# jhultman/vision3d

Measured on AMD Instinct MI355X. Metric: frames/sec SECOND fwd, 16k-pt KITTI cloud, higher is better.
Workload: dtype f16x3-scaled (fp32-class): fp32 operands split into f16 hi + lo pieces of x * s under per-tensor power-of-two scales, 3 MFMA terms (lo*hi + hi*lo + hi*hi), fp32 accumulate; relative product error 2^-22 -- the result differs from the reference's fp32 modules by fp32 summation noise: strict elementwis

## Files before the change

### include/vision3d_hip.h

```cpp
#ifndef VISION3D_HIP_H
#define VISION3D_HIP_H

#include <stddef.h>
#include <stdint.h>

#ifdef __cplusplus
extern "C" {
#endif

#define V3D_OK 0
#define V3D_EINVAL (-1)
#define V3D_EWORKSPACE (-2)
#define V3D_EUNSUPPORTED (-3)

typedef void* v3d_stream_t;

const char* v3d_version(void);
int v3d_hip_runtime_version(void);
const char* v3d_compiler_version(void);
const char* v3d_error_string(int code);

int v3d_box_iou_rotated(const float* boxes1, int M, const float* boxes2, int N, float* ious, v3d_stream_t stream);

int v3d_box_iou_rotated_3d(const float* boxes1, int M, const float* boxes2, int N, float* ious, v3d_stream_t stream);

size_t v3d_nms_rotated_workspace(int N);
int v3d_nms_rotated(const float* boxes, const float* scores, int N, float iou_threshold, int64_t* keep,
                    int32_t* n_keep, void* workspace, size_t workspace_bytes, v3d_stream_t stream);

size_t v3d_proposals_workspace(int B, int n_cls, int topk);
int v3d_proposals(const float* head_maps, const float* anchors, int B, int n_cls, int n_yaw, int H, int W, int topk,
                  const float* score_thresh_host, float iou_threshold, float* out_boxes, int64_t* out_batch_idx,
                  int64_t* out_class_idx, float* out_scores, int32_t* n_out, void* workspace, size_t workspace_bytes,
                  v3d_stream_t stream);
int v3d_proposals_flag(const float* head_maps, const float* anchors, int B, int n_cls, int n_yaw, int H, int W, int topk,
                       const float* score_thresh_host, float iou_threshold, float* out_boxes, int64_t* out_batch_idx,
                       int64_t* out_class_idx, float* out_scores, int32_t* n_out , const int32_t* aux_flag,
                       void* workspace, size_t workspace_bytes, v3d_stream_t stream);
int v3d_proposals_topk(const float* head_maps, const float* anchors, int B, int n_cls, int n_yaw, int H, int W, int topk,
                       float* boxes, float* scores, void* workspace, size_t workspace_bytes, v3d_stream_t stream);
size_t v3d_refine_nms_workspace(int B, int n_cls, int topk);
int v3d_refine_nms(const float* deltas, const float* proposals, const float* conf, int B, int n_cls, int topk,
                   const float* score_thresh_host, float iou_threshold, float* refined, float* out_boxes, int64_t* out_batch_idx,
                   int64_t* out_class_idx, float* out_scores, int32_t* n_out, void* workspace, size_t workspace_bytes,
                   v3d_stream_t stream);

size_t v3d_sparse_bn_workspace(int n, int C);
int v3d_sparse_bn_relu_fwd(const float* x, int n, int C, const float* gamma, const float* beta, float eps, int relu, float* y,
                           float* save_mean, float* save_invstd, float* var_unbiased, float* running_mean ,
                           float* running_var , float momentum,
                           int64_t* num_batches_tracked , void* workspace, size_t workspace_bytes,
                           v3d_stream_t stream);
int v3d_sparse_bn_relu_bwd(const float* x, const float* dy, int n, int C, const float* gamma, const float* beta,
                           const float* save_mean, const float* save_invstd, int relu, float* dx, float* dgamma, float* dbeta,
                           void* workspace, size_t workspace_bytes, v3d_stream_t stream);

size_t v3d_assign_targets_workspace(int n_gt, int n_cls, int anchors_per_class);
int v3d_assign_targets(const float* gt_boxes, const int64_t* gt_class, int n_gt, const float* anchors, int n_cls,
                       int anchors_per_class, const float* iou_thresh_host, int allow_low_quality, int8_t* G_cls, uint8_t* M_cls,
                       float* G_reg, uint8_t* M_reg, int64_t* matches, void* workspace, size_t workspace_bytes,
                       v3d_stream_t stream);

int v3d_refine_targets(const float* proposals, const int64_t* proposal_class, int B, int n, const float* gt_boxes,
                       const int64_t* gt_class, const int32_t* gt_offsets, int n_gt, const float* draws, float conf_lo, float conf_hi,
                       float reg_iou, float fg_iou, int rois_per_frame, int fg_quota, float* iou, int64_t* match, float* conf,
                       float* G_reg, uint8_t* M_cls, uint8_t* M_reg, v3d_stream_t stream);

size_t v3d_augment_work_bytes(int N, int n, int k);
int v3d_augment_frame(const float* points, int N, int C, const float* boxes, const int64_t* class_idx, int n,
                      const float* db_points, const float* db_boxes, const void* samples, int k, int sample_points, int flip,
                      double factor, double cos_theta, double sin_theta, double theta, float* out_points, float* out_boxes,
                      int64_t* out_class_idx, void* work, size_t work_bytes, v3d_stream_t stream);

size_t v3d_object_noise_workspace(int n_boxes, int T);
int v3d_object_noise(const float* points, const int32_t* point_offsets_host, const float* boxes, const int32_t* box_offsets_host,
                     int B, int C, const float* trans, const float* rot, int T, float collision_iou, float* out_points,
                     float* out_boxes, int32_t* chosen, void* workspace, size_t workspace_bytes, v3d_stream_t stream);

#define V3D_DATABASE_MAX_BOXES 256
size_t v3d_database_work_bytes(int n_points, int n_boxes, int n_frames);
int v3d_database_extract(const float* points, int n_points, int C, const int32_t* point_offsets, const double* box_prep, int n_boxes,
                         const int32_t* box_offsets, int n_frames, int min_pts, int32_t* counts, int32_t* starts, int32_t* src_index,
                         float* out_points, int64_t cap, int32_t* totals, void* work, size_t work_bytes, v3d_stream_t stream);

int v3d_points_in_boxes(const float* points, int N, int C, const float* boxes, int n, int use_z, uint8_t* mask,
                        v3d_stream_t stream);

size_t v3d_voxelize_workspace(int n_points);
int v3d_voxelize(const float* points, int n_points, int C, const int32_t* frame_offsets_host, int B,
                 const float* voxel_size_host, const float* bounds_host, int max_pts, int max_voxels, float* voxels,
                 int32_t* coords, int32_t* occupancy, float* mean, int32_t* n_voxels, void* workspace,
                 size_t workspace_bytes, v3d_stream_t stream);

size_t v3d_rulebook_workspace(int cap_in, int cap_out, int K);
int v3d_rulebook_subm(const int32_t* coords, const int32_t* n, int cap, const int32_t* spatial_shape_host,
                      const int32_t* ksize_host, int32_t* nbr, void* workspace, size_t workspace_bytes,
                      v3d_stream_t stream);
int v3d_rulebook_sparse(const int32_t* coords_in, const int32_t* n_in, int cap_in,
                        const int32_t* spatial_shape_host, const int32_t* ksize_host, const int32_t* stride_host,
                        const int32_t* padding_host, int32_t* coords_out, int32_t* n_out, int cap_out, int32_t* nbr,
                        int32_t* overflow, void* workspace, size_t workspace_bytes, v3d_stream_t stream);

int v3d_sparse_conv_fwd(const float* in, const float* weight, const int32_t* nbr, const int32_t* n_out, int cap_out,
                        int K, int Cin, int Cout, const float* scale, const float* shift, int relu, float* out,
                        int algo, v3d_stream_t stream);

#define V3D_PREC_BF16X3 0
#define V3D_PREC_F16S 1
size_t v3d_sparse_conv_weight_image_bytes(int K, int Cin, int Cout);
int v3d_sparse_conv_pack_weights(const float* weight, int K, int Cin, int Cout, int prec, void* image, v3d_stream_t stream);
int v3d_act_scale_from_rows(const float* rows, const int32_t* n_rows, int cap, int C, int headroom_bits, float* entry,
                            uint32_t* scratch, v3d_stream_t stream);
int v3d_sparse_conv_fwd_packed(const float* in, const void* weight_image, const int32_t* nbr, const int32_t* n_out,
                               int cap_out, int K, int Cin, int Cout, const float* scale, const float* shift, int relu,
                               float* out, int rows_hint, int prec, const float* act_in, const float* act_next,
                               int32_t* range_flag, const void* in_split, void* out_split, v3d_stream_t stream);
int v3d_sparse_rows_split(const float* rows, const int32_t* n_rows, int cap, int C, int prec, const float* act_entry,
                          void* out_split, v3d_stream_t stream);
size_t v3d_sparse_brick_table_bytes(int cap, int K, size_t* lidx_bytes, size_t* ulist_bytes, size_t* ucnt_bytes,
                                    size_t* tmask_bytes);
int v3d_sparse_brick_plan(const int32_t* nbr, const int32_t* n_rows, int cap, int K, uint16_t* lidx, int32_t* ulist,
                          int32_t* ucnt, uint32_t* tmask, v3d_stream_t stream);
int v3d_sparse_conv_fwd_brick(const void* in_split, const void* weight_image, const int32_t* nbr, const uint16_t* lidx,
                              const int32_t* ulist, const int32_t* ucnt, const uint32_t* tmask, const int32_t* n_out,
                              int cap, int K, int Cin, int Cout, const float* scale, const float* shift, int relu, float* out,
                              int prec, const float* act_in, const float* act_next, int32_t* range_flag, void* out_split,
                              v3d_stream_t stream);

int v3d_rulebook_transpose(const int32_t* nbr, const int32_t* n_out, int cap_out, int K, int cap_in, int32_t* nbr_t,
                           v3d_stream_t stream);
size_t v3d_sparse_conv_bwd_weight_workspace(int K, int Cin, int Cout);
int v3d_sparse_conv_bwd_weight(const float* X, const float* dY, const int32_t* nbr, const int32_t* n_out, int cap_out,
                               int K, int Cin, int Cout, float* dW, void* workspace, size_t workspace_bytes,
                               v3d_stream_t stream);

int v3d_densify(const float* feat, const int32_t* coords, const int32_t* n, int cap, int B, int C,
                const int32_t* spatial_shape_host, float* dense, v3d_stream_t stream);

size_t v3d_fps_workspace(int B, int N);
int v3d_furthest_point_sample(const float* xyz, int B, int N, int K, int32_t* idx, void* workspace,
                              size_t workspace_bytes, v3d_stream_t stream);
size_t v3d_keypoints_sector_workspace(int B, int N, int S);
int v3d_keypoints_sector(const float* points, int point_stride, int B, int N, int K, int S, const float* proposals, int P, float radius,
                         int32_t* idx, int32_t* sector_counts, void* workspace, size_t workspace_bytes, v3d_stream_t stream);
int v3d_gather_points(const float* feat, const int32_t* idx, int B, int C, int N, int K, float* out,
                      v3d_stream_t stream);
int v3d_ball_query(const float* xyz, const float* new_xyz, int B, int N, int M, float radius_a, int nsample_a, int32_t* idx_a,
                   float radius_b, int nsample_b, int32_t* idx_b, v3d_stream_t stream);
size_t v3d_ball_query_grid_workspace(int B, int N);
int v3d_ball_query_grid(const float* xyz, const float* new_xyz, int B, int N, int M, float radius_a, int nsample_a, int32_t* idx_a,
                        float radius_b, int nsample_b, int32_t* idx_b, void* workspace, size_t workspace_bytes, v3d_stream_t stream);
int v3d_ball_query_grid_build(int n_db, const float* const* xyz, const int32_t* N, const float* radius_max, void* const* workspace,
                              const size_t* workspace_bytes, int B, v3d_stream_t stream);
int v3d_ball_query_grid_query(const float* new_xyz, int B, int N, int M, float radius_a, int nsample_a, int32_t* idx_a,
                              float radius_b, int nsample_b, int32_t* idx_b, const void* workspace, size_t workspace_bytes,
                              v3d_stream_t stream);
int v3d_ball_query_grid_query_many(int n_jobs, const float* new_xyz, int B, int M, const int32_t* N, const float* radius_a,
                                   const int32_t* nsample_a, int32_t* const* idx_a, const float* radius_b, const int32_t* nsample_b,
                                   int32_t* const* idx_b, const void* const* workspace, const size_t* workspace_bytes,
                                   v3d_stream_t stream);
int v3d_group_points(const float* feat, const int32_t* idx, int B, int C, int N, int M, int nsample, float* out,
                     v3d_stream_t stream);
int v3d_bev_bilinear(const float* feature_map, const float* grid, int B, int C, int H, int W, int K, float* out,
                     v3d_stream_t stream);
int v3d_bev_gather_keypoints(const float* feature_map, const float* keypoint_xyz, int B, int C, int H, int W, int K, float offset_x,
                             float offset_y, float pixel_x, float pixel_y, float* out, int ldo, v3d_stream_t stream);

int v3d_voxel_centers(const int32_t* indices, int n, float scale_x, float scale_y, float scale_z, float offset_x, float offset_y,
                      float offset_z, float* out, v3d_stream_t stream);
int v3d_roi_grid_points(const float* boxes, const float* samples, const float* cos_yaw, const float* sin_yaw, int n_boxes, int m,
                        float* out, v3d_stream_t stream);

int v3d_sa_mlp_layer(const float* feat, const float* xyz, const float* new_xyz, const int32_t* idx, int B, int N, int M, int ns,
                     int Kf, const float* W, const float* bias, int Nout, int relu, int pool, float* out, int ldo, int n_store,
                     v3d_stream_t stream);
int v3d_sa_mlp_pair(const float* P, const float* xyz, const float* new_xyz, const int32_t* idx, int B, int N, int M, int ns, int K1,
                    int ldp, const float* wx, const float* b1, const float* W, const float* bias, int Nout, int relu, int pool,
                    float* out, int ldo, int n_store, v3d_stream_t stream);
int v3d_sa_mlp_pair2(const float* P_a, const float* P_b, const float* xyz, const float* new_xyz, const int32_t* idx_a, const int32_t* idx_b,
                     int B, int N, int M, int ns_a, int ns_b, int K1, int ldp, const float* wx_a, const float* b1_a, const float* wx_b,
                     const float* b1_b, const float* W_a, const float* bias_a, const float* W_b, const float* bias_b, int Nout, int relu,
                     int pool, float* out_a, float* out_b, int ldo, int n_store, v3d_stream_t stream);
int v3d_linear_rows(const float* A, int lda, int R, int K, const float* W, const float* bias, int Nout, int relu, float* out, int ldo,
                    int n_store, v3d_stream_t stream);
int v3d_linear_rows_many(int n_jobs, const float* const* A, const int32_t* lda, const int32_t* R, const int32_t* K, const float* const* W,
                         const float* const* bias, const int32_t* Nout, const int32_t* relu, float* const* out, const int32_t* ldo,
                         const int32_t* n_store, v3d_stream_t stream);

typedef struct v3d_backbone v3d_backbone;
typedef struct {
  int32_t subm;
  int32_t cin, cout;
  int32_t ksize[3], stride[3], padding[3];
  int32_t key;
  int32_t relu;
} v3d_layer_desc;
typedef struct {
  float voxel_size[3];
  float bounds[6];
  int32_t max_pts, max_voxels;
  int32_t point_channels;
  int32_t grid_shape[3];
  int32_t max_batch, max_points;
  int32_t n_layers;
  float growth;
  int32_t conv_algo;
} v3d_backbone_config;
int v3d_backbone_create(const v3d_backbone_config* cfg, const v3d_layer_desc* layers, v3d_backbone** out);
void v3d_backbone_destroy(v3d_backbone* plan);
size_t v3d_backbone_arena_bytes(const v3d_backbone* plan);
int v3d_backbone_num_layers(const v3d_backbone* plan);
int v3d_backbone_set_layer(v3d_backbone* plan, int layer, const float* weight, const float* scale, const float* shift,
                           v3d_stream_t stream);
int v3d_backbone_forward(v3d_backbone* plan, const float* points, int n_points, const int32_t* frame_offsets_host,
                         int B, float* dense_nchw, void* dense_hi, void* dense_lo, v3d_stream_t stream);
int v3d_backbone_layer_output(v3d_backbone* plan, int layer, float** features, int32_t** coords,
                              int32_t** n_rows_dev, int* cap, int* channels, int32_t* shape_host);
int v3d_backbone_tune(v3d_backbone* plan);
int32_t* v3d_backbone_occupancy(v3d_backbone* plan);
int32_t* v3d_backbone_overflow_flags(v3d_backbone* plan);

size_t v3d_conv2d_weight_image_bytes(int Cin, int Cout, int ksize);
size_t v3d_bev_occupancy_words(int B, int H, int W);
int v3d_bev_occupancy_bits(const int32_t* coords , const int32_t* n, int cap, int B, int H, int W,
                           uint32_t* occ, v3d_stream_t stream);
uint32_t* v3d_backbone_bev_occupancy(v3d_backbone* plan);
int v3d_backbone_bev_planes(v3d_backbone* plan, void** hi, void** lo);
int v3d_backbone_set_throughput_mode(v3d_backbone* plan, int on);
int v3d_backbone_set_precision(v3d_backbone* plan, int prec);
int v3d_backbone_precision(const v3d_backbone* plan);
int v3d_backbone_set_presplit(v3d_backbone* plan, int on);
float* v3d_backbone_act_scales(v3d_backbone* plan);
int v3d_backbone_set_calibrating(v3d_backbone* plan, int on);
int v3d_backbone_calibrate(v3d_backbone* plan, int headroom_bits, v3d_stream_t stream);
int v3d_conv2d_bg_tiles(int B, int H, int W);
typedef struct v3d_conv2d_prec {
  int32_t prec;
  const float* in_entry;
  const float* out_entry;
  int32_t* range_flag;
  const float* w_inv;
  const float* w_inv2;
} v3d_conv2d_prec;
int v3d_conv2d_pack_weights(const float* weight, const float* scale, int Cout, int Cin, int ksize, int prec, void* image,
                            v3d_stream_t stream);
int v3d_conv2d_nhwc_split(const void* x_hi, const void* x_lo, const void* weight_image, const float* bias, int relu, int B,
                          int H, int W, int Cin, int Cout, int ksize, void* y_hi, void* y_lo, float* y_nchw,
                          const uint32_t* occ, int reach, const void* bg_hi, const void* bg_lo, uint32_t* work,
                          uint32_t* tile_state, uint32_t* reset_ptr, int reset_words, const v3d_conv2d_prec* pr,
                          v3d_stream_t stream);
int v3d_conv2d_1x1_head_fused(const void* x_hi, const void* x_lo, const void* w1_image, const float* b1, int relu1,
                              const void* w2_image, const float* b2, int relu2, int B, int H, int W, int Cmid, int Cout2,
                              float* y_nchw, const v3d_conv2d_prec* pr, v3d_stream_t stream);
int v3d_nchw_to_split_nhwc(const float* x, int B, int C, int H, int W, void* out_hi, void* out_lo, int prec,
                           const float* act_entry, v3d_stream_t stream);
int v3d_densify_nhwc_split(const float* feat, const int32_t* coords, const int32_t* n, int cap, int B, int C,
                           const int32_t* spatial_shape_host, void* out_hi, void* out_lo, v3d_stream_t stream);
int v3d_split_nhwc_to_nchw(const void* x_hi, const void* x_lo, int B, int C, int H, int W, float* out, v3d_stream_t stream);
int v3d_backbone_forward_reuse(v3d_backbone* plan, int B, float* dense_nchw, void* dense_hi, void* dense_lo, v3d_stream_t stream);

int v3d_backbone_forward_voxels(v3d_backbone* plan, const float* voxel_mean, const int32_t* coords, int n_voxels, int B,
                                float* dense_nchw, void* dense_hi, void* dense_lo, v3d_stream_t stream);

size_t v3d_proposal_loss_workspace(void);
int v3d_proposal_loss_fwd_bwd(const float* maps, const int8_t* g_cls, const uint8_t* m_cls, const float* g_reg, const uint8_t* m_reg,
                              int B, int n_cls, int n_yaw, int H, int W, float alpha, float gamma, float* losses, float* dmaps,
                              void* workspace, size_t workspace_bytes, v3d_stream_t stream);
int v3d_proposal_loss_scale(float* dmaps, int B, int n_cls, int n_yaw, int H, int W, const float* g_cls, const float* g_reg,
                            v3d_stream_t stream);

int v3d_refine_loss_fwd_bwd(const float* R_reg, int ld_reg, const float* R_cls, int ld_cls, const float* G_conf, const float* G_reg,
                            const uint8_t* M_cls, const uint8_t* M_reg, int rows, float* losses, float* dR_reg, float* dR_cls,
                            v3d_stream_t stream);
int v3d_refine_loss_scale(float* dR_reg, float* dR_cls, int rows, const float* g_cls, const float* g_reg, v3d_stream_t stream);

int v3d_keypoint_weight(const float* hidden, int ldh, int H, const float* w2, const float* b2, float* feats, int ldf, int C,
                        int rows, float* logits, v3d_stream_t stream);

int v3d_keypoint_seg_loss_fwd_bwd(const float* keypoints, const float* logits, int B, int K, const float* gt_boxes,
                                  const int64_t* gt_class, const int32_t* gt_offsets, int n_gt, const float* extra_host, float alpha,
                                  float gamma, uint8_t* labels, float* losses, float* d_logits, v3d_stream_t stream);
int v3d_keypoint_seg_loss_scale(float* d_logits, int rows, const float* g, v3d_stream_t stream);

size_t v3d_voxel_query_workspace(int cap);
int v3d_voxel_query(const float* points, int rows, int rows_per_frame, const int32_t* coords, const int32_t* n, int cap,
                    const int32_t* shape_host, const float* scale_host, const float* offset_host, const int32_t* range_host,
                    float radius, int nsample, int32_t* idx, uint8_t* empty, void* workspace, size_t workspace_bytes,
                    v3d_stream_t stream);
int v3d_voxel_pool_pair(const float* P, int ldp, const int32_t* coords, int cap, const float* points, const int32_t* idx, int rows,
                        int nsample, const float* scale_host, const float* offset_host, int K1, const float* wx, const float* b1,
                        const float* W, const float* bias, int Nout, float* out, int ldo, v3d_stream_t stream);

int v3d_center_targets(const float* boxes, const int32_t* classes, const int32_t* box_offsets_host, int B, int n_cls, int H, int W,
                       const double* geom_host, double min_overlap, int min_radius, float* heat, int32_t* ind, uint8_t* mask,
                       int32_t* cls, float* reg, v3d_stream_t stream);
size_t v3d_center_loss_workspace(void);
int v3d_center_loss_fwd_bwd(const float* maps, const float* heat, const int32_t* ind, const uint8_t* mask, const float* reg, int B,
                            int n_cls, int H, int W, float alpha, float beta, const float* code_weights_host, float* losses,
                            float* dmaps, void* workspace, size_t workspace_bytes, v3d_stream_t stream);
int v3d_center_loss_scale(float* dmaps, int B, int n_cls, int H, int W, const float* g_hm, const float* g_reg, v3d_stream_t stream);
size_t v3d_center_decode_workspace(int B, int n_cls, int H, int W);
int v3d_center_decode(const float* maps, int B, int n_cls, int H, int W, const double* geom_host, int topk, float* boxes,
                      float* scores, void* workspace, size_t workspace_bytes, v3d_stream_t stream);

typedef struct {
  const float* weight;
  const float* gamma;
  const float* beta;
  float* running_mean;
  float* running_var;
  int64_t* num_batches_tracked;
  float eps, momentum;
  float* grad_weight;
  float* grad_gamma;
  float* grad_beta;
} v3d_train_layer;
int v3d_backbone_train_forward(v3d_backbone* plan, const float* voxel_mean, const int32_t* coords, int n_voxels, int B,
                               const v3d_train_layer* layers_host, float* dense_out ,
                               void* dense_nhwc_bf16 ,
                               v3d_stream_t stream);
int v3d_backbone_train_backward(v3d_backbone* plan, const float* grad_dense ,
                                const void* grad_nhwc_bf16, int B, const v3d_train_layer* layers_host, v3d_stream_t stream);
size_t v3d_backbone_train_arena_bytes(const v3d_backbone* plan);
int v3d_backbone_tune_from_voxels(v3d_backbone* plan, const int32_t* coords, int n_voxels, int B, v3d_stream_t stream);


size_t v3d_dense_train_weight_image_bytes(int ksize);
int v3d_dense_train_pack_weights(const float* weight, int ksize, int transpose, void* image, v3d_stream_t stream);
int v3d_dense_train_conv_tiles(int B, int H, int W);
int v3d_dense_train_conv(const void* x, const void* image, int B, int H, int W, int ksize, void* y, float* stats,
                         v3d_stream_t stream);
int v3d_dense_train_bn_finalize(const float* stats, int tiles, long long count, float eps, float momentum, float* mean,
                                float* invstd, float* running_mean, float* running_var, int64_t* num_batches_tracked,
                                v3d_stream_t stream);
int v3d_dense_train_bn_relu_apply(const void* x, long long M, const float* mean, const float* invstd, const float* gamma,
                                  const float* beta, int relu, void* y, v3d_stream_t stream);
size_t v3d_dense_train_bn_bwd_workspace(void);
int v3d_dense_train_bn_relu_bwd(const void* x, const void* dy, long long M, const float* mean, const float* invstd,
                                const float* gamma, const float* beta, int relu, void* dx, float* dgamma, float* dbeta,
                                void* workspace, size_t workspace_bytes, v3d_stream_t stream);
size_t v3d_dense_train_wgrad_workspace(int ksize);
int v3d_dense_train_wgrad(const void* x, const void* dy, int B, int H, int W, int ksize, float* dw, void* workspace,
                          size_t workspace_bytes, v3d_stream_t stream);
size_t v3d_dense_train_head_workspace(int O);
int v3d_dense_train_head_fwd(const void* feat, int B, int H, int W, const float* weight, const float* bias, int O, float* maps,
                             v3d_stream_t stream);
int v3d_dense_train_head_bwd(const void* feat, const float* dmaps, int B, int H, int W, const float* weight, int O, void* dfeat,
                             float* dweight, float* dbias, void* workspace, size_t workspace_bytes, v3d_stream_t stream);
typedef struct {
  const float* weight;
  const float* gamma;
  const float* beta;
  float* running_mean;
  float* running_var;
  int64_t* num_batches_tracked;
  float eps, momentum;
  int32_t ksize;
  float* grad_weight;
  float* grad_gamma;
  float* grad_beta;
} v3d_dense_train_layer;
size_t v3d_dense_train_arena_bytes(int B, int H, int W, int n_layers, int O);
int v3d_dense_train_arena_init(void* arena, int B, int H, int W, int n_layers, int O, v3d_stream_t stream);
int v3d_dense_train_forward(const void* bev, int B, int H, int W, const v3d_dense_train_layer* layers, int n_layers,
                            const float* head_weight, const float* head_bias, int O, void* arena, float* maps, v3d_stream_t stream);
int v3d_dense_train_backward(const void* bev, const float* dmaps, int B, int H, int W, const v3d_dense_train_layer* layers,
                             int n_layers, const float* head_weight, int O, void* arena, float* dhead_weight, float* dhead_bias,
                             void* dbev, v3d_stream_t stream);
size_t v3d_dense_train_arena_bytes_split(int B, int H, int W, int n_layers, int O);
int v3d_dense_train_forward_split(const void* bev_hi, const void* bev_lo, int B, int H, int W, const v3d_dense_train_layer* layers,
                                  int n_layers, const float* head_weight, const float* head_bias, int O, void* arena, float* maps,
                                  v3d_stream_t stream);
int v3d_dense_train_backward_split(const void* bev_hi, const void* bev_lo, const float* dmaps, int B, int H, int W,
                                   const v3d_dense_train_layer* layers, int n_layers, const float* head_weight, int O, void* arena,
                                   float* dhead_weight, float* dhead_bias, void* dbev_hi, void* dbev_lo, v3d_stream_t stream);

#define V3D_KITTI_MAX_DT 1024
#define V3D_KITTI_MAX_GT 256
#define V3D_KITTI_MAX_COMBOS 1024
#define V3D_KITTI_COMBO_CHUNK 64
#define V3D_KITTI_SAMPLE_PTS 41
#define V3D_KITTI_CODE_CAR 0
#define V3D_KITTI_CODE_PEDESTRIAN 1
#define V3D_KITTI_CODE_CYCLIST 2
// ... 37 lines not shown
```

### vision3d_amd/_lib.py

```python
import ctypes as C
import contextlib
import os

import torch

_HERE = os.path.dirname(os.path.abspath(__file__))
LIB_PATH = os.environ.get("V3D_HIP_LIB") or os.path.join(_HERE, "lib", "libvision3d_hip.so")

_vp, _i, _f, _sz = C.c_void_p, C.c_int, C.c_float, C.c_size_t

_SIGNATURES = {
    "v3d_version": (C.c_char_p, []),
    "v3d_hip_runtime_version": (_i, []),
    "v3d_compiler_version": (C.c_char_p, []),
    "v3d_error_string": (C.c_char_p, [_i]),
    "v3d_box_iou_rotated": (_i, [_vp, _i, _vp, _i, _vp, _vp]),
    "v3d_box_iou_rotated_3d": (_i, [_vp, _i, _vp, _i, _vp, _vp]),
    "v3d_nms_rotated_workspace": (_sz, [_i]),
    "v3d_nms_rotated": (_i, [_vp, _vp, _i, _f, _vp, _vp, _vp, _sz, _vp]),
    "v3d_proposals_workspace": (_sz, [_i, _i, _i]),
    "v3d_proposals": (_i, [_vp, _vp, _i, _i, _i, _i, _i, _i, _vp, _f, _vp, _vp, _vp, _vp, _vp, _vp, _sz, _vp]),
    "v3d_proposals_flag": (_i, [_vp, _vp, _i, _i, _i, _i, _i, _i, _vp, _f, _vp, _vp, _vp, _vp, _vp, _vp, _vp, _sz, _vp]),
    "v3d_proposals_topk": (_i, [_vp, _vp, _i, _i, _i, _i, _i, _i, _vp, _vp, _vp, _sz, _vp]),
    "v3d_refine_nms_workspace": (_sz, [_i, _i, _i]),
    "v3d_refine_nms": (_i, [_vp, _vp, _vp, _i, _i, _i, _vp, _f, _vp, _vp, _vp, _vp, _vp, _vp, _vp, _sz, _vp]),
    "v3d_sparse_bn_workspace": (_sz, [_i, _i]),
    "v3d_sparse_bn_relu_fwd": (_i, [_vp, _i, _i, _vp, _vp, _f, _i, _vp, _vp, _vp, _vp, _vp, _vp, _f, _vp, _vp, _sz, _vp]),
    "v3d_sparse_bn_relu_bwd": (_i, [_vp, _vp, _i, _i, _vp, _vp, _vp, _vp, _i, _vp, _vp, _vp, _vp, _sz, _vp]),
    "v3d_assign_targets_workspace": (_sz, [_i, _i, _i]),
    "v3d_assign_targets": (_i, [_vp, _vp, _i, _vp, _i, _i, _vp, _i, _vp, _vp, _vp, _vp, _vp, _vp, _sz, _vp]),
    "v3d_points_in_boxes": (_i, [_vp, _i, _i, _vp, _i, _i, _vp, _vp]),
    "v3d_augment_work_bytes": (_sz, [_i, _i, _i]),
    "v3d_augment_frame": (_i, [_vp, _i, _i, _vp, _vp, _i, _vp, _vp, _vp, _i, _i, _i, C.c_double, C.c_double, C.c_double, C.c_double,
                               _vp, _vp, _vp, _vp, _sz, _vp]),
    "v3d_object_noise_workspace": (_sz, [_i, _i]),
    "v3d_object_noise": (_i, [_vp, _vp, _vp, _vp, _i, _i, _vp, _vp, _i, _f, _vp, _vp, _vp, _vp, _sz, _vp]),
    "v3d_database_work_bytes": (_sz, [_i, _i, _i]),
    "v3d_database_extract": (_i, [_vp, _i, _i, _vp, _vp, _i, _vp, _i, _i, _vp, _vp, _vp, _vp, C.c_int64, _vp, _vp, _sz, _vp]),
    "v3d_voxelize_workspace": (_sz, [_i]),
    "v3d_voxelize": (_i, [_vp, _i, _i, _vp, _i, _vp, _vp, _i, _i, _vp, _vp, _vp, _vp, _vp, _vp, _sz, _vp]),
    "v3d_rulebook_workspace": (_sz, [_i, _i, _i]),
    "v3d_rulebook_subm": (_i, [_vp, _vp, _i, _vp, _vp, _vp, _vp, _sz, _vp]),
    "v3d_rulebook_sparse": (_i, [_vp, _vp, _i, _vp, _vp, _vp, _vp, _vp, _vp, _i, _vp, _vp, _vp, _sz, _vp]),
    "v3d_sparse_conv_fwd": (_i, [_vp, _vp, _vp, _vp, _i, _i, _i, _i, _vp, _vp, _i, _vp, _i, _vp]),
    "v3d_sparse_conv_weight_image_bytes": (_sz, [_i, _i, _i]),
    "v3d_sparse_conv_pack_weights": (_i, [_vp, _i, _i, _i, _i, _vp, _vp]),
    "v3d_sparse_conv_fwd_packed": (_i, [_vp, _vp, _vp, _vp, _i, _i, _i, _i, _vp, _vp, _i, _vp, _i, _i, _vp, _vp, _vp, _vp, _vp, _vp]),
    "v3d_sparse_rows_split": (_i, [_vp, _vp, _i, _i, _i, _vp, _vp, _vp]),
    "v3d_sparse_brick_table_bytes": (_sz, [_i, _i, _vp, _vp, _vp, _vp]),
    "v3d_sparse_brick_plan": (_i, [_vp, _vp, _i, _i, _vp, _vp, _vp, _vp, _vp]),
    "v3d_sparse_conv_fwd_brick": (_i, [_vp, _vp, _vp, _vp, _vp, _vp, _vp, _vp, _i, _i, _i, _i, _vp, _vp, _i, _vp, _i, _vp, _vp, _vp, _vp, _vp]),
    "v3d_act_scale_from_rows": (_i, [_vp, _vp, _i, _i, _i, _vp, _vp, _vp]),
    "v3d_rulebook_transpose": (_i, [_vp, _vp, _i, _i, _i, _vp, _vp]),
    "v3d_sparse_conv_bwd_weight_workspace": (_sz, [_i, _i, _i]),
    "v3d_sparse_conv_bwd_weight": (_i, [_vp, _vp, _vp, _vp, _i, _i, _i, _i, _vp, _vp, _sz, _vp]),
    "v3d_densify": (_i, [_vp, _vp, _vp, _i, _i, _i, _vp, _vp, _vp]),
    "v3d_fps_workspace": (_sz, [_i, _i]),
    "v3d_furthest_point_sample": (_i, [_vp, _i, _i, _i, _vp, _vp, _sz, _vp]),
    "v3d_keypoints_sector_workspace": (_sz, [_i, _i, _i]),
    "v3d_keypoints_sector": (_i, [_vp, _i, _i, _i, _i, _i, _vp, _i, _f, _vp, _vp, _vp, _sz, _vp]),
    "v3d_gather_points": (_i, [_vp, _vp, _i, _i, _i, _i, _vp, _vp]),
    "v3d_ball_query": (_i, [_vp, _vp, _i, _i, _i, _f, _i, _vp, _f, _i, _vp, _vp]),
    "v3d_ball_query_grid_workspace": (_sz, [_i, _i]),
    "v3d_ball_query_grid": (_i, [_vp, _vp, _i, _i, _i, _f, _i, _vp, _f, _i, _vp, _vp, _sz, _vp]),
    "v3d_ball_query_grid_build": (_i, [_i, _vp, _vp, _vp, _vp, _vp, _i, _vp]),
    "v3d_ball_query_grid_query_many": (_i, [_i, _vp, _i, _i, _vp, _vp, _vp, _vp, _vp, _vp, _vp, _vp, _vp, _vp]),
    "v3d_ball_query_grid_query": (_i, [_vp, _i, _i, _i, _f, _i, _vp, _f, _i, _vp, _vp, _sz, _vp]),
    "v3d_group_points": (_i, [_vp, _vp, _i, _i, _i, _i, _i, _vp, _vp]),
    "v3d_bev_bilinear": (_i, [_vp, _vp, _i, _i, _i, _i, _i, _vp, _vp]),
    "v3d_sa_mlp_layer": (_i, [_vp, _vp, _vp, _vp, _i, _i, _i, _i, _i, _vp, _vp, _i, _i, _i, _vp, _i, _i, _vp]),
    "v3d_sa_mlp_pair": (_i, [_vp, _vp, _vp, _vp, _i, _i, _i, _i, _i, _i, _vp, _vp, _vp, _vp, _i, _i, _i, _vp, _i, _i, _vp]),
    "v3d_voxel_centers": (_i, [_vp, _i, _f, _f, _f, _f, _f, _f, _vp, _vp]),
    "v3d_sa_mlp_pair2": (_i, [_vp, _vp, _vp, _vp, _vp, _vp, _i, _i, _i, _i, _i, _i, _i, _vp, _vp, _vp, _vp, _vp, _vp, _vp, _vp, _i, _i, _i,
                              _vp, _vp, _i, _i, _vp]),
    "v3d_roi_grid_points": (_i, [_vp, _vp, _vp, _vp, _i, _i, _vp, _vp]),
    "v3d_linear_rows_many": (_i, [_i, _vp, _vp, _vp, _vp, _vp, _vp, _vp, _vp, _vp, _vp, _vp, _vp]),
    "v3d_linear_rows": (_i, [_vp, _i, _i, _i, _vp, _vp, _i, _i, _vp, _i, _i, _vp]),
    "v3d_bev_gather_keypoints": (_i, [_vp, _vp, _i, _i, _i, _i, _i, _f, _f, _f, _f, _vp, _i, _vp]),
    "v3d_backbone_create": (_i, [_vp, _vp, _vp]),
    "v3d_backbone_destroy": (None, [_vp]),
    "v3d_backbone_arena_bytes": (_sz, [_vp]),
    "v3d_backbone_tune": (_i, [_vp]),
    "v3d_backbone_num_layers": (_i, [_vp]),
    "v3d_backbone_set_layer": (_i, [_vp, _i, _vp, _vp, _vp, _vp]),
    "v3d_backbone_layer_output": (_i, [_vp, _i, _vp, _vp, _vp, _vp, _vp, _vp]),
    "v3d_backbone_occupancy": (_vp, [_vp]),
    "v3d_backbone_overflow_flags": (_vp, [_vp]),
    "v3d_backbone_forward": (_i, [_vp, _vp, _i, _vp, _i, _vp, _vp, _vp, _vp]),
    "v3d_backbone_forward_reuse": (_i, [_vp, _i, _vp, _vp, _vp, _vp]),
    "v3d_backbone_forward_voxels": (_i, [_vp, _vp, _vp, _i, _i, _vp, _vp, _vp, _vp]),
    "v3d_backbone_train_forward": (_i, [_vp, _vp, _vp, _i, _i, _vp, _vp, _vp, _vp]),
    "v3d_backbone_train_backward": (_i, [_vp, _vp, _vp, _i, _vp, _vp]),
    "v3d_backbone_train_arena_bytes": (_sz, [_vp]),
    "v3d_backbone_tune_from_voxels": (_i, [_vp, _vp, _i, _i, _vp]),
    "v3d_bev_occupancy_words": (_sz, [_i, _i, _i]),
    "v3d_bev_occupancy_bits": (_i, [_vp, _vp, _i, _i, _i, _i, _vp, _vp]),
    "v3d_backbone_bev_occupancy": (_vp, [_vp]),
    "v3d_backbone_bev_planes": (_i, [_vp, C.POINTER(_vp), C.POINTER(_vp)]),
    "v3d_backbone_set_throughput_mode": (_i, [_vp, _i]),
    "v3d_conv2d_bg_tiles": (_i, [_i, _i, _i]),
    "v3d_conv2d_pack_weights": (_i, [_vp, _vp, _i, _i, _i, _i, _vp, _vp]),
    "v3d_conv2d_nhwc_split": (_i, [_vp, _vp, _vp, _vp, _i, _i, _i, _i, _i, _i, _i, _vp, _vp, _vp, _vp, _i, _vp, _vp, _vp, _vp, _vp, _i, _vp, _vp]),
    "v3d_conv2d_1x1_head_fused": (_i, [_vp, _vp, _vp, _vp, _i, _vp, _vp, _i, _i, _i, _i, _i, _i, _vp, _vp, _vp]),
    "v3d_nchw_to_split_nhwc": (_i, [_vp, _i, _i, _i, _i, _vp, _vp, _i, _vp, _vp]),
    "v3d_backbone_set_precision": (_i, [_vp, _i]),
    "v3d_backbone_precision": (_i, [_vp]),
    "v3d_backbone_set_presplit": (_i, [_vp, _i]),
    "v3d_backbone_act_scales": (_vp, [_vp]),
    "v3d_backbone_set_calibrating": (_i, [_vp, _i]),
    "v3d_backbone_calibrate": (_i, [_vp, _i, _vp]),
    "v3d_proposal_loss_workspace": (_sz, []),
    "v3d_proposal_loss_fwd_bwd": (_i, [_vp, _vp, _vp, _vp, _vp, _i, _i, _i, _i, _i, _f, _f, _vp, _vp, _vp, _sz, _vp]),
    "v3d_proposal_loss_scale": (_i, [_vp, _i, _i, _i, _i, _i, _vp, _vp, _vp]),
    "v3d_refine_targets": (_i, [_vp, _vp, _i, _i, _vp, _vp, _vp, _i, _vp, _f, _f, _f, _f, _i, _i, _vp, _vp, _vp, _vp, _vp, _vp, _vp]),
    "v3d_refine_loss_fwd_bwd": (_i, [_vp, _i, _vp, _i, _vp, _vp, _vp, _vp, _i, _vp, _vp, _vp, _vp]),
    "v3d_refine_loss_scale": (_i, [_vp, _vp, _i, _vp, _vp, _vp]),
    "v3d_keypoint_weight": (_i, [_vp, _i, _i, _vp, _vp, _vp, _i, _i, _i, _vp, _vp]),
    "v3d_keypoint_seg_loss_fwd_bwd": (_i, [_vp, _vp, _i, _i, _vp, _vp, _vp, _i, _vp, _f, _f, _vp, _vp, _vp, _vp]),
    "v3d_keypoint_seg_loss_scale": (_i, [_vp, _i, _vp, _vp]),
    "v3d_voxel_query_workspace": (_sz, [_i]),
    "v3d_voxel_query": (_i, [_vp, _i, _i, _vp, _vp, _i, _vp, _vp, _vp, _vp, _f, _i, _vp, _vp, _vp, _sz, _vp]),
    "v3d_voxel_pool_pair": (_i, [_vp, _i, _vp, _i, _vp, _vp, _i, _i, _vp, _vp, _i, _vp, _vp, _vp, _vp, _i, _vp, _i, _vp]),
    "v3d_center_targets": (_i, [_vp, _vp, _vp, _i, _i, _i, _i, _vp, C.c_double, _i, _vp, _vp, _vp, _vp, _vp, _vp]),
    "v3d_center_loss_workspace": (_sz, []),
    "v3d_center_loss_fwd_bwd": (_i, [_vp, _vp, _vp, _vp, _vp, _i, _i, _i, _i, _f, _f, _vp, _vp, _vp, _vp, _sz, _vp]),
    "v3d_center_loss_scale": (_i, [_vp, _i, _i, _i, _i, _vp, _vp, _vp]),
    "v3d_center_decode_workspace": (_sz, [_i, _i, _i, _i]),
    "v3d_center_decode": (_i, [_vp, _i, _i, _i, _i, _vp, _i, _vp, _vp, _vp, _sz, _vp]),
    "v3d_conv2d_weight_image_bytes": (_sz, [_i, _i, _i]),
    "v3d_densify_nhwc_split": (_i, [_vp, _vp, _vp, _i, _i, _i, _vp, _vp, _vp, _vp]),
    "v3d_split_nhwc_to_nchw": (_i, [_vp, _vp, _i, _i, _i, _i, _vp, _vp]),
    "v3d_dense_train_weight_image_bytes": (_sz, [_i]),
    "v3d_dense_train_pack_weights": (_i, [_vp, _i, _i, _vp, _vp]),
    "v3d_dense_train_conv_tiles": (_i, [_i, _i, _i]),
    "v3d_dense_train_conv": (_i, [_vp, _vp, _i, _i, _i, _i, _vp, _vp, _vp]),
    "v3d_dense_train_bn_finalize": (_i, [_vp, _i, C.c_longlong, _f, _f, _vp, _vp, _vp, _vp, _vp, _vp]),
    "v3d_dense_train_bn_relu_apply": (_i, [_vp, C.c_longlong, _vp, _vp, _vp, _vp, _i, _vp, _vp]),
    "v3d_dense_train_bn_bwd_workspace": (_sz, []),
    "v3d_dense_train_bn_relu_bwd": (_i, [_vp, _vp, C.c_longlong, _vp, _vp, _vp, _vp, _i, _vp, _vp, _vp, _vp, _sz, _vp]),
    "v3d_dense_train_wgrad_workspace": (_sz, [_i]),
    "v3d_dense_train_wgrad": (_i, [_vp, _vp, _i, _i, _i, _i, _vp, _vp, _sz, _vp]),
    "v3d_dense_train_head_workspace": (_sz, [_i]),
    "v3d_dense_train_head_fwd": (_i, [_vp, _i, _i, _i, _vp, _vp, _i, _vp, _vp]),
    "v3d_dense_train_head_bwd": (_i, [_vp, _vp, _i, _i, _i, _vp, _i, _vp, _vp, _vp, _vp, _sz, _vp]),
    "v3d_dense_train_arena_bytes": (_sz, [_i, _i, _i, _i, _i]),
    "v3d_dense_train_arena_init": (_i, [_vp, _i, _i, _i, _i, _i, _vp]),
    "v3d_dense_train_forward": (_i, [_vp, _i, _i, _i, _vp, _i, _vp, _vp, _i, _vp, _vp, _vp]),
    "v3d_dense_train_arena_bytes_split": (_sz, [_i, _i, _i, _i, _i]),
    "v3d_dense_train_forward_split": (_i, [_vp, _vp, _i, _i, _i, _vp, _i, _vp, _vp, _i, _vp, _vp, _vp]),
    "v3d_dense_train_backward_split": (_i, [_vp, _vp, _vp, _i, _i, _i, _vp, _i, _vp, _i, _vp, _vp, _vp, _vp, _vp, _vp]),
    "v3d_dense_train_backward": (_i, [_vp, _vp, _i, _i, _i, _vp, _i, _vp, _i, _vp, _vp, _vp, _vp, _vp]),
    "v3d_kitti_eval_overlaps": (_i, [_vp, _vp, _vp, _vp, _vp, _i, _i, _i, _vp, _vp, _vp]),
    "v3d_kitti_eval_overlaps_image": (_i, [_vp, _vp, _vp, _vp, _vp, _i, _i, _i, _vp, _vp]),
    "v3d_kitti_eval_pass1": (_i, [_vp, _vp, _vp, _vp, _vp, _vp, _vp, C.c_longlong, _i, _i, _i, _vp, _i, _i, _vp, _vp, _vp, _vp]),
    "v3d_kitti_eval_thresholds": (_i, [_vp, _i, _vp, _vp, _i, _vp, _vp, _vp]),
    "v3d_kitti_eval_pass2": (_i, [_vp, _vp, _vp, _vp, _vp, _vp, _vp, _vp, _vp, C.c_longlong, _i, _i, _i, _vp, _i, _vp, _vp, _vp,
                                  _vp, _vp]),
    "v3d_kitti_eval_ap": (_i, [_vp, _vp, _vp, _i, _vp, _vp, _vp]),
}


class LayerDesc(C.Structure):
    _fields_ = [("subm", C.c_int32), ("cin", C.c_int32), ("cout", C.c_int32), ("ksize", C.c_int32 * 3),
                ("stride", C.c_int32 * 3), ("padding", C.c_int32 * 3), ("key", C.c_int32), ("relu", C.c_int32)]


class BackboneConfig(C.Structure):
    _fields_ = [("voxel_size", C.c_float * 3), ("bounds", C.c_float * 6), ("max_pts", C.c_int32),
                ("max_voxels", C.c_int32), ("point_channels", C.c_int32), ("grid_shape", C.c_int32 * 3),
                ("max_batch", C.c_int32), ("max_points", C.c_int32), ("n_layers", C.c_int32), ("growth", C.c_float),
                ("conv_algo", C.c_int32)]



class Conv2dPrec(C.Structure):
    _fields_ = [("prec", C.c_int32), ("in_entry", _vp), ("out_entry", _vp), ("range_flag", _vp), ("w_inv", _vp), ("w_inv2", _vp)]


PREC_BF16X3, PREC_F16S = 0, 1
PRECISIONS = {"bf16x3": PREC_BF16X3, "fp32": PREC_F16S, "f16s": PREC_F16S}


class TrainLayer(C.Structure):
    _fields_ = [("weight", _vp), ("gamma", _vp), ("beta", _vp), ("running_mean", _vp), ("running_var", _vp),
                ("num_batches_tracked", _vp), ("eps", C.c_float), ("momentum", C.c_float), ("grad_weight", _vp),
                ("grad_gamma", _vp), ("grad_beta", _vp)]


class DenseTrainLayer(C.Structure):
    _fields_ = [("weight", _vp), ("gamma", _vp), ("beta", _vp), ("running_mean", _vp), ("running_var", _vp),
                ("num_batches_tracked", _vp), ("eps", C.c_float), ("momentum", C.c_float), ("ksize", C.c_int32),
                ("grad_weight", _vp), ("grad_gamma", _vp), ("grad_beta", _vp)]


class KittiCombo(C.Structure):
    _fields_ = [("cls", C.c_int32), ("neighbour", C.c_int32), ("difficulty", C.c_int32), ("metric", C.c_int32),
                ("min_overlap", C.c_float)]


_lib = None


class NativeLibraryMissing(RuntimeError):
    pass


def lib():
    global _lib
    if _lib is None:
        if not os.path.exists(LIB_PATH):
            raise NativeLibraryMissing(
                f"{LIB_PATH} not found: build it with `python -c 'import __graft_entry__ as g; g.build()'` "
                "(make -C vision3d_amd/csrc).  vision3d_amd has no CPU fallback.")
        handle = C.CDLL(LIB_PATH)
        for name, (res, args) in _SIGNATURES.items():
            fn = getattr(handle, name)
            fn.restype, fn.argtypes = res, args
        _lib = handle
    return _lib


def exported_symbols():
    return sorted(_SIGNATURES)


def check(code, what):
    if code != 0:
        msg = lib().v3d_error_string(int(code)).decode()
        raise RuntimeError(f"{what} failed: {msg} (code {code})")


_raw_stream = getattr(torch._C, "_cuda_getCurrentRawStream", None)


def stream_ptr():
    if _raw_stream is not None:
        return _raw_stream(torch.cuda.current_device())
    return torch.cuda.current_stream().cuda_stream


_NULL_GUARD = contextlib.nullcontext()


def device_guard(device):
    index = device.index if isinstance(device, torch.device) else torch.device(device).index
    if index is None or index == torch.cuda.current_device():
        return _NULL_GUARD
    return torch.cuda.device(index)


def ptr(t):
    return 0 if t is None else t.data_ptr()


def require_gpu(name, *tensors):
    for t in tensors:
        if t is not None and not t.is_cuda:
            raise RuntimeError(f"{name}: tensors must live on the GPU (vision3d_amd has no CPU path); got {t.device}")


# ... 38 lines not shown
```

### vision3d_amd/csrc/rb_device.h

```cpp
#pragma once
#include "v3d_internal.h"

struct RbGeom {
  int in_shape[3];
  int out_shape[3];
  int ks[3], stride[3], pad[3];
  int K;
  int kc[3], Kc;
};

#define RB_MAX_BATCH 64
__device__ __forceinline__ v3d_key_t rb_key(int b, int z, int y, int x, const int* shape) {
  return (((v3d_key_t)b * shape[0] + z) * shape[1] + y) * shape[2] + x;
}

template <int KPT>
__device__ __forceinline__ void rb_subm_entries(const int4* __restrict__ coords, int n, int cap, const RbGeom& g, const V3dHash& h,
                                                int* __restrict__ nbr, int kgroup, int o) {
  if (o >= n) return;
  const int4 c = coords[o];
  const bool keyed = (unsigned)c.x < (unsigned)RB_MAX_BATCH;
  v3d_key_t key[KPT], w[KPT];
  unsigned s[KPT];
  bool look[KPT];
// ... 143 lines not shown
    int k, oz, oy, ox, s = -1;
    if (rb_ticket(c, j, g, k, oz, oy, ox)) {
      s = (unsigned)c.x < (unsigned)RB_MAX_BATCH ? v3d_site_insert(h, rb_key(c.x, oz, oy, ox, g.out_shape), V3D_SITE_NO_ROW) : -1;
      if (s >= 0) {
        atomicMin(&first_ticket[s], (unsigned)t);
        s |= k << RB_SLOT_BITS;
      } else {
        atomicExch(overflow, 1);
        if (overflow_any) atomicExch(overflow_any, 1);
      }
    }
    cand_slot[t] = s;
  }
}

__device__ __forceinline__ bool rb_is_first(const int* cand_slot, const unsigned* first_ticket, long long t,
                                            long long nt) {
  if (t >= nt) return false;
  const int s = cand_slot[t];
  return s != -1 && first_ticket[s & RB_SLOT_MASK] == (unsigned)t;
}

#define RB_PER_THREAD (V3D_SCAN_CHUNK / V3D_BLOCK)
static_assert(RB_PER_THREAD == 8, "rb_first_flags loads two int4");
__device__ __forceinline__ unsigned rb_first_flags(const int* __restrict__ cand_slot, const unsigned* __restrict__ first_ticket,
                                                   long long t0, long long nt) {
  if (t0 >= nt) return 0u;
  const int4 a = *reinterpret_cast<const int4*>(cand_slot + t0);
  const int4 b = *reinterpret_cast<const int4*>(cand_slot + t0 + 4);
  const int s[8] = {a.x, a.y, a.z, a.w, b.x, b.y, b.z, b.w};
  unsigned flags = 0u;
#pragma unroll
  for (int r = 0; r < 8; r++)
    if (t0 + r < nt && s[r] != -1 && first_ticket[s[r] & RB_SLOT_MASK] == (unsigned)(t0 + r)) flags |= 1u << r;
  return flags;
}

#define RB_SCAN_LDS (32 + 2 * V3D_SCAN_CHUNK)
__device__ __forceinline__ void rb_scan_emit_body(const int4* __restrict__ coords, const int* __restrict__ n_ptr, int cap_in, const RbGeom& g,
                                                  const int* __restrict__ cand_slot, const unsigned* __restrict__ first_ticket,
                                                  int* __restrict__ chunk_counts, int cap_out, int4* __restrict__ coords_out,
                                                  int* __restrict__ vals, int* __restrict__ n_out, int* __restrict__ overflow,
                                                  int* __restrict__ overflow_any, int* __restrict__ nbr_init, const V3dHash& out_hash,
                                                  const int b, const int nblocks, unsigned char* __restrict__ lds_raw) {
  int* lds = reinterpret_cast<int*>(lds_raw);
  int* s_part = lds + 4;
  unsigned short* list = reinterpret_cast<unsigned short*>(lds_raw + 32);
  const long long nt = (long long)min(*n_ptr, cap_in) * g.Kc;
  const int tid = threadIdx.x, lane = tid & 63, w = tid >> 6;
  const long long base = (long long)b * V3D_SCAN_CHUNK;
  const bool live = base < nt, last = b == nblocks - 1;
  if (!live && !last) return;
  const long long t0 = base + (long long)tid * RB_PER_THREAD;
  const unsigned flags = live ? rb_first_flags(cand_slot, first_ticket, t0, nt) : 0u;
  const int mine = __popc(flags);
  int incl = mine;
#pragma unroll
  for (int off = 1; off < 64; off <<= 1) {
    const int t = __shfl_up(incl, off);
    if (lane >= off) incl += t;
  }
  if (lane == 63) lds[w] = incl;
  __syncthreads();
  const int cnt = lds[0] + lds[1] + lds[2] + lds[3];
  if (tid == 0 && live) v3d_publish_count(chunk_counts + b, cnt);
  {
    int lr = incl - mine;
    for (int i = 0; i < w; i++) lr += lds[i];
    unsigned f = flags;
    while (f) {
      const int r = __ffs(f) - 1;
      f &= f - 1;
      list[lr++] = (unsigned short)(tid * RB_PER_THREAD + r);
    }
  }
  __syncthreads();
  int word0 = -1;
  int4 c0 = make_int4(0, 0, 0, 0);
  if (tid < cnt) {
    const long long t = base + list[tid];
    word0 = cand_slot[t];
    c0 = coords[(int)(t / g.Kc)];
  }
  asm volatile("" ::: "memory");
  int part = 0;
  {
    const int n_live = (int)((nt + V3D_SCAN_CHUNK - 1) / V3D_SCAN_CHUNK);
    for (int i = tid; i < min(b, n_live); i += V3D_BLOCK) part += v3d_wait_count(chunk_counts + i);
#pragma unroll
    for (int off = 32; off > 0; off >>= 1) part += __shfl_xor(part, off);
    if (lane == 0) s_part[w] = part;
  }
  __syncthreads();
  const int prefix = s_part[0] + s_part[1] + s_part[2] + s_part[3];
  if (last && tid == 0) {
    const int total = prefix + cnt;
    if (total > cap_out) {
      atomicExch(overflow, 1);
      if (overflow_any) atomicExch(overflow_any, 1);
    }
    *n_out = min(total, cap_out);
  }
  if (!live) return;
  if (nbr_init) {
    const int c0r = min(prefix, cap_out), c1r = min(prefix + cnt, cap_out), w_ = c1r - c0r;
    for (int kk = tid >> 5; kk < g.K; kk += V3D_BLOCK / 32)
      for (int r = tid & 31; r < w_; r += 32) nbr_init[(size_t)kk * cap_out + c0r + r] = -1;
  }
  for (int q = tid; q < cnt; q += V3D_BLOCK) {
    const int rank = prefix + q;
    if (rank >= cap_out) break;
    int word = word0;
    int4 c = c0;
    if (q != tid) {
      const long long t = base + list[q];
      word = cand_slot[t];
      c = coords[(int)(t / g.Kc)];
    }
    const int s = word & RB_SLOT_MASK;
    int oz, oy, ox;
    rb_candidate(c, (int)((unsigned)word >> RB_SLOT_BITS), g, oz, oy, ox);
    coords_out[rank] = make_int4(c.x, oz, oy, ox);
    vals[s] = rank;
    v3d_site_set_row(out_hash, s, rb_key(c.x, oz, oy, ox, g.out_shape), (unsigned)rank);
  }
}

__device__ __forceinline__ void rb_fill_nbr_body(const int* __restrict__ n_ptr, int cap_in, int K, const int* __restrict__ cand_slot,
                                                 const int* __restrict__ vals, int cap_out, int* __restrict__ nbr, int fill_blocks,
                                                 const int4* __restrict__ coords_out, const int* __restrict__ n_out_ptr, const RbGeom& sg,
                                                 const V3dHash& sh, int* __restrict__ subm_nbr, int subm_blocks, const RbCandJob& job,
                                                 const int bid) {
  if (bid < fill_blocks) {
    const long long nt = (long long)min(*n_ptr, cap_in) * K;
    for (long long t = (long long)bid * V3D_BLOCK + threadIdx.x; t < nt; t += (long long)fill_blocks * V3D_BLOCK) {
      const int word = cand_slot[t];
      if (word == -1) continue;
      const int o = vals[word & RB_SLOT_MASK];
      if (o < 0) continue;
      nbr[(size_t)((unsigned)word >> RB_SLOT_BITS) * cap_out + o] = (int)(t / K);
    }
    return;
  }
  if (bid >= fill_blocks + subm_blocks) {
    rb_candidates_body(job.coords, job.n_ptr, job.cap_in, job.g, job.h, job.first_ticket, job.cand_slot, job.overflow,
                       job.overflow_any, bid - fill_blocks - subm_blocks, job.blocks);
    return;
  }
  const int idx = bid - fill_blocks;
  rb_subm_block(coords_out, min(*n_out_ptr, cap_out), cap_out, sg, sh, subm_nbr, idx);
}


struct RbScanJob {
  int blocks;
  int cap_in, cap_out;
  const int4* coords;
  const int* n_ptr;
  RbGeom g;
  const int* cand_slot;
  const unsigned* first_ticket;
  int* chunk_counts;
  int4* coords_out;
  int* vals;
  int* n_out;
  int* overflow;
  int* overflow_any;
  int* nbr_init;
  V3dHash out_hash;
};
struct RbFillJob {
  int blocks;
  const int* n_ptr;
  int cap_in, Kc;
  const int* cand_slot;
  const int* vals;
  int cap_out;
  int* nbr;
  int fill_blocks, subm_blocks;
  const int4* coords_out;
  const int* n_out;
  RbGeom sg;
  V3dHash sh;
  int* subm_nbr;
  RbCandJob job;
};
struct RbStep {
  int kind;
  RbScanJob scan;
  RbFillJob fill;
};

__device__ __forceinline__ void rb_rider_run(const RbScanJob& r, const int bid, unsigned char* __restrict__ lds) {
  rb_scan_emit_body(r.coords, r.n_ptr, r.cap_in, r.g, r.cand_slot, r.first_ticket, r.chunk_counts, r.cap_out, r.coords_out, r.vals, r.n_out,
                    r.overflow, r.overflow_any, r.nbr_init, r.out_hash, bid, r.blocks, lds);
}
```

### vision3d_amd/csrc/rulebook.hip

```cpp
#include "rb_device.h"

__global__ __launch_bounds__(V3D_BLOCK) void rb_hash_build_kernel(const int4* __restrict__ coords,
                                                                  const int* __restrict__ n_ptr, int cap,
                                                                  const RbGeom g, const V3dHash h,
                                                                  int* __restrict__ vals) {
  const int n = min(*n_ptr, cap);
  for (int i = blockIdx.x * V3D_BLOCK + threadIdx.x; i < n; i += gridDim.x * V3D_BLOCK) {
    const int4 c = coords[i];
    if ((unsigned)c.x >= (unsigned)RB_MAX_BATCH) continue;
    const int s = v3d_site_insert(h, rb_key(c.x, c.y, c.z, c.w, g.in_shape), (unsigned)i);
    if (s >= 0) vals[s] = i;
  }
}

__global__ __launch_bounds__(V3D_BLOCK) void rb_candidates_kernel(const int4* __restrict__ coords,
                                                                  const int* __restrict__ n_ptr, int cap_in,
                                                                  const RbGeom g, const V3dHash h,
                                                                  unsigned* __restrict__ first_ticket,
                                                                  int* __restrict__ cand_slot,
                                                                  int* __restrict__ overflow, int* __restrict__ overflow_any) {
  rb_candidates_body(coords, n_ptr, cap_in, g, h, first_ticket, cand_slot, overflow, overflow_any, blockIdx.x, gridDim.x);
}

__global__ __launch_bounds__(V3D_BLOCK) void rb_subm_nbr_kernel(const int4* __restrict__ coords,
                                                                const int* __restrict__ n_ptr, int cap,
                                                                const RbGeom g, const V3dHash h,
                                                                const int* __restrict__ vals, int* __restrict__ nbr,
                                                                int subm_blocks, const RbCandJob job) {
  if ((int)blockIdx.x >= subm_blocks) {
    rb_candidates_body(job.coords, job.n_ptr, job.cap_in, job.g, job.h, job.first_ticket, job.cand_slot, job.overflow,
                       job.overflow_any, blockIdx.x - subm_blocks, job.blocks);
    return;
  }
  rb_subm_block(coords, min(*n_ptr, cap), cap, g, h, nbr, blockIdx.x);
}

static int fill_geom(RbGeom& g, const int32_t* shape, const int32_t* ks, const int32_t* stride, const int32_t* pad) {
  g.K = 1;
  for (int j = 0; j < 3; j++) {
    g.in_shape[j] = shape[j];
    g.ks[j] = ks[j];
    g.stride[j] = stride ? stride[j] : 1;
    g.pad[j] = pad ? pad[j] : ks[j] / 2;
    if (g.in_shape[j] < 1 || g.ks[j] < 1 || g.stride[j] < 1 || g.pad[j] < 0) return V3D_EINVAL;
    g.out_shape[j] = (g.in_shape[j] + 2 * g.pad[j] - g.ks[j]) / g.stride[j] + 1;
    if (g.out_shape[j] < 1) return V3D_EINVAL;
    g.K *= g.ks[j];
  }
  g.Kc = 1;
  for (int j = 0; j < 3; j++) {
    g.kc[j] = (g.ks[j] + g.stride[j] - 1) / g.stride[j];
    g.Kc *= g.kc[j];
  }
  if (g.K > 62) return V3D_EUNSUPPORTED;
  if ((long long)g.in_shape[0] * g.in_shape[1] * g.in_shape[2] >= (1ll << 34)) return V3D_EUNSUPPORTED;
  if ((long long)g.out_shape[0] * g.out_shape[1] * g.out_shape[2] >= (1ll << 34)) return V3D_EUNSUPPORTED;
  return V3D_OK;
}

int v3d_i_hash_build(const int32_t* coords, const int32_t* n, int cap, const int32_t* shape, V3dRbHash h, int clear,
                     hipStream_t st) {
  RbGeom g;
  const int32_t ones[3] = {1, 1, 1};
  int rc = fill_geom(g, shape, ones, nullptr, nullptr);
  if (rc) return rc;
  if (cap > V3D_SITE_MAX_ROWS) return V3D_EUNSUPPORTED;
  if (clear) V3D_CHECK_HIP(v3d_fill_async(h.keys, 0xFF, (size_t)h.hcap * 8, st));
  V3dHash hh = v3d_make_hash(h.keys, h.hcap);
  hipLaunchKernelGGL(rb_hash_build_kernel, dim3(min(v3d_ceil_div(cap, V3D_BLOCK), 2048)), dim3(V3D_BLOCK), 0, st,
                     (const int4*)coords, n, cap, g, hh, h.vals);
  V3D_CHECK_LAUNCH();
  return V3D_OK;
}

static int make_cand_job(const V3dRbCandNext* next, RbCandJob& job) {
  job = RbCandJob{};
  if (!next) return V3D_OK;
  int rc = fill_geom(job.g, next->shape, next->ksize, next->stride, next->padding);
  if (rc) return rc;
  const long long tickets = (long long)next->cap_in * job.g.Kc;
  if (tickets >= (1ll << 31) || next->out.hcap > (1u << RB_SLOT_BITS)) return V3D_EUNSUPPORTED;
  if ((char*)next->first_ticket != (char*)next->out.keys + (size_t)next->out.hcap * 8 ||
      (char*)next->out.vals != (char*)next->first_ticket + (size_t)next->out.hcap * 4)
    return V3D_EINVAL;
  job.coords = (const int4*)next->coords_in;
  job.n_ptr = next->n_in;
  job.cap_in = next->cap_in;
  job.h = v3d_make_hash(next->out.keys, next->out.hcap);
  job.first_ticket = next->first_ticket;
  job.cand_slot = next->cand_slot;
  job.overflow = next->overflow;
  job.overflow_any = next->overflow_any;
  job.blocks = min(v3d_ceil_div(tickets, V3D_BLOCK), 4096);
  return V3D_OK;
}

int v3d_i_subm_nbr(const int32_t* coords, const int32_t* n, int cap, const int32_t* shape, const int32_t* ksize,
                   V3dRbHash h, int32_t* nbr, hipStream_t st, const V3dRbCandNext* next) {
  RbGeom g;
  int rc = fill_geom(g, shape, ksize, nullptr, nullptr);
  if (rc) return rc;
  for (int j = 0; j < 3; j++)
    if (!(g.ks[j] & 1)) return V3D_EINVAL;
  V3dHash hh = v3d_make_hash(h.keys, h.hcap);
  RbCandJob job;
  rc = make_cand_job(next, job);
  if (rc) return rc;
  const int subm_blocks = rb_subm_blocks(cap, g);
  hipLaunchKernelGGL(rb_subm_nbr_kernel, dim3(subm_blocks + job.blocks), dim3(V3D_BLOCK), 0, st,
                     (const int4*)coords, n, cap, g, hh, h.vals, nbr, subm_blocks, job);
  V3D_CHECK_LAUNCH();
  return V3D_OK;
}

__global__ __launch_bounds__(V3D_BLOCK) void rb_scan_emit_kernel(const RbScanJob r) {
  __shared__ __attribute__((aligned(16))) unsigned char lds[RB_SCAN_LDS];
  rb_rider_run(r, blockIdx.x, lds);
}
__global__ __launch_bounds__(V3D_BLOCK) void rb_fill_nbr_kernel(const int* __restrict__ n_ptr, int cap_in, int K,
                                                                const int* __restrict__ cand_slot,
                                                                const int* __restrict__ vals, int cap_out,
                                                                int* __restrict__ nbr, int fill_blocks,
                                                                const int4* __restrict__ coords_out,
                                                                const int* __restrict__ n_out_ptr, const RbGeom sg,
                                                                const V3dHash sh, int* __restrict__ subm_nbr, int subm_blocks,
                                                                const RbCandJob job) {
  rb_fill_nbr_body(n_ptr, cap_in, K, cand_slot, vals, cap_out, nbr, fill_blocks, coords_out, n_out_ptr, sg, sh, subm_nbr, subm_blocks, job,
                   blockIdx.x);
}
int v3d_i_rb_step_launch(const RbStep& s, hipStream_t st) {
  if (s.kind == 1) {
    if (s.scan.blocks < 1) return V3D_OK;
    hipLaunchKernelGGL(rb_scan_emit_kernel, dim3(s.scan.blocks), dim3(V3D_BLOCK), 0, st, s.scan);
  } else {
    const RbFillJob& f = s.fill;
    if (f.blocks < 1) return V3D_OK;
    hipLaunchKernelGGL(rb_fill_nbr_kernel, dim3(f.blocks), dim3(V3D_BLOCK), 0, st, f.n_ptr, f.cap_in, f.Kc, f.cand_slot, f.vals, f.cap_out, f.nbr,
                       f.fill_blocks, f.coords_out, f.n_out, f.sg, f.sh, f.subm_nbr, f.subm_blocks, f.job);
  }
  V3D_CHECK_LAUNCH();
  return V3D_OK;
}

int v3d_i_sparse_rulebook_steps(const int32_t* coords_in, const int32_t* n_in, int cap_in, const int32_t* shape,
                                const int32_t* ksize, const int32_t* stride, const int32_t* padding, int32_t* coords_out,
                                int32_t* n_out, int cap_out, int32_t* nbr, int32_t* overflow, V3dRbHash out,
                                unsigned* first_ticket, int* cand_slot, int* chunk_counts, const int32_t* next_subm_ksize,
                                int32_t* next_subm_nbr, int32_t* overflow_any, const V3dRbCandNext* next, int init_columns,
                                RbStep* scan, RbStep* fill) {
  RbGeom g;
  int rc = fill_geom(g, shape, ksize, stride, padding);
  if (rc) return rc;
  const long long tickets = (long long)cap_in * g.Kc;
  if (tickets >= (1ll << 31) || cap_out > V3D_SITE_MAX_ROWS || out.hcap > (1u << RB_SLOT_BITS)) return V3D_EUNSUPPORTED;
  if ((char*)first_ticket != (char*)out.keys + (size_t)out.hcap * 8 || (char*)out.vals != (char*)first_ticket + (size_t)out.hcap * 4)
    return V3D_EINVAL;
  *scan = RbStep{};
  scan->kind = 1;
  RbScanJob& r = scan->scan;
  r.blocks = v3d_ceil_div(tickets, V3D_SCAN_CHUNK);
  r.cap_in = cap_in;
  r.cap_out = cap_out;
  r.coords = (const int4*)coords_in;
  r.n_ptr = n_in;
  r.g = g;
  r.cand_slot = cand_slot;
  r.first_ticket = first_ticket;
  r.chunk_counts = chunk_counts;
  r.coords_out = (int4*)coords_out;
  r.vals = out.vals;
  r.n_out = n_out;
  r.overflow = overflow;
  r.overflow_any = overflow_any;
  r.nbr_init = init_columns ? nbr : nullptr;
  r.out_hash = v3d_make_hash(out.keys, out.hcap);
  *fill = RbStep{};
  fill->kind = 2;
  RbFillJob& f = fill->fill;
  f.n_ptr = n_in;
  f.cap_in = cap_in;
  f.Kc = g.Kc;
  f.cand_slot = cand_slot;
  f.vals = out.vals;
  f.cap_out = cap_out;
  f.nbr = nbr;
  f.fill_blocks = min(v3d_ceil_div(tickets, V3D_BLOCK), 4096);
  f.coords_out = (const int4*)coords_out;
  f.n_out = n_out;
  f.sg = g;
  f.sh = r.out_hash;
  if (next_subm_ksize && next_subm_nbr) {
    rc = fill_geom(f.sg, g.out_shape, next_subm_ksize, nullptr, nullptr);
    if (rc) return rc;
    for (int j = 0; j < 3; j++)
      if (!(f.sg.ks[j] & 1)) return V3D_EINVAL;
    f.subm_blocks = rb_subm_blocks(cap_out, f.sg);
    f.subm_nbr = next_subm_nbr;
  }
  rc = make_cand_job(next, f.job);
  if (rc) return rc;
  f.blocks = f.fill_blocks + f.subm_blocks + f.job.blocks;
  return V3D_OK;
}

int v3d_i_sparse_rulebook(const int32_t* coords_in, const int32_t* n_in, int cap_in, const int32_t* shape,
                          const int32_t* ksize, const int32_t* stride, const int32_t* padding, int32_t* coords_out,
                          int32_t* n_out, int cap_out, int32_t* nbr, int32_t* overflow, V3dRbHash out,
                          unsigned* first_ticket, int* cand_slot, int* chunk_counts, int32_t* out_shape, int clear,
                          const int32_t* next_subm_ksize, int32_t* next_subm_nbr, hipStream_t st, int32_t* overflow_any,
                          int candidates_done, const V3dRbCandNext* next, int init_columns) {
  RbStep scan, fill;
  int rc = v3d_i_sparse_rulebook_steps(coords_in, n_in, cap_in, shape, ksize, stride, padding, coords_out, n_out, cap_out, nbr, overflow,
                                       out, first_ticket, cand_slot, chunk_counts, next_subm_ksize, next_subm_nbr, overflow_any, next,
                                       init_columns, &scan, &fill);
  if (rc) return rc;
  const RbGeom& g = scan.scan.g;
  if (out_shape)
    for (int j = 0; j < 3; j++) out_shape[j] = g.out_shape[j];
  if (clear) {
    V3D_CHECK_HIP(v3d_fill_async(out.keys, 0xFF, (size_t)out.hcap * 16, st));
    V3D_CHECK_HIP(v3d_fill_async(nbr, 0xFF, (size_t)g.K * cap_out * 4, st));
    V3D_CHECK_HIP(v3d_fill_async(overflow, 0, 4, st));
    V3D_CHECK_HIP(v3d_fill_async(chunk_counts, 0xFF, (size_t)scan.scan.blocks * 4, st));
  }
  if (!candidates_done)
    hipLaunchKernelGGL(rb_candidates_kernel, dim3(fill.fill.fill_blocks), dim3(V3D_BLOCK), 0, st, (const int4*)coords_in, n_in, cap_in,
                       g, scan.scan.out_hash, first_ticket, cand_slot, overflow, overflow_any);
  rc = v3d_i_rb_step_launch(scan, st);
  if (rc) return rc;
  return v3d_i_rb_step_launch(fill, st);
}

extern "C" size_t v3d_rulebook_workspace(int cap_in, int cap_out, int K) {
  const size_t ci = (size_t)(cap_in > 0 ? cap_in : 1), co = (size_t)(cap_out > 0 ? cap_out : 1);
  const size_t hcap = v3d_hash_capacity((long long)(ci > co ? ci : co));
  const size_t tickets = ci * (size_t)(K > 0 ? K : 1);
  const size_t chunks = (tickets + V3D_SCAN_CHUNK - 1) / V3D_SCAN_CHUNK;
  return v3d_align(hcap * 8) + 2 * v3d_align(hcap * 4) + v3d_align(tickets * 4) + v3d_align(chunks * 4) + 256;
}

extern "C" int v3d_rulebook_subm(const int32_t* coords, const int32_t* n, int cap, const int32_t* spatial_shape_host,
                                 const int32_t* ksize_host, int32_t* nbr, void* workspace, size_t workspace_bytes,
                                 v3d_stream_t stream) {
  hipStream_t st = (hipStream_t)stream;
  if (!coords || !n || cap < 1 || !spatial_shape_host || !ksize_host || !nbr || !workspace) return V3D_EINVAL;
  const unsigned hcap = v3d_hash_capacity(cap);
  V3dArena ar(workspace, workspace_bytes);
  V3dRbHash h;
  h.keys = ar.take<v3d_key_t>(hcap);
  h.vals = ar.take<int>(hcap);
  h.hcap = hcap;
  if (!ar.ok()) return V3D_EWORKSPACE;
  int rc = v3d_i_hash_build(coords, n, cap, spatial_shape_host, h, 1, st);
  if (rc) return rc;
  return v3d_i_subm_nbr(coords, n, cap, spatial_shape_host, ksize_host, h, nbr, st, nullptr);
}

extern "C" int v3d_rulebook_sparse(const int32_t* coords_in, const int32_t* n_in, int cap_in,
                                   const int32_t* spatial_shape_host, const int32_t* ksize_host,
                                   const int32_t* stride_host, const int32_t* padding_host, int32_t* coords_out,
                                   int32_t* n_out, int cap_out, int32_t* nbr, int32_t* overflow, void* workspace,
                                   size_t workspace_bytes, v3d_stream_t stream) {
  hipStream_t st = (hipStream_t)stream;
// ... 45 lines not shown
```

### vision3d_amd/csrc/second_plan.hip

```cpp
#include <algorithm>
#include <new>
#include <vector>

#include "v3d_internal.h"
#include "rb_device.h"
#include "split_prec.h"

struct PlanLayer {
  v3d_layer_desc d;
  int K;
  int stage_in, stage_out;
  int rulebook;
  bool builds_rulebook;
  float *weight, *scale, *shift, *out;
  void* out_s;
  void* wimg;
  int has_affine;
  int* chunk_counts;
  int rows_hint;
  int rows_hint_in;
  int cand_buf;
};

struct PlanTrain;

struct PlanStage {
  int cap;
  int hash_items;
  int shape[3];
  int32_t* coords;
  int32_t* n_dev;
  V3dRbHash hash;
  unsigned* first_ticket;
  bool hash_ready_by_sparse;
};

struct v3d_backbone {
  v3d_backbone_config cfg;
  std::vector<PlanLayer> layers;
  std::vector<PlanStage> stages;
  std::vector<int32_t*> nbr;
  std::vector<int> nbr_cap;
  void* arena = nullptr;
  size_t arena_bytes = 0;
  void* vox_ws = nullptr;
  size_t vox_ws_bytes = 0;
  int32_t* occupancy = nullptr;
  float* mean = nullptr;
  int* cand_slot[2] = {nullptr, nullptr};
  int32_t* overflow = nullptr;
  char* ff_begin = nullptr;
  size_t ff_bytes = 0;
  int out_channels = 0;
  uint32_t* bev_occ = nullptr;
  void *bev_hi = nullptr, *bev_lo = nullptr;
  int32_t *bev_pix = nullptr, *bev_pix_n = nullptr;
  int ring_tiles_min = 2;
#ifdef V3D_EXP_NO_RIDERS
  bool rb_riders = false;
#else
  bool rb_riders = true;
#endif
  int prec = V3D_PREC_BF16X3;
  bool calibrating = false;
  bool presplit = true;
  bool fp32_rows = true;
  float* act_tab = nullptr;
  float* w_inv_tab = nullptr;
  unsigned* frame_max = nullptr;
  const int32_t** entry_rows = nullptr;
  struct PlanTrain* train = nullptr;
};

static int conv_fan(const v3d_layer_desc& d) {
  int fan = 1;
  for (int j = 0; j < 3; j++) fan *= (d.ksize[j] + d.stride[j] - 1) / d.stride[j];
  return fan;
}

extern "C" int v3d_backbone_create(const v3d_backbone_config* cfg, const v3d_layer_desc* descs, v3d_backbone** out) {
  if (!cfg || !descs || !out || cfg->n_layers < 1 || cfg->max_batch < 1 || cfg->max_points < 1) return V3D_EINVAL;
  if (cfg->max_batch > 64) return V3D_EUNSUPPORTED;
  v3d_backbone* p = new (std::nothrow) v3d_backbone();
  if (!p) return V3D_EINVAL;
  p->cfg = *cfg;
  const float growth = cfg->growth > 0.f ? cfg->growth : 2.0f;
  long long cap0 = (long long)cfg->max_batch * cfg->max_voxels;
  if (cap0 > cfg->max_points) cap0 = cfg->max_points;
  if (cap0 < 1) cap0 = 1;

  PlanStage s0{};
  s0.hash_items = (int)cap0;
  cap0 = (cap0 + 63) / 64 * 64;
  if ((cap0 / 64) % 2 == 0) cap0 += 64;
  s0.cap = (int)cap0;
  for (int j = 0; j < 3; j++) s0.shape[j] = cfg->grid_shape[j];
  p->stages.push_back(s0);
  std::vector<int> key_to_rb;
  std::vector<int> key_stage, key_id;
  int cur = 0, cin = cfg->point_channels, n_strided = 0;
  long long max_tickets = 1;
  for (int l = 0; l < cfg->n_layers; l++) {
    PlanLayer L{};
    L.d = descs[l];
    if (L.d.cin != cin) { delete p; return V3D_EINVAL; }
    L.K = L.d.ksize[0] * L.d.ksize[1] * L.d.ksize[2];
    if (L.K < 1 || L.K > 62) { delete p; return V3D_EUNSUPPORTED; }
    L.stage_in = cur;
    if (L.d.subm) {
      L.stage_out = cur;
      int found = -1;
      if (L.d.key >= 0)
        for (size_t i = 0; i < key_id.size(); i++)
          if (key_id[i] == L.d.key && key_stage[i] == cur) found = key_to_rb[i];
      if (found >= 0) {
        L.rulebook = found;
        L.builds_rulebook = false;
      } else {
        L.rulebook = (int)p->nbr_cap.size();
        L.builds_rulebook = true;
        p->nbr_cap.push_back(p->stages[cur].cap);
        if (L.d.key >= 0) { key_id.push_back(L.d.key); key_stage.push_back(cur); key_to_rb.push_back(L.rulebook); }
      }
    } else {
      PlanStage ns{};
      long long cells = cfg->max_batch;
      for (int j = 0; j < 3; j++) {
        ns.shape[j] = (p->stages[cur].shape[j] + 2 * L.d.padding[j] - L.d.ksize[j]) / L.d.stride[j] + 1;
        if (ns.shape[j] < 1) { delete p; return V3D_EINVAL; }
        cells *= ns.shape[j];
      }
      long long cap = (long long)p->stages[cur].cap * conv_fan(L.d);
      if (cap > cells) cap = cells;
      const long long lim = (long long)(cap0 * (double)growth);
      if (cap > lim) cap = lim;
      if (cap < 1) cap = 1;
      ns.hash_items = (int)cap;
      cap = (cap + 63) / 64 * 64;
      if ((cap / 64) % 2 == 0) cap += 64;
      ns.cap = (int)cap;
      ns.hash_ready_by_sparse = true;
      const long long tickets = (long long)p->stages[cur].cap * conv_fan(L.d);
      if (tickets > max_tickets) max_tickets = tickets;
      p->stages.push_back(ns);
      cur = (int)p->stages.size() - 1;
      L.stage_out = cur;
      L.rulebook = (int)p->nbr_cap.size();
      L.builds_rulebook = true;
      L.cand_buf = n_strided++ & 1;
      p->nbr_cap.push_back(ns.cap);
    }
    L.rows_hint = L.rows_hint_in = 0;
    cin = L.d.cout;
    p->layers.push_back(L);
  }
  p->out_channels = cin;

  for (const auto& st : p->stages)
    if (st.cap > V3D_SITE_MAX_ROWS) { delete p; return V3D_EUNSUPPORTED; }
  auto carve = [&](V3dArena& ar) {
    p->ff_begin = ar.base + ar.off;
    p->vox_ws_bytes = v3d_voxelize_workspace(cfg->max_points);
    p->vox_ws = ar.take<char>(p->vox_ws_bytes);
    for (auto& st : p->stages) {
      st.hash.hcap = v3d_hash_capacity(st.hash_items);
      st.hash.keys = ar.take<v3d_key_t>(st.hash.hcap);
      st.first_ticket = ar.take<unsigned>(st.hash.hcap);
      st.hash.vals = ar.take<int>(st.hash.hcap);
    }
    p->nbr.resize(p->nbr_cap.size());
    std::vector<int> rbK(p->nbr_cap.size(), 1);
    for (auto& L : p->layers) rbK[L.rulebook] = L.K;
    p->overflow = ar.take<int32_t>(p->layers.size() + 1);
    {
      const PlanStage& sl = p->stages.back();
      p->bev_occ = ar.take<uint32_t>(v3d_bev_occupancy_words(cfg->max_batch, sl.shape[1], sl.shape[2]));
    }
    for (auto& L : p->layers)
      if (!L.d.subm) L.chunk_counts = ar.take<int>((size_t)v3d_ceil_div((long long)p->stages[L.stage_in].cap * conv_fan(L.d), V3D_SCAN_CHUNK) + 2);
    p->ff_bytes = (size_t)((ar.base + ar.off) - p->ff_begin);
    for (size_t i = 0; i < p->nbr.size(); i++) p->nbr[i] = ar.take<int32_t>((size_t)rbK[i] * p->nbr_cap[i]);
    p->occupancy = ar.take<int32_t>(p->stages[0].cap);
    p->mean = ar.take<float>((size_t)p->stages[0].cap * cfg->point_channels);
    for (auto& st : p->stages) {
      st.coords = ar.take<int32_t>((size_t)st.cap * 4);
      st.n_dev = ar.take<int32_t>(1);
    }
    {
      const PlanStage& sl = p->stages.back();
      const size_t plane = (size_t)cfg->max_batch * sl.shape[0] * sl.shape[1] * sl.shape[2] * p->out_channels * 2;
      p->bev_hi = ar.take<char>(plane);
      p->bev_lo = ar.take<char>(plane);
      p->bev_pix = ar.take<int32_t>(sl.cap);
      p->bev_pix_n = ar.take<int32_t>(1);
    }
    p->act_tab = ar.take<float>(4 * (p->layers.size() + 1) + p->layers.size());
    p->w_inv_tab = p->act_tab + 4 * (p->layers.size() + 1);
    p->frame_max = ar.take<unsigned>(p->layers.size() + 1);
    p->entry_rows = ar.take<const int32_t*>(p->layers.size() + 1);
    p->cand_slot[0] = ar.take<int>((size_t)max_tickets);
    p->cand_slot[1] = ar.take<int>((size_t)max_tickets);
    for (auto& L : p->layers) {
      L.weight = ar.take<float>((size_t)L.K * L.d.cin * L.d.cout);
      L.wimg = ar.take<char>(v3d_sparse_conv_weight_image_bytes(L.K, L.d.cin, L.d.cout));
      L.scale = ar.take<float>(L.d.cout);
      L.shift = ar.take<float>(L.d.cout);
      L.out = ar.take<float>((size_t)p->stages[L.stage_out].cap * L.d.cout);
      L.out_s = (&L != &p->layers.back() && L.d.cout % 8 == 0) ? (void*)ar.take<float>((size_t)p->stages[L.stage_out].cap * L.d.cout) : nullptr;
    }
  };
  {
    V3dArena probe((void*)256, (size_t)1 << 60);
    carve(probe);
    p->arena_bytes = probe.off + 4096;
  }
  hipError_t e = hipMalloc(&p->arena, p->arena_bytes);
  if (e != hipSuccess) { delete p; return (int)e; }
  V3dArena ar(p->arena, p->arena_bytes);
  carve(ar);
  if (!ar.ok()) { (void)hipFree(p->arena); delete p; return V3D_EWORKSPACE; }
  e = hipMemset(p->ff_begin, 0xFF, p->ff_bytes);
  if (e == hipSuccess) e = hipMemset(p->bev_hi, 0, (size_t)((char*)p->bev_lo - (char*)p->bev_hi) * 2);
  if (e == hipSuccess) e = hipMemset(p->bev_pix_n, 0, sizeof(int32_t));
  if (e == hipSuccess) e = hipMemset(p->frame_max, 0, (p->layers.size() + 1) * sizeof(unsigned));
  if (e == hipSuccess) {
    std::vector<const int32_t*> rows(p->layers.size() + 1);
    rows[0] = p->stages[0].n_dev;
    for (size_t l = 0; l < p->layers.size(); l++) rows[l + 1] = p->stages[p->layers[l].stage_out].n_dev;
    e = hipMemcpy(p->entry_rows, rows.data(), rows.size() * sizeof(const int32_t*), hipMemcpyHostToDevice);
  }
  if (e == hipSuccess) {
    std::vector<float> tab;
    for (size_t i = 0; i <= p->layers.size(); i++) tab.insert(tab.end(), {1.f, 1.f, 32768.f, 0.f});
    for (size_t i = 0; i < p->layers.size(); i++) tab.push_back(1.f);
    e = hipMemcpy(p->act_tab, tab.data(), tab.size() * sizeof(float), hipMemcpyHostToDevice);
  }
  if (e != hipSuccess) { (void)hipFree(p->arena); delete p; return (int)e; }
  *out = p;
  return V3D_OK;
}

static void plan_train_free(v3d_backbone* p);

extern "C" void v3d_backbone_destroy(v3d_backbone* p) {
  if (!p) return;
  plan_train_free(p);
  if (p->arena) (void)hipFree(p->arena);
  delete p;
}

extern "C" size_t v3d_backbone_arena_bytes(const v3d_backbone* p) { return p ? p->arena_bytes : 0; }

extern "C" int v3d_backbone_set_layer(v3d_backbone* p, int layer, const float* weight, const float* scale,
                                      const float* shift, v3d_stream_t stream) {
  if (!p || layer < 0 || layer >= (int)p->layers.size() || !weight) return V3D_EINVAL;
  if ((scale == nullptr) != (shift == nullptr)) return V3D_EINVAL;
  hipStream_t st = (hipStream_t)stream;
  PlanLayer& L = p->layers[layer];
  V3D_CHECK_HIP(hipMemcpyAsync(L.weight, weight, (size_t)L.K * L.d.cin * L.d.cout * 4, hipMemcpyDeviceToDevice, st));
  L.has_affine = scale != nullptr;
  if (L.d.cout % 16 == 0) {
    int rc = v3d_sparse_conv_pack_weights(L.weight, L.K, L.d.cin, L.d.cout, p->prec, L.wimg, stream);
    if (rc) return rc;
    if (p->prec == V3D_PREC_F16S) {
      const char* trailer = (const char*)L.wimg + v3d_sparse_conv_weight_image_bytes(L.K, L.d.cin, L.d.cout) - V3D_WIMG_TRAILER;
      V3D_CHECK_HIP(hipMemcpyAsync(p->w_inv_tab + layer, trailer + V3D_WIMG_INV_SCALE * sizeof(float), sizeof(float), hipMemcpyDeviceToDevice, st));
    }
  }
  if (scale) {
    V3D_CHECK_HIP(hipMemcpyAsync(L.scale, scale, (size_t)L.d.cout * 4, hipMemcpyDeviceToDevice, st));
    V3D_CHECK_HIP(hipMemcpyAsync(L.shift, shift, (size_t)L.d.cout * 4, hipMemcpyDeviceToDevice, st));
  }
  return V3D_OK;
}

static int plan_run_layers(v3d_backbone* p, int B, bool hash0_done, float* dense_out, void* dense_hi, void* dense_lo,
                           hipStream_t st, bool reuse_rulebooks = false);

__global__ __launch_bounds__(256) void plan_frame_start_kernel(uint4* __restrict__ ff, size_t nvec, int fill_blocks,
                                                               const int* __restrict__ pix, const int* __restrict__ n_ptr, int cap,
                                                               int units, uint4* __restrict__ hi, uint4* __restrict__ lo,
                                                               unsigned* __restrict__ frame_max, int n_frame_max) {
  if (blockIdx.x == 0 && (int)threadIdx.x < n_frame_max) frame_max[threadIdx.x] = 0u;
  if ((int)blockIdx.x < fill_blocks) {
    for (size_t i = (size_t)blockIdx.x * 256 + threadIdx.x; i < nvec; i += (size_t)fill_blocks * 256)
      ff[i] = make_uint4(0xFFFFFFFFu, 0xFFFFFFFFu, 0xFFFFFFFFu, 0xFFFFFFFFu);
    return;
  }
  const long long total = (long long)min(*n_ptr, cap) * units;
  const int nb = gridDim.x - fill_blocks;
  for (long long t = (long long)(blockIdx.x - fill_blocks) * 256 + threadIdx.x; t < total; t += (long long)nb * 256) {
    const size_t o = (size_t)pix[t / units] * units + (size_t)(t % units);
    hi[o] = make_uint4(0u, 0u, 0u, 0u);
    lo[o] = make_uint4(0u, 0u, 0u, 0u);
  }
}

static int plan_own_planes(v3d_backbone* p, void* dense_hi, void* dense_lo, bool& own) {
  own = false;
  if (!dense_hi && !dense_lo) return V3D_OK;
  if ((dense_hi == p->bev_hi) != (dense_lo == p->bev_lo)) return V3D_EINVAL;
  own = dense_hi == p->bev_hi;
  return V3D_OK;
}

static int plan_frame_start(v3d_backbone* p, void* dense_hi, void* dense_lo, hipStream_t st) {
  bool own;
  int rc = plan_own_planes(p, dense_hi, dense_lo, own);
  if (rc) return rc;
  if (!own || (p->ff_bytes & 15) || ((uintptr_t)p->ff_begin & 15) || (p->out_channels * p->stages.back().shape[0]) % 8) {
    V3D_CHECK_HIP(v3d_fill_async(p->ff_begin, 0xFF, p->ff_bytes, st));
    V3D_CHECK_HIP(v3d_fill_async(p->frame_max, 0, (p->layers.size() + 1) * sizeof(unsigned), st));
    if (!own) return V3D_OK;
    const PlanStage& sl = p->stages.back();
    return v3d_i_bev_clear_pixels(p->bev_pix, p->bev_pix_n, sl.cap, p->out_channels * sl.shape[0], p->bev_hi, p->bev_lo, st);
  }
  const PlanStage& sl = p->stages.back();
  const int units = p->out_channels * sl.shape[0] / 8;
  const size_t nvec = p->ff_bytes / 16;
  const int fill_blocks = (int)std::min<size_t>((nvec + 255) / 256, 4096);
  const int clear_blocks = (int)std::min<long long>(v3d_ceil_div((long long)sl.cap * units, 256), 1024);
  hipLaunchKernelGGL(plan_frame_start_kernel, dim3(fill_blocks + clear_blocks), dim3(256), 0, st, (uint4*)p->ff_begin, nvec, fill_blocks,
                     p->bev_pix, p->bev_pix_n, sl.cap, units, (uint4*)p->bev_hi, (uint4*)p->bev_lo, p->frame_max, (int)p->layers.size() + 1);
  V3D_CHECK_LAUNCH();
  return V3D_OK;
}

__global__ __launch_bounds__(64) void plan_quiet_check_kernel(const float* __restrict__ act_tab, const unsigned* __restrict__ seen,
                                                              const int32_t* const* __restrict__ entry_rows, int n_entries,
                                                              int* __restrict__ flag) {
  bool quiet = false;
  for (int l = 1 + (int)threadIdx.x; l < n_entries; l += 64)
    quiet |= seen[l] == 0u && *entry_rows[l] > 0 && act_tab[4 * l + 3] != 0.f;
  if (__ballot(quiet) != 0ull && threadIdx.x == 0) atomicMax(flag, V3D_FLAG_QUIET);
}

static int plan_clear_own_planes(v3d_backbone* p, void* dense_hi, void* dense_lo, hipStream_t st) {
  bool own;
  int rc = plan_own_planes(p, dense_hi, dense_lo, own);
  if (rc || !own) return rc;
  const PlanStage& sl = p->stages.back();
  return v3d_i_bev_clear_pixels(p->bev_pix, p->bev_pix_n, sl.cap, p->out_channels * sl.shape[0], p->bev_hi, p->bev_lo, st);
}

extern "C" int v3d_backbone_set_throughput_mode(v3d_backbone* p, int on) {
  if (!p) return V3D_EINVAL;
  p->ring_tiles_min = on ? 4 : 2;
  p->fp32_rows = !on;
  return V3D_OK;
}

extern "C" int v3d_backbone_bev_planes(v3d_backbone* p, void** hi, void** lo) {
  if (!p || !hi || !lo) return V3D_EINVAL;
  *hi = p->bev_hi;
  *lo = p->bev_lo;
  return V3D_OK;
}

extern "C" int v3d_backbone_set_precision(v3d_backbone* p, int prec) {
  if (!p || (prec != V3D_PREC_BF16X3 && prec != V3D_PREC_F16S)) return V3D_EINVAL;
  p->prec = prec;
  return V3D_OK;
}
extern "C" int v3d_backbone_precision(const v3d_backbone* p) { return p ? p->prec : V3D_EINVAL; }

extern "C" int v3d_backbone_set_presplit(v3d_backbone* p, int on) {
  if (!p) return V3D_EINVAL;
  p->presplit = on != 0;
  return V3D_OK;
}

extern "C" float* v3d_backbone_act_scales(v3d_backbone* p) { return p ? p->act_tab : nullptr; }

extern "C" int v3d_backbone_set_calibrating(v3d_backbone* p, int on) {
  if (!p) return V3D_EINVAL;
  p->calibrating = on != 0;
  return V3D_OK;
}

extern "C" int v3d_backbone_calibrate(v3d_backbone* p, int headroom_bits, v3d_stream_t stream) {
  if (!p || headroom_bits < 0 || headroom_bits > 12) return V3D_EINVAL;
  for (size_t l = 0; l <= p->layers.size(); l++) {
    const float* rows = l == 0 ? p->mean : p->layers[l - 1].out;
    const int C = l == 0 ? p->cfg.point_channels : p->layers[l - 1].d.cout;
    const PlanStage& sg = p->stages[l == 0 ? 0 : p->layers[l - 1].stage_out];
    int rc = v3d_act_scale_from_rows(rows, sg.n_dev, sg.cap, C, headroom_bits, p->act_tab + 4 * l, nullptr, stream);
    if (rc) return rc;
  }
  return V3D_OK;
}

extern "C" int v3d_backbone_forward(v3d_backbone* p, const float* points, int n_points,
                                     const int32_t* frame_offsets_host, int B, float* dense_out, void* dense_hi,
                                     void* dense_lo, v3d_stream_t stream) {
  if (!p || !frame_offsets_host || B < 1 || B > p->cfg.max_batch || n_points < 0 || n_points > p->cfg.max_points)
    return V3D_EINVAL;
  hipStream_t st = (hipStream_t)stream;
  const v3d_backbone_config& c = p->cfg;
  PlanStage& s0 = p->stages[0];
  {
    const int rcc = plan_frame_start(p, dense_hi, dense_lo, st);
    if (rcc) return rcc;
  }
  const bool vox_hash = !p->layers.empty() && p->layers[0].d.subm && p->layers[0].builds_rulebook;
  int rc = v3d_i_voxelize(points, n_points, c.point_channels, frame_offsets_host, B, c.voxel_size, c.bounds, c.max_pts,
                          c.max_voxels, nullptr, s0.coords, p->occupancy, p->mean, s0.n_dev, p->vox_ws, p->vox_ws_bytes, 0,
                          vox_hash ? &s0.hash : nullptr, s0.shape, st);
  if (rc) return rc;
  return plan_run_layers(p, B, vox_hash, dense_out, dense_hi, dense_lo, st);
}

extern "C" int v3d_backbone_forward_reuse(v3d_backbone* p, int B, float* dense_out, void* dense_hi, void* dense_lo,
                                          v3d_stream_t stream) {
  if (!p || B < 1 || B > p->cfg.max_batch) return V3D_EINVAL;
  {
    const int rcc = plan_clear_own_planes(p, dense_hi, dense_lo, (hipStream_t)stream);
    if (rcc) return rcc;
  }
  return plan_run_layers(p, B, true, dense_out, dense_hi, dense_lo, (hipStream_t)stream, true);
}

extern "C" int v3d_backbone_forward_voxels(v3d_backbone* p, const float* voxel_mean, const int32_t* coords, int n_voxels, int B,
                                           float* dense_out, void* dense_hi, void* dense_lo, v3d_stream_t stream) {
  if (!p || !voxel_mean || !coords || B < 1 || B > p->cfg.max_batch || n_voxels < 0 || n_voxels > p->stages[0].cap)
    return V3D_EINVAL;
  hipStream_t st = (hipStream_t)stream;
  PlanStage& s0 = p->stages[0];
  {
    const int rcc = plan_frame_start(p, dense_hi, dense_lo, st);
    if (rcc) return rcc;
  }
  if (n_voxels > 0) {
    V3D_CHECK_HIP(hipMemcpyAsync(s0.coords, coords, (size_t)n_voxels * 4 * sizeof(int32_t), hipMemcpyDeviceToDevice, st));
    V3D_CHECK_HIP(hipMemcpyAsync(p->mean, voxel_mean, (size_t)n_voxels * p->cfg.point_channels * sizeof(float),
                                 hipMemcpyDeviceToDevice, st));
  }
  V3D_CHECK_HIP(hipMemsetD32Async((hipDeviceptr_t)s0.n_dev, n_voxels, 1, st));
  return plan_run_layers(p, B, false, dense_out, dense_hi, dense_lo, st);
}

static bool plan_next_strided(v3d_backbone* p, size_t l, int stage, std::vector<char>* cand_done, V3dRbCandNext& nx) {
  if (!cand_done) return false;
  for (size_t m = l + 1; m < p->layers.size(); m++) {
    PlanLayer& M = p->layers[m];
    if (!M.builds_rulebook || M.d.subm || M.stage_in != stage) continue;
    if ((*cand_done)[m]) return false;
    PlanStage &mi = p->stages[M.stage_in], &mo = p->stages[M.stage_out];
    nx.coords_in = mi.coords; nx.n_in = mi.n_dev; nx.cap_in = mi.cap; nx.shape = mi.shape;
    nx.ksize = M.d.ksize; nx.stride = M.d.stride; nx.padding = M.d.padding;
    nx.out = mo.hash; nx.first_ticket = mo.first_ticket; nx.cand_slot = p->cand_slot[M.cand_buf];
    nx.overflow = p->overflow + m; nx.overflow_any = p->overflow + p->layers.size();
    (*cand_done)[m] = 1;
    return true;
  }
  return false;
}

struct PlanRbQueue {
  std::vector<RbStep> steps;
  std::vector<int> rb_step;
  size_t launched = 0;
};
static int plan_rb_flush(PlanRbQueue& q, int upto , hipStream_t st) {
  while ((int)q.launched <= upto && q.launched < q.steps.size()) {
    const int rc = v3d_i_rb_step_launch(q.steps[q.launched++], st);
    if (rc) return rc;
  }
  return V3D_OK;
}

static int plan_layer_rulebook(v3d_backbone* p, size_t l, std::vector<char>& rb_done, bool& hash0_done, hipStream_t st,
                               std::vector<char>* cand_done = nullptr, PlanRbQueue* defer = nullptr) {
  PlanLayer& L = p->layers[l];
  if (!L.builds_rulebook || rb_done[l]) return V3D_OK;
  PlanStage& si = p->stages[L.stage_in];
  PlanStage& so = p->stages[L.stage_out];
  int rc;
  V3dRbCandNext nx;
  if (L.d.subm) {
    if (defer) {
      rc = plan_rb_flush(*defer, (int)defer->steps.size() - 1, st);
      if (rc) return rc;
    }
    if (!si.hash_ready_by_sparse && !(L.stage_in == 0 && hash0_done)) {
      rc = v3d_i_hash_build(si.coords, si.n_dev, si.cap, si.shape, si.hash, 0, st);
      if (rc) return rc;
      if (L.stage_in == 0) hash0_done = true;
    }
    const bool carry = plan_next_strided(p, l, L.stage_in, cand_done, nx);
    return v3d_i_subm_nbr(si.coords, si.n_dev, si.cap, si.shape, L.d.ksize, si.hash, p->nbr[L.rulebook], st, carry ? &nx : nullptr);
  }
  const bool fuse = l + 1 < p->layers.size() && p->layers[l + 1].d.subm && p->layers[l + 1].builds_rulebook &&
                    p->layers[l + 1].stage_in == L.stage_out;
  const int mine_done = cand_done && (*cand_done)[l];
  const bool carry = plan_next_strided(p, l, L.stage_out, cand_done, nx);
  if (defer && mine_done) {
    RbStep scan, fill;
    rc = v3d_i_sparse_rulebook_steps(si.coords, si.n_dev, si.cap, si.shape, L.d.ksize, L.d.stride, L.d.padding, so.coords, so.n_dev, so.cap,
                                     p->nbr[L.rulebook], p->overflow + l, so.hash, so.first_ticket, p->cand_slot[L.cand_buf], L.chunk_counts,
                                     fuse ? p->layers[l + 1].d.ksize : nullptr, fuse ? p->nbr[p->layers[l + 1].rulebook] : nullptr,
                                     p->overflow + p->layers.size(), carry ? &nx : nullptr, 1, &scan, &fill);
    if (rc) return rc;
    defer->steps.push_back(scan);
    defer->steps.push_back(fill);
    defer->rb_step[L.rulebook] = (int)defer->steps.size() - 1;
    if (fuse) {
      rb_done[l + 1] = 1;
      defer->rb_step[p->layers[l + 1].rulebook] = (int)defer->steps.size() - 1;
    }
    return V3D_OK;
  }
  if (defer) {
    rc = plan_rb_flush(*defer, (int)defer->steps.size() - 1, st);
    if (rc) return rc;
  }
  rc = v3d_i_sparse_rulebook(si.coords, si.n_dev, si.cap, si.shape, L.d.ksize, L.d.stride, L.d.padding, so.coords, so.n_dev,
                             so.cap, p->nbr[L.rulebook], p->overflow + l, so.hash, so.first_ticket, p->cand_slot[L.cand_buf],
                             L.chunk_counts, nullptr, 0, fuse ? p->layers[l + 1].d.ksize : nullptr,
                             fuse ? p->nbr[p->layers[l + 1].rulebook] : nullptr, st,
                             p->overflow + p->layers.size() , mine_done, carry ? &nx : nullptr,
                             1 );
  if (fuse) rb_done[l + 1] = 1;
  return rc;
}

static int plan_layer_conv(v3d_backbone* p, PlanLayer& L, const float* feat, const void* wimg, const float* weight,
                           const float* scale, const float* shift, int relu, float* out, hipStream_t st,
                           const V3dDensifyOut* densify = nullptr, bool* densified = nullptr, bool inference = false,
                           const void** feat_split = nullptr ,
                           const RbScanJob* rider = nullptr, bool* rider_taken = nullptr ) {
  const v3d_backbone_config& c = p->cfg;
  PlanStage& so = p->stages[L.stage_out];
  int rc = V3D_EUNSUPPORTED;
  if (densified) *densified = false;
  if (rider_taken) *rider_taken = false;
  if (v3d_ablate('c') || (v3d_ablate('r') && L.d.cin == 64 && L.d.cout == 64 && L.K == 27)) return V3D_OK;
  const bool exact_pass = inference && p->calibrating;
  if (!exact_pass && (c.conv_algo == 4 || (c.conv_algo == 0 && L.d.cin >= 16))) {
    const int prec = inference ? p->prec : V3D_PREC_BF16X3;
    const size_t l = (size_t)(&L - p->layers.data());
    const V3dActScale as{p->act_tab + 4 * l, p->act_tab + 4 * (l + 1), p->overflow + p->layers.size(), p->w_inv_tab + l,
#ifdef V3D_EXP_NO_SEEN
                         nullptr};
#else
                         inference ? p->frame_max + l + 1 : nullptr};
#endif
    const void* in_s = feat_split ? *feat_split : nullptr;
    const bool next_packed = l + 1 < p->layers.size() && p->layers[l + 1].d.cin >= 16 && (c.conv_algo == 4 || c.conv_algo == 0) &&
                             v3d_i_sparse_conv_packed_supported(p->layers[l + 1].d.cin, p->layers[l + 1].d.cout);
    void* out_s = (feat_split && p->presplit && next_packed && (prec == V3D_PREC_F16S || !p->fp32_rows)) ? L.out_s : nullptr;
    if (out_s && !p->fp32_rows && !densify && v3d_i_sparse_conv_packed_supported(L.d.cin, L.d.cout)) out = nullptr;
    rc = v3d_i_sparse_conv_fwd_packed(feat, wimg, p->nbr[L.rulebook], so.n_dev, so.cap, L.K, L.d.cin, L.d.cout, scale, shift,
                                      relu, out, L.rows_hint, st, densify, p->ring_tiles_min, prec, &as, in_s, out_s, rider, rider_taken);
    if (rc == V3D_OK && densify && densified) *densified = true;
    if (feat_split) *feat_split = rc == V3D_OK ? out_s : nullptr;
  } else if (feat_split) {
    *feat_split = nullptr;
  }
  if (rc == V3D_EUNSUPPORTED) {
    const bool check = inference && p->prec == V3D_PREC_F16S && !p->calibrating;
    const size_t l = (size_t)(&L - p->layers.data());
    rc = v3d_i_sparse_conv_fwd_exact(feat, weight, p->nbr[L.rulebook], so.n_dev, so.cap, L.K, L.d.cin, L.d.cout, scale, shift, relu,
                                     out, exact_pass ? 0 : ((c.conv_algo == 4 || c.conv_algo == 0) ? 3 : c.conv_algo), st,
                                     check ? p->act_tab + 4 * (l + 1) : nullptr, check ? p->overflow + p->layers.size() : nullptr,
                                     check ? p->frame_max + l + 1 : nullptr, rider, rider_taken);
  }
  return rc;
}

static int plan_run_layers(v3d_backbone* p, int B, bool hash0_done, float* dense_out, void* dense_hi, void* dense_lo,
                           hipStream_t st, bool reuse_rulebooks) {
  int rc = V3D_OK;
  std::vector<char> rb_done(p->layers.size(), 0);
  const float* feat = p->mean;
  const void* feat_split = nullptr;
  std::vector<char> cand_done(p->layers.size(), 0);
  bool densified = false;
  PlanRbQueue rbq;
  const bool riders = !reuse_rulebooks && p->rb_riders;
  if (riders) {
    rbq.rb_step.assign(p->nbr.size(), -1);
    for (size_t l = 0; l < p->layers.size(); l++) {
      rc = plan_layer_rulebook(p, l, rb_done, hash0_done, st, &cand_done, &rbq);
      if (rc) return rc;
    }
  }
  for (size_t l = 0; l < p->layers.size(); l++) {
    PlanLayer& L = p->layers[l];
    if (!reuse_rulebooks && !riders) {
      rc = plan_layer_rulebook(p, l, rb_done, hash0_done, st, &cand_done);
      if (rc) return rc;
    }
    const RbScanJob* rider = nullptr;
    bool rider_taken = false;
    if (riders) {
      rc = plan_rb_flush(rbq, rbq.rb_step[L.rulebook], st);
      if (rc) return rc;
      if (rbq.launched < rbq.steps.size() && rbq.steps[rbq.launched].kind == 2) {
        rc = plan_rb_flush(rbq, (int)rbq.launched, st);
        if (rc) return rc;
      }
      if (rbq.launched < rbq.steps.size() && rbq.steps[rbq.launched].kind == 1) rider = &rbq.steps[rbq.launched].scan;
    }
    V3dDensifyOut dn{};
    const bool want_dn = l + 1 == p->layers.size() && !dense_out && dense_hi == p->bev_hi && dense_lo == p->bev_lo && dense_hi &&
                         L.K != 27 && L.rows_hint < 32768 && L.d.cin >= 16 && L.d.cout % 16 == 0;
    if (want_dn) {
      const PlanStage& sl = p->stages.back();
      dn = V3dDensifyOut{sl.coords, sl.shape[0], sl.shape[1], sl.shape[2], p->bev_hi, p->bev_lo, p->bev_occ, p->bev_pix, p->bev_pix_n};
    }
    rc = plan_layer_conv(p, L, feat, L.wimg, L.weight, L.has_affine ? L.scale : nullptr, L.has_affine ? L.shift : nullptr,
                         L.d.relu, L.out, st, want_dn ? &dn : nullptr, &densified, true, &feat_split, rider, &rider_taken);
    if (rc) return rc;
    if (rider_taken) rbq.launched++;
    feat = L.out;
  }
  if (riders) {
    rc = plan_rb_flush(rbq, (int)rbq.steps.size() - 1, st);
    if (rc) return rc;
  }
  if (dense_out) {
    PlanStage& sl = p->stages.back();
    rc = v3d_densify(feat, sl.coords, sl.n_dev, sl.cap, B, p->out_channels, sl.shape, dense_out, st);
    if (rc) return rc;
  }
  if ((dense_hi || dense_lo) && !densified) {
    PlanStage& sl = p->stages.back();
    const bool own = dense_hi == p->bev_hi && dense_lo == p->bev_lo;
    rc = v3d_i_densify_nhwc_split(feat, sl.coords, sl.n_dev, sl.cap, B, p->out_channels, sl.shape, dense_hi, dense_lo, p->bev_occ,
                                  st, own ? p->bev_pix : nullptr, own ? p->bev_pix_n : nullptr, p->prec,
                                  p->act_tab + 4 * p->layers.size(), p->overflow + p->layers.size(),
                                  p->prec == V3D_PREC_F16S && !p->calibrating ? p->frame_max + p->layers.size() : nullptr);
    if (rc) return rc;
  }
#ifndef V3D_EXP_NO_SEEN
  if (p->prec == V3D_PREC_F16S && !p->calibrating) {
    hipLaunchKernelGGL(plan_quiet_check_kernel, dim3(1), dim3(64), 0, st, p->act_tab, p->frame_max, p->entry_rows, (int)p->layers.size() + 1,
                       p->overflow + (int)p->layers.size());
    V3D_CHECK_LAUNCH();
  }
#endif
  return V3D_OK;
}

extern "C" int v3d_backbone_layer_output(v3d_backbone* p, int layer, float** features, int32_t** coords,
                                         int32_t** n_rows_dev, int* cap, int* channels, int32_t* shape_host) {
  if (!p || layer < -1 || layer >= (int)p->layers.size()) return V3D_EINVAL;
  if (layer < 0) {
    if (features) *features = p->mean;
    if (coords) *coords = p->stages[0].coords;
    if (n_rows_dev) *n_rows_dev = p->stages[0].n_dev;
    if (cap) *cap = p->stages[0].cap;
    if (channels) *channels = p->cfg.point_channels;
    if (shape_host)
      for (int j = 0; j < 3; j++) shape_host[j] = p->stages[0].shape[j];
    return V3D_OK;
  }
  PlanLayer& L = p->layers[layer];
  PlanStage& so = p->stages[L.stage_out];
  if (features) *features = L.out;
  if (coords) *coords = so.coords;
  if (n_rows_dev) *n_rows_dev = so.n_dev;
  if (cap) *cap = so.cap;
  if (channels) *channels = L.d.cout;
  if (shape_host)
    for (int j = 0; j < 3; j++) shape_host[j] = so.shape[j];
  return V3D_OK;
}

extern "C" int v3d_backbone_tune(v3d_backbone* p) {
  if (!p) return V3D_EINVAL;
  std::vector<int> n_stage(p->stages.size(), 0);
  for (size_t s = 0; s < p->stages.size(); s++) {
    hipError_t e = hipMemcpy(&n_stage[s], p->stages[s].n_dev, sizeof(int), hipMemcpyDeviceToHost);
    if (e != hipSuccess) return (int)e;
  }
  for (auto& L : p->layers) {
    L.rows_hint = n_stage[L.stage_out];
    L.rows_hint_in = n_stage[L.stage_in];
  }
  return V3D_OK;
}

extern "C" int v3d_backbone_tune_from_voxels(v3d_backbone* p, const int32_t* coords, int n_voxels, int B, v3d_stream_t stream) {
  if (!p || !coords || B < 1 || B > p->cfg.max_batch || n_voxels < 1 || n_voxels > p->stages[0].cap) return V3D_EINVAL;
  hipStream_t st = (hipStream_t)stream;
  PlanStage& s0 = p->stages[0];
  V3D_CHECK_HIP(v3d_fill_async(p->ff_begin, 0xFF, p->ff_bytes, st));
  V3D_CHECK_HIP(hipMemcpyAsync(s0.coords, coords, (size_t)n_voxels * 4 * sizeof(int32_t), hipMemcpyDeviceToDevice, st));
  V3D_CHECK_HIP(hipMemsetD32Async((hipDeviceptr_t)s0.n_dev, n_voxels, 1, st));
  std::vector<char> rb_done(p->layers.size(), 0);
  bool hash0_done = false;
  for (size_t l = 0; l < p->layers.size(); l++) {
    int rc = plan_layer_rulebook(p, l, rb_done, hash0_done, st);
    if (rc) return rc;
  }
  V3D_CHECK_HIP(hipStreamSynchronize(st));
  return v3d_backbone_tune(p);
}

extern "C" uint32_t* v3d_backbone_bev_occupancy(v3d_backbone* p) { return p ? p->bev_occ : nullptr; }

extern "C" int32_t* v3d_backbone_occupancy(v3d_backbone* p) { return p ? p->occupancy : nullptr; }
extern "C" int32_t* v3d_backbone_overflow_flags(v3d_backbone* p) { return p ? p->overflow : nullptr; }
extern "C" int v3d_backbone_num_layers(const v3d_backbone* p) { return p ? (int)p->layers.size() : 0; }

struct PlanTrainLayer {
  float* conv_out = nullptr;
  float* stats = nullptr;
  void* wimg_t = nullptr;
  bool wimg_t_ready = false;
  int32_t* nbr_t = nullptr;
};

struct PlanTrain {
  void* arena = nullptr;
  size_t arena_bytes = 0;
  std::vector<PlanTrainLayer> tl;
  float* g[2] = {nullptr, nullptr};
  float* g_conv = nullptr;
  float* w_t = nullptr;
  void* dw_ws = nullptr;
  size_t dw_ws_bytes = 0;
  void* bn_ws = nullptr;
  size_t bn_ws_bytes = 0;
  bool forward_done = false;
};

static void plan_train_free(v3d_backbone* p) {
  if (!p->train) return;
  if (p->train->arena) (void)hipFree(p->train->arena);
  delete p->train;
  p->train = nullptr;
}

static int plan_train_alloc(v3d_backbone* p) {
  if (p->train) return V3D_OK;
  for (auto& L : p->layers) {
    const int c = L.d.cout;
    if (c < 4 || c > V3D_BLOCK || (c & (c - 1))) return V3D_EUNSUPPORTED;
  }
  PlanTrain* t = new (std::nothrow) PlanTrain();
  if (!t) return V3D_EINVAL;
  t->tl.resize(p->layers.size());
  auto carve = [&](V3dArena& ar) {
    size_t max_rows = 1, max_w = 1, max_dw = 1;
    int max_c = 4;
    for (size_t l = 0; l < p->layers.size(); l++) {
      PlanLayer& L = p->layers[l];
      PlanTrainLayer& T = t->tl[l];
      const PlanStage &si = p->stages[L.stage_in], &so = p->stages[L.stage_out];
      T.conv_out = ar.take<float>((size_t)so.cap * L.d.cout);
      T.stats = ar.take<float>((size_t)3 * L.d.cout);
      if (L.d.cin >= 16 && L.d.cin % 16 == 0)
        T.wimg_t = ar.take<char>(v3d_sparse_conv_weight_image_bytes(L.K, L.d.cout, L.d.cin));
      if (!L.d.subm && l > 0) T.nbr_t = ar.take<int32_t>((size_t)L.K * si.cap);
      max_rows = std::max(max_rows, std::max((size_t)so.cap * L.d.cout, (size_t)si.cap * L.d.cin));
      max_w = std::max(max_w, (size_t)L.K * L.d.cin * L.d.cout);
      max_dw = std::max(max_dw, v3d_sparse_conv_bwd_weight_workspace(L.K, L.d.cin, L.d.cout));
      max_c = std::max(max_c, (int)L.d.cout);
    }
    t->g[0] = ar.take<float>(max_rows);
    t->g[1] = ar.take<float>(max_rows);
    t->g_conv = ar.take<float>(max_rows);
    t->w_t = ar.take<float>(max_w);
    t->dw_ws_bytes = max_dw;
// ... 213 lines not shown
```

### vision3d_amd/csrc/sp_device.h

```cpp
#pragma once
#include "v3d_internal.h"
#include "split_prec.h"

template <int PREC, int INS>
__device__ __forceinline__ void split_in(const float (&x)[8], const float s, u32x4& hi, u32x4& lo) {
  if constexpr (INS) {
    hi = u32x4{__float_as_uint(x[0]), __float_as_uint(x[1]), __float_as_uint(x[2]), __float_as_uint(x[3])};
    lo = u32x4{__float_as_uint(x[4]), __float_as_uint(x[5]), __float_as_uint(x[6]), __float_as_uint(x[7])};
  } else {
    split_act<PREC>(x, s, hi, lo);
  }
}

template <int PREC, int COUT>
__device__ __forceinline__ void sp_store_split(unsigned short* __restrict__ out_s, const int row, const int col, const int r, const float v,
                                               const float s) {
  const float pv = __builtin_bit_cast(float, __builtin_amdgcn_update_dpp(0, __builtin_bit_cast(int, v), 0xB1 , 0xF, 0xF, true));
  unsigned h, l;
  split_pair<PREC>((r & 1) ? pv : v, (r & 1) ? v : pv, s, h, l);
  *reinterpret_cast<unsigned*>(out_s + (size_t)row * (2 * COUT) + ((r & 1) ? COUT : 0) + (col & ~1)) = (r & 1) ? l : h;
}

#define SP_STAGE_STRIDE(COUT) ((COUT) * 4 + 16)
#define SP_STAGE_BYTES(COUT) (16 * SP_STAGE_STRIDE(COUT))
template <int COUT, int NT = 64>
__device__ __forceinline__ void sp_stage_flush(const unsigned char* stage, unsigned char* __restrict__ dst_tile, const int nv, const int t) {
  constexpr int ROWB = COUT * 4, CPR = ROWB / 16;
#pragma unroll
  for (int i = 0; i < (16 * CPR + NT - 1) / NT; i++) {
    const int ch = i * NT + t, row = ch / CPR, wc = ch % CPR;
    if (ch < 16 * CPR && row < nv)
      *reinterpret_cast<uint4*>(dst_tile + (size_t)row * ROWB + wc * 16) = *reinterpret_cast<const uint4*>(stage + row * SP_STAGE_STRIDE(COUT) + wc * 16);
  }
}
template <int COUT>
__device__ __forceinline__ void sp_stage_put_f32(unsigned char* stage, const int rowi, const int col, const float v) {
  *reinterpret_cast<float*>(stage + rowi * SP_STAGE_STRIDE(COUT) + col * 4) = v;
}
template <int PREC, int COUT>
__device__ __forceinline__ void sp_stage_put_split(unsigned char* stage, const int rowi, const int col, const int r, const float v, const float s) {
  const float pv = __builtin_bit_cast(float, __builtin_amdgcn_update_dpp(0, __builtin_bit_cast(int, v), 0xB1 , 0xF, 0xF, true));
  unsigned h, l;
  split_pair<PREC>((r & 1) ? pv : v, (r & 1) ? v : pv, s, h, l);
  *reinterpret_cast<unsigned*>(stage + rowi * SP_STAGE_STRIDE(COUT) + ((r & 1) ? COUT * 2 : 0) + (col & ~1) * 2) = (r & 1) ? l : h;
}
template <int COUT, int NB>
__device__ __forceinline__ void sp_tile_store_f32(unsigned char* stage, float* __restrict__ out_tile, const float (&v)[NB][4], const int nv,
                                                  const int lane) {
  const int r = lane & 15, kg = lane >> 4;
#pragma unroll
  for (int j = 0; j < NB; j++)
#pragma unroll
    for (int rr = 0; rr < 4; rr++) sp_stage_put_f32<COUT>(stage, kg * 4 + rr, j * 16 + r, v[j][rr]);
  sp_stage_flush<COUT>(stage, reinterpret_cast<unsigned char*>(out_tile), nv, lane);
}
template <int PREC, int COUT, int NB>
__device__ __forceinline__ void sp_tile_store_split(unsigned char* stage, unsigned short* __restrict__ out_s_tile, const float (&v)[NB][4],
                                                    const float s, const int nv, const int lane) {
  const int r = lane & 15, kg = lane >> 4;
#pragma unroll
  for (int j = 0; j < NB; j++)
#pragma unroll
    for (int rr = 0; rr < 4; rr++) sp_stage_put_split<PREC, COUT>(stage, kg * 4 + rr, j * 16 + r, r, v[j][rr], s);
  sp_stage_flush<COUT>(stage, reinterpret_cast<unsigned char*>(out_s_tile), nv, lane);
}

struct SpScales {
  float s_in, undo, limit;
};
template <int PREC>
__device__ __forceinline__ SpScales sp_scales(const V3dActScale& as, const unsigned short* wimg, size_t img_elems) {
  SpScales r{1.f, 1.f, 3.0e38f};
  if constexpr (PREC == 1) {
    r.s_in = as.in[0];
    r.undo = as.in[1] * (as.w_inv ? *as.w_inv : reinterpret_cast<const float*>(wimg + img_elems)[V3D_WIMG_INV_SCALE]);
    if (as.next) r.limit = as.next[2];
  }
  return r;
}
__device__ __forceinline__ void sp_range_check(const V3dActScale& as, const float vmax, const float limit) {
  if (as.flag && vmax > limit) atomicMax(as.flag, V3D_FLAG_RANGE);
  if (as.seen) v3d_mark_seen(as.seen, vmax, limit * (1.f / (float)(1 << V3D_QUIET_BITS)));
}

static __device__ __attribute__((aligned(256))) const float spr_zero_row[128] = {};

__device__ __forceinline__ void asm_gld16(f32x4& d, const void* p) { asm volatile("global_load_dwordx4 %0, %1, off" : "=v"(d) : "v"(p) : "memory"); }
__device__ __forceinline__ void asm_gld16_16(f32x4& d, const void* p) { asm volatile("global_load_dwordx4 %0, %1, off offset:16" : "=v"(d) : "v"(p) : "memory"); }
__device__ __forceinline__ void asm_gld16_128(f32x4& d, const void* p) { asm volatile("global_load_dwordx4 %0, %1, off offset:128" : "=v"(d) : "v"(p) : "memory"); }
__device__ __forceinline__ void asm_gld16_144(f32x4& d, const void* p) { asm volatile("global_load_dwordx4 %0, %1, off offset:144" : "=v"(d) : "v"(p) : "memory"); }
__device__ __forceinline__ void asm_gld4(int& d, const void* p) { asm volatile("global_load_dword %0, %1, off" : "=v"(d) : "v"(p) : "memory"); }
template <int N> __device__ __forceinline__ void vm_wait_tie(f32x4 (&a)[2]) { asm volatile("s_waitcnt vmcnt(%2)" : "+v"(a[0]), "+v"(a[1]) : "n"(N) : "memory"); }
template <int N> __device__ __forceinline__ void vm_wait_tie(f32x4 (&a)[4]) { asm volatile("s_waitcnt vmcnt(%4)" : "+v"(a[0]), "+v"(a[1]), "+v"(a[2]), "+v"(a[3]) : "n"(N) : "memory"); }
template <int N> __device__ __forceinline__ void vm_wait_tie(f32x4 (&a)[8]) {
  asm volatile("s_waitcnt vmcnt(%8)" : "+v"(a[0]), "+v"(a[1]), "+v"(a[2]), "+v"(a[3]), "+v"(a[4]), "+v"(a[5]), "+v"(a[6]), "+v"(a[7]) : "n"(N) : "memory");
}
template <int N> __device__ __forceinline__ void vm_wait_tie(f32x4 (&a)[1]) { asm volatile("s_waitcnt vmcnt(%1)" : "+v"(a[0]) : "n"(N) : "memory"); }
template <int N> __device__ __forceinline__ void vm_wait_tie_after(f32x4 (&a)[1], f32x4& after) { asm volatile("s_waitcnt vmcnt(%2)" : "+v"(a[0]), "+v"(after) : "n"(N) : "memory"); }
template <int N> __device__ __forceinline__ void vm_wait_tie_after(f32x4 (&a)[2], f32x4& after) { asm volatile("s_waitcnt vmcnt(%3)" : "+v"(a[0]), "+v"(a[1]), "+v"(after) : "n"(N) : "memory"); }
template <int N> __device__ __forceinline__ void vm_wait_tie(int (&a)[1]) { asm volatile("s_waitcnt vmcnt(%1)" : "+v"(a[0]) : "n"(N) : "memory"); }
template <int N> __device__ __forceinline__ void vm_wait_tie(int (&a)[2]) { asm volatile("s_waitcnt vmcnt(%2)" : "+v"(a[0]), "+v"(a[1]) : "n"(N) : "memory"); }
template <int N> __device__ __forceinline__ void vm_wait_tie(int (&a)[3]) { asm volatile("s_waitcnt vmcnt(%3)" : "+v"(a[0]), "+v"(a[1]), "+v"(a[2]) : "n"(N) : "memory"); }

__device__ __forceinline__ void asm_gld16_64(f32x4& d, const void* p) { asm volatile("global_load_dwordx4 %0, %1, off offset:64" : "=v"(d) : "v"(p) : "memory"); }
__device__ __forceinline__ void asm_gld16_192(f32x4& d, const void* p) { asm volatile("global_load_dwordx4 %0, %1, off offset:192" : "=v"(d) : "v"(p) : "memory"); }
__device__ __forceinline__ void asm_dma16(const void* gsrc, unsigned lds_dst) {
  unsigned keep;
  asm volatile("s_mov_b32 %0, m0\n\ts_mov_b32 m0, %2\n\ts_nop 0\n\tglobal_load_lds_dwordx4 %1, off\n\ts_mov_b32 m0, %0"
               : "=&s"(keep) : "v"(gsrc), "s"(lds_dst) : "memory");
}
template <int N> __device__ __forceinline__ void vm_wait() { asm volatile("s_waitcnt vmcnt(%0)" ::"n"(N) : "memory"); }
__device__ __forceinline__ unsigned lds_addr_of(const void* p) { return (unsigned)(unsigned long long)p; }
```

### vision3d_amd/csrc/spconv.hip

```cpp
#include "v3d_internal.h"

#include "sp_device.h"
#include "rb_device.h"

#define SP_RIDER_PROLOGUE(lds)                                                                        \
  if (rider.blocks && (int)blockIdx.x < rider.blocks) {                                               \
    if (threadIdx.x < V3D_BLOCK) rb_rider_run(rider, (int)blockIdx.x, (unsigned char*)(lds));         \
    return;                                                                                           \
  }                                                                                                   \
  const int bid = (int)blockIdx.x - rider.blocks;                                                     \
  [[maybe_unused]] const int nblk = (int)gridDim.x - rider.blocks;



__global__ __launch_bounds__(V3D_BLOCK) void spconv_fwd_scalar(const float* __restrict__ in,
                                                               const float* __restrict__ W,
                                                               const int* __restrict__ nbr,
                                                               const int* __restrict__ n_ptr, int cap, int K, int Cin,
                                                               int Cout, const float* __restrict__ scale,
                                                               const float* __restrict__ shift, int relu,
                                                               float* __restrict__ out) {
  const int n = min(*n_ptr, cap);
  const long long total = (long long)n * Cout;
  for (long long t = (long long)blockIdx.x * V3D_BLOCK + threadIdx.x; t < total; t += (long long)gridDim.x * V3D_BLOCK) {
// ... 750 lines not shown
#pragma unroll
    for (int t = 0; t < T; t++)
#pragma unroll
      for (int j = 0; j < NB; j++) acc[t][j] = f32x4{0.f, 0.f, 0.f, 0.f};

    auto step = [&](int k, int cur) {
      issue_idx(k + 2, src[cur]);
      issue_w(k + 1);
      if constexpr (!STAGE) vm_wait_tie<T + WPT>(araw[cur]);
      vm_wait_tie<T + WPT>(src[cur ^ 1]);
      row_ptrs(k + 1, src[cur ^ 1]);
      if constexpr (STAGE) {
        const int sw = (r >> 3) & 1;
        const unsigned char* sl = aslot + wave * (T * CIN * 64) + (INS ? r * 64 + ((kg ^ sw) * 16) : (kg >> 1) * 1024 + r * 64);
#pragma unroll
        for (int t = 0; t < T; t++)
#pragma unroll
          for (int ki = 0; ki < KI; ki++)
#pragma unroll
            for (int v = 0; v < 2; v++)
              araw[0][(t * KI + ki) * 2 + v] =
                  INS ? *reinterpret_cast<const f32x4*>(sl + t * (CIN * 64) + (v * KI + ki) * 1024)
                      : *reinterpret_cast<const f32x4*>(sl + t * (CIN * 64) + ki * 2048 + ((((kg & 1) * 2 + v) ^ sw) * 16));
      }
      const u32x4* bw = reinterpret_cast<const u32x4*>(wbuf0 + cur * WBYTES) + lane;
      u32x4 bh[KI][NB], bl[KI][NB];
#pragma unroll
      for (int ki = 0; ki < KI; ki++)
#pragma unroll
        for (int j = 0; j < NB; j++) {
          bh[ki][j] = bw[(size_t)((ki * NB + j) * 2) * 64];
          bl[ki][j] = bw[(size_t)((ki * NB + j) * 2 + 1) * 64];
        }
#pragma unroll
      for (int t = 0; t < T; t++) {
#pragma unroll
        for (int ki = 0; ki < KI; ki++) {
          const f32x4 v0 = araw[STAGE ? 0 : cur][(t * KI + ki) * 2], v1 = araw[STAGE ? 0 : cur][(t * KI + ki) * 2 + 1];
          const float x[8] = {v0.x, v0.y, v0.z, v0.w, v1.x, v1.y, v1.z, v1.w};
          u32x4 ah, al;
          split_in<PREC, INS>(x, ss.s_in, ah, al);
#pragma unroll
          for (int j = 0; j < NB; j++) acc[t][j] = split_mfma<PREC>(al, bh[ki][j], acc[t][j]);
#pragma unroll
          for (int j = 0; j < NB; j++) acc[t][j] = split_mfma<PREC>(ah, bl[ki][j], acc[t][j]);
#pragma unroll
          for (int j = 0; j < NB; j++) acc[t][j] = split_mfma<PREC>(ah, bh[ki][j], acc[t][j]);
          __builtin_amdgcn_sched_barrier(0);
          issue_chunk(t, ki, araw[STAGE ? 0 : cur ^ 1]);
          __builtin_amdgcn_sched_barrier(0);
        }
      }
      vm_wait_tie_after<G>(wreg, acc[T - 1][NB - 1]);
      store_w(cur ^ 1);
      __syncthreads();
    };

    issue_idx(0, src[0]);
    issue_idx(1, src[1]);
    issue_w(0);
    vm_wait_tie<T + WPT>(src[0]);
    row_ptrs(0, src[0]);
#pragma unroll
    for (int t = 0; t < T; t++)
#pragma unroll
      for (int ki = 0; ki < KI; ki++) issue_chunk(t, ki, araw[0]);
    vm_wait_tie<G>(wreg);
    store_w(0);
    __syncthreads();
#pragma unroll 1
    for (int k = 0; k < K; k += 2) {
      step(k, 0);
      step(k + 1, 1);
    }
    asm volatile("s_waitcnt vmcnt(0)" ::: "memory");
    if constexpr (STAGE && T * CIN * 64 >= SP_STAGE_BYTES(COUT)) {
      unsigned char* stage = aslot + wave * (T * CIN * 64);
#pragma unroll
      for (int t = 0; t < T; t++) {
        float v[NB][4];
#pragma unroll
        for (int j = 0; j < NB; j++) {
          const int col = j * 16 + r;
          const float sc = (scale ? scale[col] : 1.f) * ss.undo, sh = scale ? shift[col] : 0.f;
#pragma unroll
          for (int rr = 0; rr < 4; rr++) {
            float vv = acc[t][j][rr];
            if (scale || PREC == 1) vv = vv * sc + sh;
            if (relu) vv = fmaxf(vv, 0.f);
            if constexpr (PREC == 1)
              if (row0 + t * 16 + kg * 4 + rr < n) vmax = fmaxf(vmax, fabsf(vv));
            v[j][rr] = vv;
          }
        }
        const int nv = min(16, n - (row0 + t * 16));
        if (nv > 0) {
          if (out) sp_tile_store_f32<COUT, NB>(stage, out + (size_t)(row0 + t * 16) * COUT, v, nv, lane);
          if (out_s) sp_tile_store_split<PREC, COUT, NB>(stage, out_s + (size_t)(row0 + t * 16) * (2 * COUT), v, s_next, nv, lane);
        }
      }
    } else {
#pragma unroll
      for (int t = 0; t < T; t++)
#pragma unroll
        for (int j = 0; j < NB; j++) {
          const int col = j * 16 + r;
          const float sc = (scale ? scale[col] : 1.f) * ss.undo, sh = scale ? shift[col] : 0.f;
#pragma unroll
          for (int rr = 0; rr < 4; rr++) {
            const int row = row0 + t * 16 + kg * 4 + rr;
            if (row < n) {
              float vv = acc[t][j][rr];
              if (scale || PREC == 1) vv = vv * sc + sh;
              if (relu) vv = fmaxf(vv, 0.f);
              if constexpr (PREC == 1) vmax = fmaxf(vmax, fabsf(vv));
              if (out) out[(size_t)row * COUT + col] = vv;
              if (out_s) sp_store_split<PREC, COUT>(out_s, row, col, r, vv, s_next);
            }
          }
        }
    }
  }
  if constexpr (PREC == 1) sp_range_check(as, vmax, ss.limit);
}

template <int CIN, int COUT, int TMAX, int K, int STAGE, int PREC, int INS>
__global__ __launch_bounds__(512) void spconv_fwd_rows_kouter(const float* __restrict__ in,
                                                              const unsigned short* __restrict__ wimg,
                                                              const int* __restrict__ nbr, const int* __restrict__ n_ptr,
                                                              int cap, const float* __restrict__ scale,
                                                              const float* __restrict__ shift, int relu,
                                                              float* __restrict__ out, const V3dActScale as,
                                                              unsigned short* __restrict__ out_s) {
  constexpr int WBYTES = (CIN / 32) * (COUT / 16) * 2 * 1024;
  __shared__ __attribute__((aligned(16))) unsigned char wbuf[2 * WBYTES];
  __shared__ __attribute__((aligned(16))) unsigned char aslot[STAGE ? 8 * TMAX * CIN * 64 : 16];
  const int n = min(*n_ptr, cap);
  if constexpr (TMAX == 3) {
    if (n > 2 * 128 * 256)
      spconv_kouter_body<CIN, COUT, 3, K, STAGE, PREC, INS>(in, wimg, nbr, n, cap, scale, shift, relu, out, wbuf, aslot, as, out_s);
    else
      spconv_kouter_body<CIN, COUT, 2, K, STAGE, PREC, INS>(in, wimg, nbr, n, cap, scale, shift, relu, out, wbuf, aslot, as, out_s);
  } else {
    spconv_kouter_body<CIN, COUT, TMAX, K, STAGE, PREC, INS>(in, wimg, nbr, n, cap, scale, shift, relu, out, wbuf, aslot, as, out_s);
  }
}


template <int CIN, int COUT, int OG, int NBUF, int NMV, int ALOOK, int STAGE, int TILES, int PREC, int INS>
__device__ __forceinline__ void spconv_ring_body(const float* __restrict__ in, const unsigned short* __restrict__ wimg,
                                                 const int* __restrict__ nbr, const int n, int cap, const float* __restrict__ scale,
                                                 const float* __restrict__ shift, int relu, float* __restrict__ out, const int wg_in,
                                                 const SpScales& ss, float& vmax, unsigned short* __restrict__ out_s, const float s_next,
                                                 unsigned char* __restrict__ wb0 ) {
  constexpr int K = 27, ROUNDS = (K + OG - 1) / OG, NCW = TILES * OG;
  constexpr int LOOK = NBUF - 1;
  constexpr int ABUF = ALOOK + 1;
  constexpr int KI = CIN / 32, NB = COUT / 16;
  constexpr int NF = KI * NB * 2;
  constexpr int WBYTES = NF * 1024;
  constexpr int RB = OG * WBYTES;
  constexpr int FPM = OG * NF / NMV;
  constexpr int NSTG = (ROUNDS + 3) / 4;
  static_assert(CIN % 32 == 0 && CIN <= 128 && (OG * NF) % NMV == 0 && (LOOK - 1) * FPM < 64, "shape not covered by the ring kernel");
  static_assert(RB >= TILES * OG * NB * 4 * 64 * 4, "partials must fit one round buffer");
  static_assert(ALOOK >= 1 && ALOOK <= 4 && (ALOOK * KI * 2 <= 8 || ALOOK * KI * 2 == 12 || ALOOK * KI * 2 == 16), "gather look-ahead");
  __shared__ __attribute__((aligned(16))) unsigned char wb1[RB];
  __shared__ __attribute__((aligned(16))) unsigned char wb2[NBUF >= 3 ? RB : 16];
  __shared__ __attribute__((aligned(16))) unsigned char wb3[NBUF == 4 ? RB : 16];
  __shared__ int nbr_all[TILES * K * 16];
  __shared__ __attribute__((aligned(16))) unsigned char aslot[STAGE ? NCW * ALOOK * CIN * 64 : 16];
#define SPR_RING(i) ((i) % NBUF == 0 ? wb0 : ((i) % NBUF == 1 ? wb1 : ((i) % NBUF == 2 ? wb2 : wb3)))
  const int tid = threadIdx.x, lane = tid & 63;
  const int wv = __builtin_amdgcn_readfirstlane(tid >> 6);
  int wg = wg_in;
  {
    const int nwg = (n + 16 * TILES - 1) / (16 * TILES);
    const int qd = nwg / 8, rmd = nwg % 8, xcd = wg % 8, idx = wg / 8;
    wg = (xcd < rmd ? xcd * (qd + 1) : rmd * (qd + 1) + (xcd - rmd) * qd) + idx;
  }

  [[maybe_unused]] const int wave = wv == NCW ? 3 : (wv < 3 ? wv : 99);
  SPR_STAMP(0);
  if (wv >= NCW) {
    typedef const __attribute__((address_space(1))) void* gptr_t;
    typedef __attribute__((address_space(3))) void* lptr_t;
    const int mv = wv - NCW;
    const unsigned char* wsrc = reinterpret_cast<const unsigned char*>(wimg) + (size_t)mv * FPM * 1024 + (size_t)lane * 16;
#define SPR_DMA(R)                                                                                                  \
  {                                                                                                                 \
    const unsigned char* gsrc = wsrc + (size_t)(R) * RB;                                                            \
    _Pragma("unroll") for (int i = 0; i < FPM; i++) {                                                               \
      const bool ok = (R) * OG + (mv * FPM + i) / NF < K;                                                           \
      __builtin_amdgcn_global_load_lds((gptr_t)(gsrc + i * 1024 - (ok ? 0 : WBYTES)),                               \
                                       (lptr_t)(SPR_RING(R) + (mv * FPM + i) * 1024), 16, 0, 0);                    \
    }                                                                                                               \
  }
#pragma unroll
    for (int R = 0; R < LOOK; R++) SPR_DMA(R)
    SPR_STAMP(1);
#pragma unroll
    for (int R = 0; R < ROUNDS; R++) {
      const int younger = (ROUNDS - 1 - R) < (LOOK - 1) ? (ROUNDS - 1 - R) : (LOOK - 1);
      if (younger == 2) asm volatile("s_waitcnt vmcnt(%0)\n\ts_barrier" ::"n"(2 * FPM < 64 ? 2 * FPM : 63) : "memory");
      else if (younger == 1) asm volatile("s_waitcnt vmcnt(%0)\n\ts_barrier" ::"n"(FPM) : "memory");
      else asm volatile("s_waitcnt vmcnt(0)\n\ts_barrier" ::: "memory");
      if (R + LOOK < ROUNDS) SPR_DMA(R + LOOK)
      SPR_STAMP(3 + (R < 9 ? R : 8));
    }
#undef SPR_DMA
    __syncthreads();
    return;
  }

  const int t = wv / OG, g = wv % OG;
  int* nbr_s = nbr_all + t * K * 16;
  const int row0 = (wg * TILES + t) * 16;
  const int r = lane & 15, kg = lane >> 4;
  f32x4 araw[STAGE ? 1 : ABUF][KI * 2];
  f32x4 acc[NB];
#pragma unroll
  for (int j = 0; j < NB; j++) acc[j] = f32x4{0.f, 0.f, 0.f, 0.f};
  const int rsel = STAGE ? (lane >> 2) : r;
  const float* prow = spr_zero_row;
  auto row_ptr = [&](int src_i) {
    const int src = src_i;
    prow = (src >= 0 ? in + (size_t)src * CIN : spr_zero_row) + (STAGE ? ((lane & 3) ^ ((lane >> 5) & 1)) * 4 : (INS ? kg * 4 : kg * 8));
  };
  const unsigned slot0 = STAGE ? __builtin_amdgcn_readfirstlane(lds_addr_of(aslot) + wv * (ALOOK * CIN * 64)) : 0u;
  auto issue_chunk = [&](int ki, int Rr) {
    if constexpr (STAGE) {
      asm_dma16(prow + (ki * 2) * 16, slot0 + (Rr % ALOOK) * (CIN * 64) + (ki * 2) * 1024);
      asm_dma16(prow + (ki * 2 + 1) * 16, slot0 + (Rr % ALOOK) * (CIN * 64) + (ki * 2 + 1) * 1024);
    } else {
      f32x4 (&a)[KI * 2] = araw[Rr % ABUF];
      if constexpr (INS) {
        if (ki == 0) {
          asm_gld16(a[0], prow);
          if constexpr (CIN == 64) asm_gld16_128(a[1], prow);
          else asm_gld16_64(a[1], prow);
        } else if constexpr (KI == 2) {
          asm_gld16_64(a[2], prow);
          asm_gld16_192(a[3], prow);
        }
      } else if (ki == 0) {
        asm_gld16(a[0], prow);
        asm_gld16_16(a[1], prow);
      } else if constexpr (KI == 2) {
        asm_gld16_128(a[2], prow);
        asm_gld16_144(a[3], prow);
      }
    }
  };
  int nsrc = -1;
  {
    const bool live = row0 + r < n;
    int first[ALOOK], stage[NSTG];
#pragma unroll
    for (int i = 0; i < ALOOK; i++) first[i] = (row0 + rsel < n && i * OG + g < K) ? nbr[(size_t)(i * OG + g) * cap + row0 + rsel] : -1;
#pragma unroll
    for (int i = 0; i < NSTG; i++) {
      const int kk = (kg + 4 * i) * OG + g;
      stage[i] = (live && kk < K) ? nbr[(size_t)kk * cap + row0 + r] : -1;
    }
#pragma unroll
    for (int i = 0; i < ALOOK; i++) {
      row_ptr(first[i]);
#pragma unroll
      for (int ki = 0; ki < KI; ki++) issue_chunk(ki, i);
    }
#pragma unroll
    for (int i = 0; i < NSTG; i++)
      if ((kg + 4 * i) * OG + g < K) nbr_s[((kg + 4 * i) * OG + g) * 16 + r] = stage[i];
    if (ALOOK < ROUNDS && ALOOK * OG + g < K) nsrc = nbr_s[(ALOOK * OG + g) * 16 + rsel];
  }
  SPR_STAMP(1);
#pragma unroll
  for (int R = 0; R < ROUNDS; R++) {
    asm volatile("s_waitcnt lgkmcnt(0)\n\ts_barrier" ::: "memory");
    if (R + ALOOK < ROUNDS) row_ptr(nsrc);
    if (R + ALOOK + 1 < ROUNDS) nsrc = ((R + ALOOK + 1) * OG + g < K) ? nbr_s[((R + ALOOK + 1) * OG + g) * 16 + rsel] : -1;
    {
      const int younger = (ROUNDS - 1 - R < ALOOK - 1 ? ROUNDS - 1 - R : ALOOK - 1) * KI * 2;
      if constexpr (STAGE) {
        if (younger == 0) vm_wait<0>();
        else if (younger == 2) vm_wait<2>();
        else if (younger == 4) vm_wait<4>();
        else if (younger == 6) vm_wait<6>();
        else if (younger == 8) vm_wait<8>();
        else vm_wait<12>();
        const int sw = (r >> 3) & 1;
        const unsigned char* sl = aslot + (wv * ALOOK + R % ALOOK) * (CIN * 64) + (INS ? r * 64 + ((kg ^ sw) * 16) : (kg >> 1) * 1024 + r * 64);
#pragma unroll
        for (int ki = 0; ki < KI; ki++)
#pragma unroll
          for (int v = 0; v < 2; v++)
            araw[0][ki * 2 + v] = INS ? *reinterpret_cast<const f32x4*>(sl + (v * KI + ki) * 1024)
                                      : *reinterpret_cast<const f32x4*>(sl + ki * 2048 + ((((kg & 1) * 2 + v) ^ sw) * 16));
      } else {
        f32x4 (&ar)[KI * 2] = araw[R % ABUF];
        if (younger == 0) vm_wait_tie<0>(ar);
        else if (younger == 2) vm_wait_tie<2>(ar);
        else if (younger == 4) vm_wait_tie<4>(ar);
        else if (younger == 6) vm_wait_tie<6>(ar);
        else if (younger == 8) vm_wait_tie<8>(ar);
        else if (younger == 12) vm_wait_tie<12>(ar);
        else vm_wait_tie<16>(ar);
      }
    }
    const u32x4* bw = reinterpret_cast<const u32x4*>(SPR_RING(R) + g * WBYTES) + lane;
    u32x4 ah[KI], al[KI], bh[KI][NB], bl[KI][NB];
#pragma unroll
    for (int ki = 0; ki < KI; ki++)
#pragma unroll
      for (int j = 0; j < NB; j++) {
        bh[ki][j] = bw[(size_t)((ki * NB + j) * 2) * 64];
        bl[ki][j] = bw[(size_t)((ki * NB + j) * 2 + 1) * 64];
      }
#pragma unroll
    for (int ki = 0; ki < KI; ki++) {
      const f32x4 v0 = araw[STAGE ? 0 : R % ABUF][ki * 2], v1 = araw[STAGE ? 0 : R % ABUF][ki * 2 + 1];
      const float x[8] = {v0.x, v0.y, v0.z, v0.w, v1.x, v1.y, v1.z, v1.w};
      split_in<PREC, INS>(x, ss.s_in, ah[ki], al[ki]);
    }
#pragma unroll
    for (int ki = 0; ki < KI; ki++) {
#pragma unroll
      for (int j = 0; j < NB; j++) acc[j] = split_mfma<PREC>(al[ki], bh[ki][j], acc[j]);
#pragma unroll
      for (int j = 0; j < NB; j++) acc[j] = split_mfma<PREC>(ah[ki], bl[ki][j], acc[j]);
#pragma unroll
      for (int j = 0; j < NB; j++) acc[j] = split_mfma<PREC>(ah[ki], bh[ki][j], acc[j]);
      if (R + ALOOK < ROUNDS) {
        __builtin_amdgcn_sched_barrier(0);
        issue_chunk(ki, R + ALOOK);
        __builtin_amdgcn_sched_barrier(0);
      }
    }
#if SPR_TIMELINE
    __builtin_amdgcn_sched_barrier(0);
    SPR_STAMP(3 + (R < 9 ? R : 8));
#endif
  }
  float* part = reinterpret_cast<float*>((ROUNDS - 1) % NBUF != 0 ? wb0 : wb1) + t * (OG * NB * 4 * 64);
#pragma unroll
  for (int j = 0; j < NB; j++)
#pragma unroll
    for (int rr = 0; rr < 4; rr++) part[((g * NB + j) * 4 + rr) * 64 + lane] = acc[j][rr];
  SPR_STAMP(12);
  __syncthreads();
  SPR_STAMP(13);
  for (int it = g; it < NB * 4; it += OG) {
    const int j = it >> 2, rr = it & 3;
    const int col = j * 16 + r, row = row0 + kg * 4 + rr;
    float v = part[((0 * NB + j) * 4 + rr) * 64 + lane];
#pragma unroll
    for (int w = 1; w < OG; w++) v += part[((w * NB + j) * 4 + rr) * 64 + lane];
    if (row < n) {
      if (scale) v = v * (scale[col] * ss.undo) + shift[col];
      else if constexpr (PREC == 1) v = v * ss.undo;
      if (relu) v = fmaxf(v, 0.f);
      if constexpr (PREC == 1) vmax = fmaxf(vmax, fabsf(v));
      if (out) out[(size_t)row * COUT + col] = v;
      if (out_s) sp_store_split<PREC, COUT>(out_s, row, col, r, v, s_next);
    }
  }
  SPR_STAMP(14);
#undef SPR_RING
}

template <int CIN, int COUT, int OG, int NBUF, int NMV, int ALOOK, int STAGE, int TILES, int PREC, int INS>
__global__ __launch_bounds__((TILES * OG + NMV) * 64) void spconv_fwd_rows_ring(const float* __restrict__ in,
                                                                          const unsigned short* __restrict__ wimg,
                                                                          const int* __restrict__ nbr,
                                                                          const int* __restrict__ n_ptr, int cap,
                                                                          const float* __restrict__ scale,
                                                                          const float* __restrict__ shift, int relu,
                                                                          float* __restrict__ out, const V3dActScale as,
                                                                          unsigned short* __restrict__ out_s, const RbScanJob rider) {
  constexpr int RB0 = OG * (CIN / 32) * (COUT / 16) * 2 * 1024;
  static_assert(RB0 >= RB_SCAN_LDS, "a rider's scratch fits round buffer 0");
  __shared__ __attribute__((aligned(16))) unsigned char wb0[RB0];
  constexpr bool HOST = !(CIN == 64 && COUT == 64);
  int bid = (int)blockIdx.x, nblk = (int)gridDim.x;
  if constexpr (HOST) {
    if (rider.blocks && bid < rider.blocks) {
      if (threadIdx.x < V3D_BLOCK) rb_rider_run(rider, bid, wb0);
      return;
    }
    bid -= rider.blocks;
    nblk -= rider.blocks;
  }
  const int n = min(*n_ptr, cap);
  const int nwg = (n + 16 * TILES - 1) / (16 * TILES);
  const SpScales ss = sp_scales<PREC>(as, wimg, (size_t)27 * (CIN / 32) * (COUT / 16) * 2 * 512);
  const float s_next = (PREC == 1 && out_s) ? as.next[0] : 1.f;
  float vmax = 0.f;
  for (int g = bid; g < nwg; g += nblk) {
    spconv_ring_body<CIN, COUT, OG, NBUF, NMV, ALOOK, STAGE, TILES, PREC, INS>(in, wimg, nbr, n, cap, scale, shift, relu, out, g, ss, vmax,
                                                                              out_s, s_next, wb0);
    __syncthreads();
  }
  if constexpr (PREC == 1) sp_range_check(as, vmax, ss.limit);
}

struct SpLaunch {
  int prec;
  V3dActScale as;
  const void* in_split;
  unsigned short* out_split;
  const RbScanJob* rider;
  bool* rider_taken;
};

static RbScanJob sp_ring_rider(const SpLaunch& sl, int max_blocks) {
  if (!sl.rider || max_blocks < 1 || sl.rider->blocks > max_blocks) return RbScanJob{};
  return *sl.rider;
}

template <int CIN, int COUT, int OG, int NBUF, int NMV, int ALOOK, int STAGE, int TILES, int PREC, int INS>
static int launch_rows_ring_p(const float* in, const void* wimg, const int* nbr, const int* n_ptr, int cap,
                              const float* scale, const float* shift, int relu, float* out, hipStream_t st, const SpLaunch& sl) {
  static V3dPerDeviceInt cache;
  int* slots = cache.slot();
  if (!*slots) {
    int dev = 0, n_cu = 0, per_cu = 0;
    V3D_CHECK_HIP(hipGetDevice(&dev));
    V3D_CHECK_HIP(hipDeviceGetAttribute(&n_cu, hipDeviceAttributeMultiprocessorCount, dev));
    V3D_CHECK_HIP(hipOccupancyMaxActiveBlocksPerMultiprocessor(&per_cu, spconv_fwd_rows_ring<CIN, COUT, OG, NBUF, NMV, ALOOK, STAGE, TILES, PREC, INS>,
                                                               (TILES * OG + NMV) * 64, 0));
    *slots = std::max(8, per_cu * n_cu / 8 * 8);
  }
  const RbScanJob r = sp_ring_rider(sl, CIN == 64 && COUT == 64 ? 0 : 512);
  const int grid = std::min(v3d_ceil_div(cap, 16 * TILES), std::max(*slots - r.blocks, 8));
  hipLaunchKernelGGL((spconv_fwd_rows_ring<CIN, COUT, OG, NBUF, NMV, ALOOK, STAGE, TILES, PREC, INS>), dim3(grid + r.blocks),
                     dim3((TILES * OG + NMV) * 64), 0, st, INS ? (const float*)sl.in_split : in, (const unsigned short*)wimg, nbr, n_ptr, cap,
                     scale, shift, relu, out, sl.as, sl.out_split, r);
  if (sl.rider_taken) *sl.rider_taken = r.blocks > 0;
  V3D_CHECK_LAUNCH();
  return V3D_OK;
}
template <int CIN, int COUT, int OG, int NBUF, int NMV, int ALOOK = 2, int STAGE = 0, int TILES = 2>
static int launch_rows_ring(const float* in, const void* wimg, const int* nbr, const int* n_ptr, int cap,
                            const float* scale, const float* shift, int relu, float* out, hipStream_t st, const SpLaunch& sl) {
#define V3D_RING(P, I) launch_rows_ring_p<CIN, COUT, OG, NBUF, NMV, ALOOK, STAGE, TILES, P, I>(in, wimg, nbr, n_ptr, cap, scale, shift, relu, out, st, sl)
  if (sl.prec == V3D_PREC_F16S) return sl.in_split ? V3D_RING(1, 1) : V3D_RING(1, 0);
  return sl.in_split ? V3D_RING(0, 1) : V3D_RING(0, 0);
#undef V3D_RING
}

template <int CIN, int COUT, int PREC, int INS>
static void launch_rows_big(const float* in, const void* wimg, const int* nbr, const int* n_ptr, int cap, int K,
                            const float* scale, const float* shift, int relu, float* out, hipStream_t st, const SpLaunch& sl) {
  constexpr int NF = ((CIN + 31) / 32) * (COUT / 16) * 2;
  const size_t lds = std::max((size_t)2 * NF * 64 * 16 + (size_t)K * 64 * 4, (size_t)4 * SP_STAGE_BYTES(COUT));
  hipLaunchKernelGGL((spconv_fwd_rows_big<CIN, COUT, PREC, INS>), dim3(v3d_ceil_div(cap, 64)), dim3(V3D_BLOCK), lds, st,
                     INS ? (const float*)sl.in_split : in, (const unsigned short*)wimg, nbr, n_ptr, cap, K, scale, shift, relu, out, sl.as,
                     sl.out_split);
}

template <int CIN, int COUT, int T, int STAGE, int PREC, int INS>
static void launch_rows_kouter(const float* in, const void* wimg, const int* nbr, const int* n_ptr, int cap,
                               const float* scale, const float* shift, int relu, float* out, hipStream_t st, const SpLaunch& sl) {
  const int passes = v3d_ceil_div(cap, 16 * (T == 3 ? 2 : T) * 8);
  const int grid = passes >= 256 ? 256 : ((passes + 7) / 8) * 8;
  hipLaunchKernelGGL((spconv_fwd_rows_kouter<CIN, COUT, T, 27, STAGE, PREC, INS>), dim3(grid), dim3(512), 0, st,
                     INS ? (const float*)sl.in_split : in, (const unsigned short*)wimg, nbr, n_ptr, cap, scale, shift, relu, out, sl.as,
                     sl.out_split);
}

#define V3D_BIG_ROWS 32768
#define V3D_RING_ROWS 16384
template <int CIN, int COUT, int PREC, int INS>
static int launch_rows(const float* in, const void* wimg, const int* nbr, const int* n_ptr, int cap, int K,
                       const float* scale, const float* shift, int relu, float* out, int rows_hint, hipStream_t st,
                       const V3dDensifyOut* densify, int tiles_min, const SpLaunch& sl) {
  const int force = densify ? 1 : (rows_hint < 0 ? -rows_hint : 0);
  if constexpr (CIN >= 32 && CIN <= 64 && COUT >= 32 && COUT <= 64) {
    if (K == 27 && (force == 6 || force == 7 || force == 8 || (force == 0 && CIN == 64 && COUT == 64 && rows_hint >= V3D_BIG_ROWS))) {
      if (force == 7) launch_rows_kouter<CIN, COUT, 2, 0, PREC, INS>(in, wimg, nbr, n_ptr, cap, scale, shift, relu, out, st, sl);
      else if (force == 8) launch_rows_kouter<CIN, COUT, 2, 1, PREC, INS>(in, wimg, nbr, n_ptr, cap, scale, shift, relu, out, st, sl);
      else launch_rows_kouter<CIN, COUT, 3, 1, PREC, INS>(in, wimg, nbr, n_ptr, cap, scale, shift, relu, out, st, sl);
      V3D_CHECK_LAUNCH();
      return V3D_OK;
    }
    if (force == 5 || (force == 0 && rows_hint >= V3D_BIG_ROWS)) {
      launch_rows_big<CIN, COUT, PREC, INS>(in, wimg, nbr, n_ptr, cap, K, scale, shift, relu, out, st, sl);
      V3D_CHECK_LAUNCH();
      return V3D_OK;
    }
    if (K == 27 && (force == 10 || force == 16 || (force >= 12 && force <= 14) || (force == 0 && rows_hint <= V3D_RING_ROWS))) {
      if constexpr (CIN == 64 && COUT == 64) {
        if (force != 16) {
          const long long want = force ? 0 : (long long)rows_hint + rows_hint / 10;
          int tiles = force == 12 ? 2 : force == 13 ? 3 : force == 14 ? 4 : (want <= 32 * 256 ? 2 : want <= 48 * 256 ? 3 : 4);
          if (!force && tiles < tiles_min) tiles = tiles_min > 4 ? 4 : tiles_min;
          if (tiles == 2) return launch_rows_ring<CIN, COUT, 3, 2, 4, 1, 1, 2>(in, wimg, nbr, n_ptr, cap, scale, shift, relu, out, st, sl);
          if (tiles == 3) return launch_rows_ring<CIN, COUT, 3, 2, 4, 1, 1, 3>(in, wimg, nbr, n_ptr, cap, scale, shift, relu, out, st, sl);
          return launch_rows_ring<CIN, COUT, 3, 2, 4, 1, 1, 4>(in, wimg, nbr, n_ptr, cap, scale, shift, relu, out, st, sl);
        }
      }
      if (force != 16 && CIN == 32 && COUT == 32) return launch_rows_ring<CIN, COUT, 3, 2, 2, 2, 1>(in, wimg, nbr, n_ptr, cap, scale, shift, relu, out, st, sl);
      return launch_rows_ring<CIN, COUT, 3, 3, 2>(in, wimg, nbr, n_ptr, cap, scale, shift, relu, out, st, sl);
    }
  }
  const size_t lds = std::max((size_t)4 * (COUT / 16) * 4 * 64 * 4 + (size_t)K * 16 * 4 + 2 * SP_STAGE_BYTES(COUT),
                              (size_t)RB_SCAN_LDS);
  const RbScanJob r = sl.rider ? *sl.rider : RbScanJob{};
  hipLaunchKernelGGL((spconv_fwd_rows<CIN, COUT, PREC, INS>), dim3(v3d_ceil_div(cap, 16) + r.blocks), dim3(V3D_BLOCK), lds, st,
                     INS ? (const float*)sl.in_split : in, (const unsigned short*)wimg, nbr, n_ptr, cap, K, scale, shift, relu, out,
                     densify ? *densify : V3dDensifyOut{}, sl.as, sl.out_split, r);
  if (sl.rider_taken) *sl.rider_taken = r.blocks > 0;
  V3D_CHECK_LAUNCH();
  return V3D_OK;
}

extern "C" int v3d_sparse_conv_fwd_packed(const float* in, const void* weight_image, const int32_t* nbr,
                                           const int32_t* n_out, int cap_out, int K, int Cin, int Cout, const float* scale,
                                           const float* shift, int relu, float* out, int rows_hint, int prec,
                                           const float* act_in, const float* act_next, int32_t* range_flag,
                                           const void* in_split, void* out_split, v3d_stream_t stream) {
  const V3dActScale as{act_in, act_next, range_flag, nullptr};
  return v3d_i_sparse_conv_fwd_packed(in ? in : (const float*)in_split, weight_image, nbr, n_out, cap_out, K, Cin, Cout, scale, shift,
                                      relu, out, rows_hint, (hipStream_t)stream, nullptr, 2, prec, &as, in_split, out_split);
}

template <int PREC>
__global__ __launch_bounds__(256) void rows_split_kernel(const float* __restrict__ rows, const int* __restrict__ n_ptr, int cap, int C,
                                                         const float* __restrict__ entry, unsigned short* __restrict__ out) {
  const long long total = (long long)(n_ptr ? min(*n_ptr, cap) : cap) * C;
  const float s = PREC == 1 ? entry[0] : 1.f;
  for (long long t = (long long)blockIdx.x * 256 + threadIdx.x; t < total; t += (long long)gridDim.x * 256) {
    const long long row = t / C;
    const int c = (int)(t - row * C);
    unsigned short h, l;
    split_one<PREC>(rows[t], s, h, l);
    out[row * 2 * C + c] = h;
    out[row * 2 * C + C + c] = l;
  }
}

extern "C" int v3d_sparse_rows_split(const float* rows, const int32_t* n_rows, int cap, int C, int prec, const float* act_entry,
                                     void* out_split, v3d_stream_t stream) {
  if (!rows || !out_split || cap < 1 || C < 8 || C % 8) return V3D_EINVAL;
  if (prec == V3D_PREC_F16S ? !act_entry : prec != V3D_PREC_BF16X3) return V3D_EINVAL;
  const int blocks = (int)std::min<long long>(((long long)cap * C + 255) / 256, 4096);
  if (prec == V3D_PREC_F16S)
    hipLaunchKernelGGL(rows_split_kernel<1>, dim3(blocks), dim3(256), 0, (hipStream_t)stream, rows, n_rows, cap, C, act_entry, (unsigned short*)out_split);
  else
    hipLaunchKernelGGL(rows_split_kernel<0>, dim3(blocks), dim3(256), 0, (hipStream_t)stream, rows, n_rows, cap, C, nullptr, (unsigned short*)out_split);
  V3D_CHECK_LAUNCH();
  return V3D_OK;
}

bool v3d_i_sparse_conv_packed_supported(int Cin, int Cout) {
  static const int shapes[][2] = {{4, 16}, {16, 16}, {16, 32}, {32, 32}, {32, 64}, {64, 64}, {4, 32}, {32, 16}, {64, 32}, {64, 128}, {128, 128}};
  for (const auto& s : shapes)
    if (s[0] == Cin && s[1] == Cout) return true;
  return false;
}

int v3d_i_sparse_conv_fwd_packed(const float* in, const void* weight_image, const int32_t* nbr, const int32_t* n_out,
                                 int cap_out, int K, int Cin, int Cout, const float* scale, const float* shift, int relu,
                                 float* out, int rows_hint, hipStream_t st, const V3dDensifyOut* densify, int ring_tiles_min,
                                 int prec, const V3dActScale* act, const void* in_split, void* out_split, const RbScanJob* rider,
                                 bool* rider_taken) {
  if (rider_taken) *rider_taken = false;
  if (!in || !weight_image || !nbr || !n_out || (!out && !out_split) || cap_out < 1 || K < 1) return V3D_EINVAL;
  if ((scale == nullptr) != (shift == nullptr)) return V3D_EINVAL;
  if (!out && densify) return V3D_EINVAL;
  if (prec != V3D_PREC_BF16X3 && prec != V3D_PREC_F16S) return V3D_EINVAL;
  if (prec == V3D_PREC_F16S && (!act || !act->in || ((densify || out_split) && !act->next))) return V3D_EINVAL;
  if (in_split && Cin % 8) return V3D_EINVAL;
  SpLaunch sl;
  sl.prec = prec;
  sl.as = (prec == V3D_PREC_F16S) ? *act : V3dActScale{nullptr, nullptr, nullptr, nullptr};
  sl.in_split = in_split;
  sl.out_split = (unsigned short*)out_split;
  sl.rider = rider;
  sl.rider_taken = rider_taken;
#define V3D_GO(ci, co, P, I) \
  return launch_rows<ci, co, P, I>(in, weight_image, nbr, n_out, cap_out, K, scale, shift, relu, out, rows_hint, st, densify, ring_tiles_min, sl)
#define V3D_TRY(ci, co)                                    \
  if (Cin == ci && Cout == co) {                           \
    if constexpr ((ci) % 8 == 0) {                         \
      if (prec == V3D_PREC_F16S && in_split) V3D_GO(ci, co, 1, 1); \
      if (prec == V3D_PREC_BF16X3 && in_split) V3D_GO(ci, co, 0, 1); \
    }                                                      \
    if (prec == V3D_PREC_F16S) V3D_GO(ci, co, 1, 0);       \
    V3D_GO(ci, co, 0, 0);                                  \
  }
  V3D_TRY(4, 16)
  V3D_TRY(16, 16)
  V3D_TRY(16, 32)
  V3D_TRY(32, 32)
  V3D_TRY(32, 64)
  V3D_TRY(64, 64)
  V3D_TRY(4, 32)
  V3D_TRY(32, 16)
  V3D_TRY(64, 32)
  V3D_TRY(64, 128)
  V3D_TRY(128, 128)
#undef V3D_TRY
#undef V3D_GO
  return V3D_EUNSUPPORTED;
}

extern "C" int v3d_sparse_conv_fwd(const float* in, const float* weight, const int32_t* nbr, const int32_t* n_out,
                                   int cap_out, int K, int Cin, int Cout, const float* scale, const float* shift,
                                   int relu, float* out, int algo, v3d_stream_t stream) {
  return v3d_i_sparse_conv_fwd_exact(in, weight, nbr, n_out, cap_out, K, Cin, Cout, scale, shift, relu, out, algo, (hipStream_t)stream,
                                     nullptr, nullptr, nullptr, nullptr, nullptr);
}

int v3d_i_sparse_conv_fwd_exact(const float* in, const float* weight, const int32_t* nbr, const int32_t* n_out, int cap_out, int K,
                                int Cin, int Cout, const float* scale, const float* shift, int relu, float* out, int algo,
                                hipStream_t st, const float* next_entry, int32_t* range_flag, unsigned* seen, const RbScanJob* rider,
                                bool* rider_taken) {
  if (rider_taken) *rider_taken = false;
  if (!in || !weight || !nbr || !n_out || !out || cap_out < 1 || K < 1 || Cin < 1 || Cout < 1) return V3D_EINVAL;
  if ((scale == nullptr) != (shift == nullptr)) return V3D_EINVAL;
  if (algo != 0 && algo != 1 && algo != 3) return V3D_EINVAL;
  if (algo == 0 || algo == 3) {
    int rc = V3D_EUNSUPPORTED;
#define V3D_TRY(ci, co) \
  if (Cin == ci && Cout == co) rc = launch_wave<ci, co>(in, weight, nbr, n_out, cap_out, K, scale, shift, relu, out, st, next_entry, range_flag, seen, rider, rider_taken);
    V3D_TRY(4, 16)
    V3D_TRY(16, 16)
    V3D_TRY(16, 32)
    V3D_TRY(32, 32)
    V3D_TRY(32, 64)
    V3D_TRY(64, 64)
    V3D_TRY(4, 32)
    V3D_TRY(32, 16)
    V3D_TRY(64, 32)
    V3D_TRY(64, 128)
    V3D_TRY(128, 128)
#undef V3D_TRY
    if (rc != V3D_EUNSUPPORTED || algo == 3) return rc;
  }
  const long long total = (long long)cap_out * Cout;
  const int blocks = (int)((total + V3D_BLOCK - 1) / V3D_BLOCK);
  hipLaunchKernelGGL(spconv_fwd_scalar, dim3(blocks > 8192 ? 8192 : blocks), dim3(V3D_BLOCK), 0, st, in, weight, nbr,
                       n_out, cap_out, K, Cin, Cout, scale, shift, relu, out);
  V3D_CHECK_LAUNCH();
  return V3D_OK;
}

#define BW_MAX_SPLITS 64
#define BW_Q 128

__host__ __device__ static inline int bw_rows_per_block(int n) {
  const int r = ((n + BW_MAX_SPLITS - 1) / BW_MAX_SPLITS + 255) & ~255;
  return r < 256 ? 256 : r;
}

template <int TI, int TJ>
__global__ __launch_bounds__(V3D_BLOCK) void spconv_bwd_weight_tiles(const float* __restrict__ X,
                                                                     const float* __restrict__ dY,
                                                                     const int* __restrict__ nbr,
                                                                     const int* __restrict__ n_ptr, int cap, int Cin,
                                                                     int Cout, int groups_j,
                                                                     float* __restrict__ partial ) {
  __shared__ int q_src[4][BW_Q];
  __shared__ int q_out[4][BW_Q];
  __shared__ float red[TI * TJ * 256];
  const int n = min(*n_ptr, cap);
  const int rows_per_block = bw_rows_per_block(n);
  const int slab = blockIdx.x, k = blockIdx.y, K = gridDim.y;
  const int lo = slab * rows_per_block;
  if (lo >= n) return;
  const int hi = min(n, lo + rows_per_block);
  const int ci_base = (blockIdx.z / groups_j) * TI * 16, co_base = (blockIdx.z % groups_j) * TJ * 16;
  const int lane = threadIdx.x & 63, wave = threadIdx.x >> 6;
  const int r = lane & 15, p = lane >> 4;
  const int rows_per_wave = rows_per_block >> 2;
  const int wlo = lo + wave * rows_per_wave, whi = min(hi, wlo + rows_per_wave);
  const int* __restrict__ nk = nbr + (size_t)k * cap;
  int* qs = q_src[wave];
  int* qo = q_out[wave];

  f32x4 acc[TI][TJ];
#pragma unroll
  for (int t = 0; t < TI; t++)
#pragma unroll
    for (int u = 0; u < TJ; u++) acc[t][u] = f32x4{0.f, 0.f, 0.f, 0.f};

  auto consume = [&](int base, int valid) {
    float a[4][TI], b[4][TJ];
#pragma unroll
    for (int s4 = 0; s4 < 4; s4++) {
      const int e = 4 * s4 + p;
      const bool ok = e < valid;
      const int src = ok ? qs[base + e] : 0, o = ok ? qo[base + e] : 0;
#pragma unroll
      for (int t = 0; t < TI; t++) {
        const int ci = ci_base + 16 * t + r;
        a[s4][t] = (ok && ci < Cin) ? X[(size_t)src * Cin + ci] : 0.f;
      }
#pragma unroll
      for (int u = 0; u < TJ; u++) {
        const int co = co_base + 16 * u + r;
        b[s4][u] = (ok && co < Cout) ? dY[(size_t)o * Cout + co] : 0.f;
      }
    }
#pragma unroll
    for (int s4 = 0; s4 < 4; s4++)
#pragma unroll
      for (int t = 0; t < TI; t++)
#pragma unroll
        for (int u = 0; u < TJ; u++) acc[t][u] = __builtin_amdgcn_mfma_f32_16x16x4f32(a[s4][t], b[s4][u], acc[t][u], 0, 0, 0);
  };

  int cnt = 0;
  int src_next = (wlo < whi && wlo + lane < whi) ? nk[wlo + lane] : -1;
  for (int o0 = wlo; o0 < whi; o0 += 64) {
    const int src = src_next;
    const int o = o0 + lane;
    src_next = (o + 64 < whi) ? nk[o + 64] : -1;
    const unsigned long long live = __ballot(src >= 0);
    if (src >= 0) {
      const int pos = cnt + __popcll(live & ((1ull << lane) - 1ull));
      qs[pos] = src;
      qo[pos] = o;
    }
    cnt += __popcll(live);
    int g = 0;
    for (; cnt - g >= 16; g += 16) consume(g, 16);
    if (g) {
      const int rem = cnt - g;
      int ms = 0, mo = 0;
      if (lane < rem) { ms = qs[g + lane]; mo = qo[g + lane]; }
      if (lane < rem) { qs[lane] = ms; qo[lane] = mo; }
// ... 102 lines not shown
```

### vision3d_amd/csrc/v3d_internal.h

```cpp
#pragma once
#include "v3d_common.h"
#ifdef V3D_ABLATE
#include <cstdlib>
#include <cstring>
static inline bool v3d_ablate(char c) { const char* e = getenv("V3D_ABL"); return e && strchr(e, c); }
#else
static inline bool v3d_ablate(char) { return false; }
#endif

struct RbScanJob;
struct RbStep;
struct V3dRbHash {
  v3d_key_t* keys;
  int* vals;
  unsigned hcap;
};

int v3d_i_voxelize(const float* points, int n_points, int C, const int32_t* frame_offsets_host, int B,
                   const float* voxel_size_host, const float* bounds_host, int max_pts, int max_voxels, float* voxels,
                   int32_t* coords, int32_t* occupancy, float* mean, int32_t* n_voxels, void* workspace,
                   size_t workspace_bytes, int clear_tables, const V3dRbHash* site_hash ,
                   const int32_t* site_shape , hipStream_t st);
int v3d_i_hash_build(const int32_t* coords, const int32_t* n, int cap, const int32_t* shape, V3dRbHash h, int clear,
                     hipStream_t st);
struct V3dRbCandNext {
  const int32_t* coords_in;
  const int32_t* n_in;
  int cap_in;
  const int32_t* shape;
  const int32_t *ksize, *stride, *padding;
  V3dRbHash out;
  unsigned* first_ticket;
  int* cand_slot;
  int32_t* overflow;
  int32_t* overflow_any;
};
int v3d_i_subm_nbr(const int32_t* coords, const int32_t* n, int cap, const int32_t* shape, const int32_t* ksize,
                   V3dRbHash h, int32_t* nbr, hipStream_t st, const V3dRbCandNext* next = nullptr);
int v3d_i_sparse_rulebook(const int32_t* coords_in, const int32_t* n_in, int cap_in, const int32_t* shape,
                          const int32_t* ksize, const int32_t* stride, const int32_t* padding, int32_t* coords_out,
                          int32_t* n_out, int cap_out, int32_t* nbr, int32_t* overflow, V3dRbHash out,
                          unsigned* first_ticket, int* cand_slot, int* chunk_counts ,
                          int32_t* out_shape, int clear,
                          const int32_t* next_subm_ksize ,
                          int32_t* next_subm_nbr, hipStream_t st,
                          int32_t* overflow_any = nullptr ,
                          int candidates_done = 0 ,
                          const V3dRbCandNext* next = nullptr ,
                          int init_columns = 0 );

int v3d_i_sparse_rulebook_steps(const int32_t* coords_in, const int32_t* n_in, int cap_in, const int32_t* shape,
                                const int32_t* ksize, const int32_t* stride, const int32_t* padding, int32_t* coords_out,
                                int32_t* n_out, int cap_out, int32_t* nbr, int32_t* overflow, V3dRbHash out,
                                unsigned* first_ticket, int* cand_slot, int* chunk_counts, const int32_t* next_subm_ksize,
                                int32_t* next_subm_nbr, int32_t* overflow_any, const V3dRbCandNext* next, int init_columns,
                                RbStep* scan, RbStep* fill);
int v3d_i_rb_step_launch(const RbStep& s, hipStream_t st);

int v3d_i_nms_sorted(const void* prep_sorted, const int* order, int N, float iou_threshold, int64_t* keep, int32_t* n_keep,
                     unsigned long long* mask, unsigned long long* remv, hipStream_t st);

int v3d_i_nms_mask_sorted(const void* prep_sorted, int N, float iou_threshold, unsigned long long* mask, hipStream_t st);

#define V3D_FLAG_CAPACITY 1
#define V3D_FLAG_RANGE 2
#define V3D_FLAG_QUIET 3
#define V3D_QUIET_BITS 12
struct V3dActScale {
  const float* in;
  const float* next;
  int32_t* flag;
  const float* w_inv;
  unsigned* seen;
};

struct V3dDensifyOut {
  const int32_t* coords;
  int D, H, W;
  void *hi, *lo;
  uint32_t* occ;
  int32_t *pix, *pix_n;
};
int v3d_i_sparse_conv_fwd_packed(const float* in, const void* weight_image, const int32_t* nbr, const int32_t* n_out,
                                 int cap_out, int K, int Cin, int Cout, const float* scale, const float* shift, int relu,
                                 float* out, int rows_hint, hipStream_t st, const V3dDensifyOut* densify = nullptr ,
                                 int ring_tiles_min = 2 ,
                                 int prec = V3D_PREC_BF16X3 ,
                                 const V3dActScale* act = nullptr ,
                                 const void* in_split = nullptr ,
                                 void* out_split = nullptr ,
                                 const RbScanJob* rider = nullptr ,
                                 bool* rider_taken = nullptr );

struct V3dBrickTables {
  uint16_t* lidx;
  int32_t* ulist;
  int32_t* ucnt;
  uint32_t* tmask;
};
int v3d_i_sparse_brick_plan(const int32_t* nbr, const int32_t* n_in, int cap_in, const int32_t* n_out, int cap_out, int K,
                            const V3dBrickTables& t, hipStream_t st);
int v3d_i_sparse_conv_fwd_brick(const void* in_split, const void* weight_image, const int32_t* nbr, const V3dBrickTables& bt,
                                const int32_t* n_out, int cap, int K, int Cin, int Cout, const float* scale, const float* shift, int relu,
                                float* out, int prec, const V3dActScale* act, void* out_split, hipStream_t st);

bool v3d_i_sparse_conv_packed_supported(int Cin, int Cout);

int v3d_i_sparse_conv_fwd_exact(const float* in, const float* weight, const int32_t* nbr, const int32_t* n_out, int cap_out, int K,
                                int Cin, int Cout, const float* scale, const float* shift, int relu, float* out, int algo,
                                hipStream_t st, const float* next_entry, int32_t* range_flag, unsigned* seen = nullptr,
                                const RbScanJob* rider = nullptr, bool* rider_taken = nullptr );

#define V3D_PACK_JOBS_MAX 32
struct V3dPackJobs {
  const float* w[V3D_PACK_JOBS_MAX];
  void* img[V3D_PACK_JOBS_MAX];
  int K[V3D_PACK_JOBS_MAX], cin[V3D_PACK_JOBS_MAX], cout[V3D_PACK_JOBS_MAX], mode[V3D_PACK_JOBS_MAX];
};
int v3d_i_sparse_conv_pack_batch(const V3dPackJobs& jobs, int n, hipStream_t stream);

int v3d_i_sparse_bn_relu_fwd(const float* x, int n, const int32_t* n_dev, int C, const float* gamma, const float* beta, float eps,
                             int relu, float* y, float* save_mean, float* save_invstd, float* var_unbiased, float* running_mean,
                             float* running_var, float momentum, int64_t* num_batches_tracked, void* workspace,
                             size_t workspace_bytes, hipStream_t st);
int v3d_i_sparse_bn_relu_bwd(const float* x, const float* dy, int n, const int32_t* n_dev, int C, const float* gamma,
                             const float* beta, const float* save_mean, const float* save_invstd, int relu, float* dx,
                             float* dgamma, float* dbeta, void* workspace, size_t workspace_bytes, hipStream_t st);

int v3d_i_densify_nhwc_split(const float* feat, const int32_t* coords, const int32_t* n, int cap, int B, int C,
                             const int32_t* spatial_shape_host, void* out_hi, void* out_lo, uint32_t* occ_inv, hipStream_t st,
                             int32_t* written_pix = nullptr ,
                             int32_t* written_n = nullptr, int prec = V3D_PREC_BF16X3,
                             const float* act_entry = nullptr ,
                             int32_t* range_flag = nullptr ,
                             unsigned* seen = nullptr );
int v3d_i_bev_clear_pixels(const int32_t* pix, const int32_t* n, int cap, int channels, void* hi, void* lo, hipStream_t st);
```

### vision3d_amd/runtime.py

```python
import ctypes as C
import os

import numpy as np
import torch
from torch import nn

from . import _lib as L
from .spconv.conv import _SparseConvBase
from .spconv.modules import fold_batchnorm


class RangeOverflow(RuntimeError):
    """f16s arithmetic: a tensor of the last frame exceeded the range its scale entry was calibrated for (the frame's results
    are not valid).  Recalibrate on that frame (BackbonePlan.recalibrate / DenseHeadPlan.recalibrate) and run it again --
    Second.inference and the captured-graph runners do."""


class RangeUnderflow(RangeOverflow):
    """f16s arithmetic, the other direction: a tensor of the last frame stayed 2^12 or more below the limit its scale entry was
    calibrated for (summary word 3, csrc/second_plan.hip plan_quiet_check_kernel) -- the frame's small entries no longer keep the
    22 bits of the fp32-class arithmetic.  Handled like RangeOverflow (which it subclasses, so every recalibrate-and-rerun path
    catches it): the entries are re-derived from this frame, downward, and the frame is run again."""


CALIB_HEADROOM_BITS = 5


def scale_entry_from_max(amax, headroom_bits, out=None):
    amax = amax.detach().to(torch.float32).reshape(())
    _, e = torch.frexp(amax)
    ok = torch.isfinite(amax) & (amax > 0)
    expo = torch.where(ok, (14 - int(headroom_bits)) - e, torch.zeros_like(e)).clamp(-125, 125)
    s = torch.ldexp(torch.ones((), dtype=torch.float32, device=amax.device), expo)
    entry = torch.stack((s, 1.0 / s, 32768.0 / s, amax))
    if out is not None:
        out.copy_(entry)
        return out
    return entry


class PlanCache(dict):

    def __deepcopy__(self, memo):
        return PlanCache()


def flatten_sparse_layers(module):
    mods = []

    def walk(m):
        if isinstance(m, _SparseConvBase) or not isinstance(m, nn.Sequential):
            mods.append(m)
        else:
            for c in m.children():
                walk(c)
    walk(module)
    out, i = [], 0
    while i < len(mods):
        m = mods[i]
        if not isinstance(m, _SparseConvBase):
            raise NotImplementedError(f"BackbonePlan: unsupported module {type(m).__name__} outside a conv-BN-ReLU group")
        bn = mods[i + 1] if i + 1 < len(mods) and isinstance(mods[i + 1], nn.BatchNorm1d) else None
        j = i + (2 if bn is not None else 1)
        relu = j < len(mods) and isinstance(mods[j], nn.ReLU)
        out.append((m, bn, relu))
        i = j + (1 if relu else 0)
    return out


class BackbonePlan(object):

    def __init__(self, cnn, cfg, max_batch=1, max_points=None, growth=2.0, device=None, conv_algo=0, precision="bf16x3"):
        self.device = torch.device("cuda", torch.cuda.current_device()) if device is None else torch.device(device)
        self.cfg = cfg
        self.layers = flatten_sparse_layers(cnn.blocks)
        self.grid_shape = [int(s) for s in cnn.grid_shape]
        self.max_batch = int(max_batch)
        self.max_points = int(max_points if max_points is not None else 16384 * max_batch)
        keys = {}
        descs = (L.LayerDesc * len(self.layers))()
        for d, (conv, bn, relu) in zip(descs, self.layers):
            d.subm, d.cin, d.cout = int(conv.subm), conv.in_channels, conv.out_channels
            d.ksize[:] = conv.kernel_size
            d.stride[:] = conv.stride
            d.padding[:] = conv.padding
            d.key = -1 if conv.indice_key is None else keys.setdefault(conv.indice_key, len(keys))
            d.relu = int(relu)
        c = L.BackboneConfig()
        c.voxel_size[:] = [float(v) for v in cfg.VOXEL_SIZE]
        c.bounds[:] = [float(v) for v in cfg.GRID_BOUNDS]
        c.max_pts, c.max_voxels, c.point_channels = cfg.MAX_OCCUPANCY, cfg.MAX_VOXELS, cfg.C_IN
        c.grid_shape[:] = self.grid_shape
        c.max_batch, c.max_points, c.n_layers, c.growth = self.max_batch, self.max_points, len(self.layers), float(growth)
        c.conv_algo = int(conv_algo)
        self._handle = C.c_void_p()
        with L.device_guard(self.device):
            L.check(L.lib().v3d_backbone_create(C.byref(c), descs, C.byref(self._handle)), "backbone_create")
        self.precision = None
        self.set_precision(precision)
        if os.environ.get("V3D_PRESPLIT", "1") == "0":
            self.set_presplit(False)
        self.out_channels = self.layers[-1][0].out_channels
        shape = list(self.grid_shape)
        for conv, _, _ in self.layers:
            if not conv.subm:
                shape = [(shape[j] + 2 * conv.padding[j] - conv.kernel_size[j]) // conv.stride[j] + 1 for j in range(3)]
        self.out_shape = shape
        self._stamp = None
        self._keep = []

    def __del__(self):
        h = getattr(self, "_handle", None)
        if h is not None and h.value:
            try:
                L.lib().v3d_backbone_destroy(h)
            except Exception:
                pass
            self._handle = None

    def set_precision(self, precision):
        if precision not in L.PRECISIONS:
            raise ValueError(f"precision must be one of {sorted(L.PRECISIONS)}")
        if self.precision is not None and L.PRECISIONS[precision] == L.PRECISIONS[self.precision]:
            return
        L.check(L.lib().v3d_backbone_set_precision(self._handle, L.PRECISIONS[precision]), "backbone_set_precision")
        self.precision = precision
        self._stamp = None
        self._calib = "need" if self.f16s else "off"

    @property
    def f16s(self):
        return L.PRECISIONS[self.precision] == L.PREC_F16S

    def set_presplit(self, on=True):
        L.check(L.lib().v3d_backbone_set_presplit(self._handle, int(bool(on))), "backbone_set_presplit")

    def act_scales(self):
        ptr = L.lib().v3d_backbone_act_scales(self._handle)
        return _view(ptr, (len(self.layers) + 1, 4), torch.float32, self.device)

    def bev_entry(self):
        return self.act_scales()[len(self.layers)] if self.f16s else None

    def recalibrate(self):
        if self.f16s:
            self._calib = "need"

    def copy_calibration(self, other):
        if self.f16s and other.f16s and len(other.layers) == len(self.layers):
            self.act_scales().copy_(other.act_scales())
            self._calib = other._calib
            if other._calib == "done":
                L.check(L.lib().v3d_backbone_set_calibrating(self._handle, 0), "backbone_set_calibrating")
                self.calibration_generation = self.__dict__.get("calibration_generation", 0) + 1

    def _param_stamp(self):
        st = []
        for conv, bn, _ in self.layers:
            ts = [conv.weight, conv.bias] + ([bn.running_mean, bn.running_var, bn.weight, bn.bias] if bn is not None else [])
            st.append(tuple((t.data_ptr(), t._version) for t in ts if t is not None))
        return tuple(st)

    def sync_weights(self):
        stamp = self._param_stamp()
        if stamp == self._stamp:
            return
        if self.f16s and self._stamp is not None and self._calib == "done" and not torch.cuda.is_current_stream_capturing():
            self._calib = "need"
        lib = L.lib()
        keep = []
        with L.device_guard(self.device), torch.no_grad():
            for i, (conv, bn, _) in enumerate(self.layers):
                w = conv.weight.detach().to(self.device, torch.float32).reshape(-1, conv.in_channels, conv.out_channels).contiguous()
                scale = shift = None
                if bn is not None:
                    if bn.training:
                        raise RuntimeError("BackbonePlan runs eval-mode BatchNorm only (call model.eval())")
                    scale, shift = fold_batchnorm(bn)
                if conv.bias is not None:
                    b = conv.bias.detach()
                    shift = b if shift is None else shift + b * scale
                    scale = torch.ones_like(b) if scale is None else scale
                if scale is not None:
                    scale, shift = scale.to(self.device).contiguous(), shift.to(self.device).contiguous()
                keep += [w, scale, shift]
                L.check(lib.v3d_backbone_set_layer(self._handle, i, L.ptr(w), L.ptr(scale), L.ptr(shift), L.stream_ptr()),
                        "backbone_set_layer")
        self._keep = keep
        self._stamp = stamp

    def weights_changed(self):
        return self._stamp is not None and self._param_stamp() != self._stamp

    def forward(self, points, frame_offsets, out=None):
        self.sync_weights()
        pts = L.as_f32("backbone", points)
        b = len(frame_offsets) - 1
        d, h, w = self.out_shape
        if out is None:
            out = torch.empty((b, self.out_channels * d, h, w), dtype=torch.float32, device=pts.device)
        with L.device_guard(pts.device):
            L.check(L.lib().v3d_backbone_forward(self._handle, L.ptr(pts), pts.shape[0], L.host_i32(frame_offsets), b,
                                                 L.ptr(out), None, None, L.stream_ptr()), "backbone_forward")
        if self._maybe_tune():
            return self.forward(points, frame_offsets, out)
        return out

    def tune(self):
        torch.cuda.synchronize(self.device)
        L.check(L.lib().v3d_backbone_tune(self._handle), "backbone_tune")
        self._tuned = True

    def _maybe_tune(self):
        if torch.cuda.is_current_stream_capturing():
            return False
        again = False
        if not self.__dict__.get("_tuned"):
            self.tune()
            if not self.__dict__.get("allow_overflow"):
                self.check_overflow(ignore_range=True)
            again = True
        if self._calib == "need":
            L.check(L.lib().v3d_backbone_set_calibrating(self._handle, 1), "backbone_set_calibrating")
            self._calib = "exact"
            return True
        if self._calib == "exact":
            L.check(L.lib().v3d_backbone_calibrate(self._handle, int(self.__dict__.get("calib_headroom", CALIB_HEADROOM_BITS)),
                                                   L.stream_ptr()), "backbone_calibrate")
            L.check(L.lib().v3d_backbone_set_calibrating(self._handle, 0), "backbone_set_calibrating")
            self._calib = "done"
            self.calibration_generation = self.__dict__.get("calibration_generation", 0) + 1
            return True
        return again

    def set_throughput_mode(self, on=True):
        L.check(L.lib().v3d_backbone_set_throughput_mode(self._handle, int(bool(on))), "backbone_set_throughput_mode")

    def own_planes(self, batch_size):
        hi, lo = C.c_void_p(), C.c_void_p()
        L.check(L.lib().v3d_backbone_bev_planes(self._handle, C.byref(hi), C.byref(lo)), "backbone_bev_planes")
        d, h, w = self.out_shape
        full = (self.max_batch, h, w, self.out_channels * d)
        return self._tag(_view(hi.value, full, torch.int16, self.device)[:int(batch_size)],
                         _view(lo.value, full, torch.int16, self.device)[:int(batch_size)])

    def _tag(self, hi, lo):
        tag_planes(hi, self.bev_entry(), self.overflow_any() if self.f16s else None)
        return hi, lo

    def forward_split(self, points, frame_offsets, persistent=False):
        self.sync_weights()
        pts = L.as_f32("backbone", points)
        b = len(frame_offsets) - 1
        d, h, w = self.out_shape
        hi, lo = self.own_planes(b) if persistent else self._tag(*split_planes_like(b, h, w, self.out_channels * d, pts.device))
        with L.device_guard(pts.device):
            L.check(L.lib().v3d_backbone_forward(self._handle, L.ptr(pts), pts.shape[0], L.host_i32(frame_offsets), b, 0,
                                                  L.ptr(hi), L.ptr(lo), L.stream_ptr()), "backbone_forward2")
        if self._maybe_tune():
            return self.forward_split(points, frame_offsets, persistent)
        return hi, lo

    def forward_reuse_split(self, batch_size, device):
        d, h, w = self.out_shape
        hi, lo = self._tag(*split_planes_like(int(batch_size), h, w, self.out_channels * d, device))
        with L.device_guard(device):
            L.check(L.lib().v3d_backbone_forward_reuse(self._handle, int(batch_size), 0, L.ptr(hi), L.ptr(lo), L.stream_ptr()),
                    "backbone_forward_reuse")
        return hi, lo

    def forward_voxels_split(self, voxel_mean, coordinates, batch_size):
        self.sync_weights()
        mean = L.as_f32("backbone", voxel_mean)
        coords = L.as_i32("backbone", coordinates)
        m = mean.shape[0]
        if coords.shape != (m, 4) or mean.shape[1] != self.cfg.C_IN:
            raise RuntimeError("backbone: voxel_mean (M, C_IN) / coordinates (M, 4) expected")
        d, h, w = self.out_shape
        hi, lo = self._tag(*split_planes_like(int(batch_size), h, w, self.out_channels * d, mean.device))
        with L.device_guard(mean.device):
            L.check(L.lib().v3d_backbone_forward_voxels(self._handle, L.ptr(mean), L.ptr(coords), m, int(batch_size), 0,
                                                        L.ptr(hi), L.ptr(lo), L.stream_ptr()), "backbone_forward_voxels")
        if self._maybe_tune():
            return self.forward_voxels_split(voxel_mean, coordinates, batch_size)
        return hi, lo

    def forward_voxels(self, voxel_mean, coordinates, batch_size, out=None):
        self.sync_weights()
# ... 505 lines not shown
```

Before: 4811.

## Group submanifold conv rows by neighbor-presence mask to skip empty offset rounds

Adds a per-chunk bitonic sort that orders output rows by their 27-bit neighbor-presence mask, so 16-row tiles in 64->64 submanifold convs share which kernel offsets are empty. The ring conv kernel reads rows through this permutation, builds a per-wave live mask of offset rounds via ballot, and skips the gather and MFMA work for rounds with no live neighbors. The sort kernel can ride on an earlier conv launch as extra blocks to hide its own launch. The trade-off is extra sort work, an indirection on row indices with less contiguous output writes, and added control flow in the inner loop.

```diff
diff --git a/include/vision3d_hip.h b/include/vision3d_hip.h
--- a/include/vision3d_hip.h
+++ b/include/vision3d_hip.h
@@ -117,6 +117,12 @@
                                int32_t* range_flag, const void* in_split, void* out_split, v3d_stream_t stream);
 int v3d_sparse_rows_split(const float* rows, const int32_t* n_rows, int cap, int C, int prec, const float* act_entry,
                           void* out_split, v3d_stream_t stream);
+int v3d_sparse_row_order(const int32_t* nbr, const int32_t* n_out, int cap_out, int K, int32_t* order, v3d_stream_t stream);
+int v3d_sparse_conv_fwd_ordered(const float* in, const void* weight_image, const int32_t* nbr, const int32_t* n_out,
+                                int cap_out, int K, int Cin, int Cout, const float* scale, const float* shift, int relu,
+                                float* out, int rows_hint, int prec, const float* act_in, const float* act_next,
+                                int32_t* range_flag, const void* in_split, void* out_split, const int32_t* order,
+                                v3d_stream_t stream);
 size_t v3d_sparse_brick_table_bytes(int cap, int K, size_t* lidx_bytes, size_t* ulist_bytes, size_t* ucnt_bytes,
                                     size_t* tmask_bytes);
 int v3d_sparse_brick_plan(const int32_t* nbr, const int32_t* n_rows, int cap, int K, uint16_t* lidx, int32_t* ulist,
@@ -230,6 +236,8 @@
 int v3d_backbone_set_precision(v3d_backbone* plan, int prec);
 int v3d_backbone_precision(const v3d_backbone* plan);
 int v3d_backbone_set_presplit(v3d_backbone* plan, int on);
+int v3d_backbone_set_row_grouping(v3d_backbone* plan, int on);
+int v3d_backbone_row_order(v3d_backbone* plan, int layer, int32_t** order, int32_t** nbr, int* cap, int* K);
 float* v3d_backbone_act_scales(v3d_backbone* plan);
 int v3d_backbone_set_calibrating(v3d_backbone* plan, int on);
 int v3d_backbone_calibrate(v3d_backbone* plan, int headroom_bits, v3d_stream_t stream);
diff --git a/vision3d_amd/_lib.py b/vision3d_amd/_lib.py
--- a/vision3d_amd/_lib.py
+++ b/vision3d_amd/_lib.py
@@ -106,6 +106,10 @@
     "v3d_backbone_set_precision": (_i, [_vp, _i]),
     "v3d_backbone_precision": (_i, [_vp]),
     "v3d_backbone_set_presplit": (_i, [_vp, _i]),
+    "v3d_backbone_set_row_grouping": (_i, [_vp, _i]),
+    "v3d_backbone_row_order": (_i, [_vp, _i, _vp, _vp, _vp, _vp]),
+    "v3d_sparse_row_order": (_i, [_vp, _vp, _i, _i, _vp, _vp]),
+    "v3d_sparse_conv_fwd_ordered": (_i, [_vp, _vp, _vp, _vp, _i, _i, _i, _i, _vp, _vp, _i, _vp, _i, _i, _vp, _vp, _vp, _vp, _vp, _vp, _vp]),
     "v3d_backbone_act_scales": (_vp, [_vp]),
     "v3d_backbone_set_calibrating": (_i, [_vp, _i]),
     "v3d_backbone_calibrate": (_i, [_vp, _i, _vp]),
diff --git a/vision3d_amd/csrc/rb_device.h b/vision3d_amd/csrc/rb_device.h
--- a/vision3d_amd/csrc/rb_device.h
+++ b/vision3d_amd/csrc/rb_device.h
@@ -319,6 +319,51 @@
 }
 
 
+#define RB_ORDER_LDS (8 * V3D_ORDER_CHUNK)
+static_assert((V3D_ORDER_CHUNK & (V3D_ORDER_CHUNK - 1)) == 0 && V3D_ORDER_CHUNK <= 1024 && V3D_ORDER_CHUNK >= 2 * V3D_BLOCK, "chunk: a power of two, 10 index bits");
+__device__ __forceinline__ void rb_row_order_body(const int* __restrict__ nbr, const int* __restrict__ n_ptr, int cap, int K,
+                                                  int* __restrict__ order, const int b, unsigned char* __restrict__ lds_raw) {
+  unsigned long long* key = reinterpret_cast<unsigned long long*>(lds_raw);
+  const int tid = threadIdx.x, base = b * V3D_ORDER_CHUNK;
+  const int in_chunk = min(cap - base, V3D_ORDER_CHUNK);
+  const int live = min(min(*n_ptr, cap) - base, in_chunk);
+  for (int i = max(live, 0) + tid; i < in_chunk; i += V3D_BLOCK) order[base + i] = base + i;
+  if (live <= 0) return;
+  int ns = 2;
+  while (ns < live) ns <<= 1;
+  for (int i = tid; i < ns; i += V3D_BLOCK) {
+    unsigned long long kk = ~0ull;
+    if (i < live) {
+      unsigned m = 0u;
+      for (int k = 0; k < K; k++) m |= (nbr[(size_t)k * cap + base + i] >= 0 ? 1u : 0u) << k;
+      kk = ((unsigned long long)m << 10) | (unsigned)i;
+    }
+    key[i] = kk;
+  }
+  __syncthreads();
+  for (int k = 2; k <= ns; k <<= 1)
+    for (int j = k >> 1; j > 0; j >>= 1) {
+      for (int q = tid; q < (ns >> 1); q += V3D_BLOCK) {
+        const int lo = ((q & ~(j - 1)) << 1) | (q & (j - 1)), hi = lo | j;
+        const unsigned long long x = key[lo], y = key[hi];
+        if ((x > y) == ((lo & k) == 0)) {
+          key[lo] = y;
+          key[hi] = x;
+        }
+      }
+      __syncthreads();
+    }
+  for (int i = tid; i < live; i += V3D_BLOCK) order[base + i] = base + (int)(key[i] & 1023ull);
+}
+
+struct RbOrderJob {
+  int blocks;
+  const int* nbr;
+  const int* n_ptr;
+  int cap, K;
+  int* order;
+};
+
 struct RbScanJob {
   int blocks;
   int cap_in, cap_out;
diff --git a/vision3d_amd/csrc/rulebook.hip b/vision3d_amd/csrc/rulebook.hip
--- a/vision3d_amd/csrc/rulebook.hip
+++ b/vision3d_amd/csrc/rulebook.hip
@@ -109,6 +109,19 @@
   const int subm_blocks = rb_subm_blocks(cap, g);
   hipLaunchKernelGGL(rb_subm_nbr_kernel, dim3(subm_blocks + job.blocks), dim3(V3D_BLOCK), 0, st,
                      (const int4*)coords, n, cap, g, hh, h.vals, nbr, subm_blocks, job);
+  V3D_CHECK_LAUNCH();
+  return V3D_OK;
+}
+
+__global__ __launch_bounds__(V3D_BLOCK) void rb_row_order_kernel(const int* __restrict__ nbr, const int* __restrict__ n_ptr, int cap, int K,
+                                                                 int* __restrict__ order) {
+  __shared__ __attribute__((aligned(16))) unsigned char lds[RB_ORDER_LDS];
+  rb_row_order_body(nbr, n_ptr, cap, K, order, blockIdx.x, lds);
+}
+int v3d_i_row_order(const int32_t* nbr, const int32_t* n, int cap, int K, int32_t* order, hipStream_t st) {
+  if (!nbr || !n || !order || cap < 1 || K < 1) return V3D_EINVAL;
+  if (K > 32) return V3D_EUNSUPPORTED;
+  hipLaunchKernelGGL(rb_row_order_kernel, dim3(v3d_ceil_div(cap, V3D_ORDER_CHUNK)), dim3(V3D_BLOCK), 0, st, nbr, n, cap, K, order);
   V3D_CHECK_LAUNCH();
   return V3D_OK;
 }
diff --git a/vision3d_amd/csrc/second_plan.hip b/vision3d_amd/csrc/second_plan.hip
--- a/vision3d_amd/csrc/second_plan.hip
+++ b/vision3d_amd/csrc/second_plan.hip
@@ -41,6 +41,8 @@
   std::vector<PlanStage> stages;
   std::vector<int32_t*> nbr;
   std::vector<int> nbr_cap;
+  std::vector<int32_t*> order;
+  bool row_grouping = true;
   void* arena = nullptr;
   size_t arena_bytes = 0;
   void* vox_ws = nullptr;
@@ -180,6 +182,9 @@
       if (!L.d.subm) L.chunk_counts = ar.take<int>((size_t)v3d_ceil_div((long long)p->stages[L.stage_in].cap * conv_fan(L.d), V3D_SCAN_CHUNK) + 2);
     p->ff_bytes = (size_t)((ar.base + ar.off) - p->ff_begin);
     for (size_t i = 0; i < p->nbr.size(); i++) p->nbr[i] = ar.take<int32_t>((size_t)rbK[i] * p->nbr_cap[i]);
+    p->order.assign(p->nbr.size(), nullptr);
+    for (auto& L : p->layers)
+      if (L.d.subm && L.K == 27 && L.d.cin == 64 && L.d.cout == 64 && !p->order[L.rulebook]) p->order[L.rulebook] = ar.take<int32_t>(p->nbr_cap[L.rulebook]);
     p->occupancy = ar.take<int32_t>(p->stages[0].cap);
     p->mean = ar.take<float>((size_t)p->stages[0].cap * cfg->point_channels);
     for (auto& st : p->stages) {
@@ -370,6 +375,22 @@
   return V3D_OK;
 }
 
+extern "C" int v3d_backbone_set_row_grouping(v3d_backbone* p, int on) {
+  if (!p) return V3D_EINVAL;
+  p->row_grouping = on != 0;
+  return V3D_OK;
+}
+
+extern "C" int v3d_backbone_row_order(v3d_backbone* p, int layer, int32_t** order, int32_t** nbr, int* cap, int* K) {
+  if (!p || layer < 0 || layer >= (int)p->layers.size()) return V3D_EINVAL;
+  const PlanLayer& L = p->layers[layer];
+  if (order) *order = p->row_grouping ? p->order[L.rulebook] : nullptr;
+  if (nbr) *nbr = p->nbr[L.rulebook];
+  if (cap) *cap = p->nbr_cap[L.rulebook];
+  if (K) *K = L.K;
+  return V3D_OK;
+}
+
 extern "C" float* v3d_backbone_act_scales(v3d_backbone* p) { return p ? p->act_tab : nullptr; }
 
 extern "C" int v3d_backbone_set_calibrating(v3d_backbone* p, int on) {
@@ -528,12 +549,15 @@
                            const float* scale, const float* shift, int relu, float* out, hipStream_t st,
                            const V3dDensifyOut* densify = nullptr, bool* densified = nullptr, bool inference = false,
                            const void** feat_split = nullptr ,
-                           const RbScanJob* rider = nullptr, bool* rider_taken = nullptr ) {
+                           const RbScanJob* rider = nullptr, bool* rider_taken = nullptr ,
+                           const int32_t* order = nullptr ,
+                           const RbOrderJob* order_job = nullptr, bool* order_job_taken = nullptr ) {
   const v3d_backbone_config& c = p->cfg;
   PlanStage& so = p->stages[L.stage_out];
   int rc = V3D_EUNSUPPORTED;
   if (densified) *densified = false;
   if (rider_taken) *rider_taken = false;
+  if (order_job_taken) *order_job_taken = false;
   if (v3d_ablate('c') || (v3d_ablate('r') && L.d.cin == 64 && L.d.cout == 64 && L.K == 27)) return V3D_OK;
   const bool exact_pass = inference && p->calibrating;
   if (!exact_pass && (c.conv_algo == 4 || (c.conv_algo == 0 && L.d.cin >= 16))) {
@@ -551,7 +575,8 @@
     void* out_s = (feat_split && p->presplit && next_packed && (prec == V3D_PREC_F16S || !p->fp32_rows)) ? L.out_s : nullptr;
     if (out_s && !p->fp32_rows && !densify && v3d_i_sparse_conv_packed_supported(L.d.cin, L.d.cout)) out = nullptr;
     rc = v3d_i_sparse_conv_fwd_packed(feat, wimg, p->nbr[L.rulebook], so.n_dev, so.cap, L.K, L.d.cin, L.d.cout, scale, shift,
-                                      relu, out, L.rows_hint, st, densify, p->ring_tiles_min, prec, &as, in_s, out_s, rider, rider_taken);
+                                      relu, out, L.rows_hint, st, densify, p->ring_tiles_min, prec, &as, in_s, out_s, rider, rider_taken,
+                                      order, order_job, order_job_taken);
     if (rc == V3D_OK && densify && densified) *densified = true;
     if (feat_split) *feat_split = rc == V3D_OK ? out_s : nullptr;
   } else if (feat_split) {
@@ -577,6 +602,7 @@
   std::vector<char> cand_done(p->layers.size(), 0);
   bool densified = false;
   PlanRbQueue rbq;
+  std::vector<char> order_done(p->nbr.size(), 0);
   const bool riders = !reuse_rulebooks && p->rb_riders;
   if (riders) {
     rbq.rb_step.assign(p->nbr.size(), -1);
@@ -609,9 +635,36 @@
       const PlanStage& sl = p->stages.back();
       dn = V3dDensifyOut{sl.coords, sl.shape[0], sl.shape[1], sl.shape[2], p->bev_hi, p->bev_lo, p->bev_occ, p->bev_pix, p->bev_pix_n};
     }
+    auto wants_order = [&](const PlanLayer& M) {
+      return p->row_grouping && M.d.subm && p->order[M.rulebook] && !p->calibrating && (p->cfg.conv_algo == 4 || p->cfg.conv_algo == 0) &&
+             v3d_i_sparse_conv_takes_order(M.d.cin, M.d.cout, M.K, M.rows_hint) && !v3d_ablate('c') && !v3d_ablate('r');
+    };
+    const int32_t* order = nullptr;
+    if (wants_order(L)) {
+      order = p->order[L.rulebook];
+      if (!order_done[L.rulebook]) {
+        rc = v3d_i_row_order(p->nbr[L.rulebook], p->stages[L.stage_out].n_dev, p->nbr_cap[L.rulebook], L.K, p->order[L.rulebook], st);
+        if (rc) return rc;
+        order_done[L.rulebook] = 1;
+      }
+    }
+    RbOrderJob oj{};
+    int oj_rb = -1;
+    if (reuse_rulebooks || riders)
+      for (size_t m = l + 1; m < p->layers.size() && oj_rb < 0; m++) {
+        const PlanLayer& M = p->layers[m];
+        if (!wants_order(M) || order_done[M.rulebook]) continue;
+        if (!reuse_rulebooks && rbq.rb_step[M.rulebook] >= (int)rbq.launched) continue;
+        oj_rb = M.rulebook;
+        oj = RbOrderJob{v3d_ceil_div(p->nbr_cap[oj_rb], V3D_ORDER_CHUNK), p->nbr[oj_rb], p->stages[M.stage_out].n_dev, p->nbr_cap[oj_rb], M.K,
+                        p->order[oj_rb]};
+      }
+    bool oj_taken = false;
     rc = plan_layer_conv(p, L, feat, L.wimg, L.weight, L.has_affine ? L.scale : nullptr, L.has_affine ? L.shift : nullptr,
-                         L.d.relu, L.out, st, want_dn ? &dn : nullptr, &densified, true, &feat_split, rider, &rider_taken);
-    if (rc) return rc;
+                         L.d.relu, L.out, st, want_dn ? &dn : nullptr, &densified, true, &feat_split, rider, &rider_taken, order,
+                         oj_rb >= 0 ? &oj : nullptr, &oj_taken);
+    if (rc) return rc;
+    if (oj_taken) order_done[oj_rb] = 1;
     if (rider_taken) rbq.launched++;
     feat = L.out;
   }
diff --git a/vision3d_amd/csrc/sp_device.h b/vision3d_amd/csrc/sp_device.h
--- a/vision3d_amd/csrc/sp_device.h
+++ b/vision3d_amd/csrc/sp_device.h
@@ -9,6 +9,7 @@
     lo = u32x4{__float_as_uint(x[4]), __float_as_uint(x[5]), __float_as_uint(x[6]), __float_as_uint(x[7])};
   } else {
     split_act<PREC>(x, s, hi, lo);
+    if constexpr (PREC == 1) asm("s_nop 1" : "+v"(hi), "+v"(lo));
   }
 }
 
diff --git a/vision3d_amd/csrc/spconv.hip b/vision3d_amd/csrc/spconv.hip
--- a/vision3d_amd/csrc/spconv.hip
+++ b/vision3d_amd/csrc/spconv.hip
@@ -926,7 +926,8 @@
                                                  const int* __restrict__ nbr, const int n, int cap, const float* __restrict__ scale,
                                                  const float* __restrict__ shift, int relu, float* __restrict__ out, const int wg_in,
                                                  const SpScales& ss, float& vmax, unsigned short* __restrict__ out_s, const float s_next,
-                                                 unsigned char* __restrict__ wb0 ) {
+                                                 unsigned char* __restrict__ wb0 ,
+                                                 const int* __restrict__ order ) {
   constexpr int K = 27, ROUNDS = (K + OG - 1) / OG, NCW = TILES * OG;
   constexpr int LOOK = NBUF - 1;
   constexpr int ABUF = ALOOK + 1;
@@ -991,6 +992,10 @@
   int* nbr_s = nbr_all + t * K * 16;
   const int row0 = (wg * TILES + t) * 16;
   const int r = lane & 15, kg = lane >> 4;
+  constexpr bool ORD = CIN == 64 && COUT == 64;
+  int myrow = row0 + r;
+  if constexpr (ORD)
+    if (order && row0 + r < n) myrow = order[row0 + r];
   f32x4 araw[STAGE ? 1 : ABUF][KI * 2];
   f32x4 acc[NB];
 #pragma unroll
@@ -1027,16 +1032,31 @@
     }
   };
   int nsrc = -1;
+  unsigned livemask = 0u;
+  constexpr bool SKIP_GATHER = STAGE && ALOOK == 1;
   {
     const bool live = row0 + r < n;
     int first[ALOOK], stage[NSTG];
-#pragma unroll
-    for (int i = 0; i < ALOOK; i++) first[i] = (row0 + rsel < n && i * OG + g < K) ? nbr[(size_t)(i * OG + g) * cap + row0 + rsel] : -1;
+    const int selrow = (ORD && STAGE) ? __shfl(myrow, rsel) : (STAGE ? row0 + rsel : myrow);
+#pragma unroll
+    for (int i = 0; i < ALOOK; i++) first[i] = (row0 + rsel < n && i * OG + g < K) ? nbr[(size_t)(i * OG + g) * cap + selrow] : -1;
 #pragma unroll
     for (int i = 0; i < NSTG; i++) {
       const int kk = (kg + 4 * i) * OG + g;
-      stage[i] = (live && kk < K) ? nbr[(size_t)kk * cap + row0 + r] : -1;
-    }
+      stage[i] = (live && kk < K) ? nbr[(size_t)kk * cap + myrow] : -1;
+    }
+#pragma unroll
+    for (int i = 0; i < NSTG; i++) {
+      const unsigned long long b = __ballot(stage[i] >= 0);
+#pragma unroll
+      for (int q = 0; q < 4; q++)
+        if (q + 4 * i < ROUNDS && ((b >> (16 * q)) & 0xFFFFull)) livemask |= 1u << (q + 4 * i);
+    }
+#if defined(SPR_EXP_NO_SKIP)
+    livemask = (1u << ROUNDS) - 1u;
+#elif !defined(SPR_EXP_SKIP_ALL_SHAPES)
+    if constexpr (!ORD) livemask = (1u << ROUNDS) - 1u;
+#endif
 #pragma unroll
     for (int i = 0; i < ALOOK; i++) {
       row_ptr(first[i]);
@@ -1054,6 +1074,8 @@
     asm volatile("s_waitcnt lgkmcnt(0)\n\ts_barrier" ::: "memory");
     if (R + ALOOK < ROUNDS) row_ptr(nsrc);
     if (R + ALOOK + 1 < ROUNDS) nsrc = ((R + ALOOK + 1) * OG + g < K) ? nbr_s[((R + ALOOK + 1) * OG + g) * 16 + rsel] : -1;
+    const bool lv = (livemask >> R) & 1u;
+    const bool lvn = R + ALOOK < ROUNDS && (!SKIP_GATHER || ((livemask >> (R + ALOOK)) & 1u));
     {
       const int younger = (ROUNDS - 1 - R < ALOOK - 1 ? ROUNDS - 1 - R : ALOOK - 1) * KI * 2;
       if constexpr (STAGE) {
@@ -1063,6 +1085,7 @@
         else if (younger == 6) vm_wait<6>();
         else if (younger == 8) vm_wait<8>();
         else vm_wait<12>();
+        if (lv) {
         const int sw = (r >> 3) & 1;
         const unsigned char* sl = aslot + (wv * ALOOK + R % ALOOK) * (CIN * 64) + (INS ? r * 64 + ((kg ^ sw) * 16) : (kg >> 1) * 1024 + r * 64);
 #pragma unroll
@@ -1071,6 +1094,7 @@
           for (int v = 0; v < 2; v++)
             araw[0][ki * 2 + v] = INS ? *reinterpret_cast<const f32x4*>(sl + (v * KI + ki) * 1024)
                                       : *reinterpret_cast<const f32x4*>(sl + ki * 2048 + ((((kg & 1) * 2 + v) ^ sw) * 16));
+        }
       } else {
         f32x4 (&ar)[KI * 2] = araw[R % ABUF];
         if (younger == 0) vm_wait_tie<0>(ar);
@@ -1082,6 +1106,13 @@
         else vm_wait_tie<16>(ar);
       }
     }
+    if (!lv) {
+      if (lvn) {
+#pragma unroll
+        for (int ki = 0; ki < KI; ki++) issue_chunk(ki, R + ALOOK);
+      }
+      continue;
+    }
     const u32x4* bw = reinterpret_cast<const u32x4*>(SPR_RING(R) + g * WBYTES) + lane;
     u32x4 ah[KI], al[KI], bh[KI][NB], bl[KI][NB];
 #pragma unroll
@@ -1105,7 +1136,7 @@
       for (int j = 0; j < NB; j++) acc[j] = split_mfma<PREC>(ah[ki], bl[ki][j], acc[j]);
 #pragma unroll
       for (int j = 0; j < NB; j++) acc[j] = split_mfma<PREC>(ah[ki], bh[ki][j], acc[j]);
-      if (R + ALOOK < ROUNDS) {
+      if (lvn) {
         __builtin_amdgcn_sched_barrier(0);
         issue_chunk(ki, R + ALOOK);
         __builtin_amdgcn_sched_barrier(0);
@@ -1126,11 +1157,12 @@
   SPR_STAMP(13);
   for (int it = g; it < NB * 4; it += OG) {
     const int j = it >> 2, rr = it & 3;
-    const int col = j * 16 + r, row = row0 + kg * 4 + rr;
+    const int col = j * 16 + r;
+    const int row = ORD ? __shfl(myrow, kg * 4 + rr) : row0 + kg * 4 + rr;
     float v = part[((0 * NB + j) * 4 + rr) * 64 + lane];
 #pragma unroll
     for (int w = 1; w < OG; w++) v += part[((w * NB + j) * 4 + rr) * 64 + lane];
-    if (row < n) {
+    if (row0 + kg * 4 + rr < n) {
       if (scale) v = v * (scale[col] * ss.undo) + shift[col];
       else if constexpr (PREC == 1) v = v * ss.undo;
       if (relu) v = fmaxf(v, 0.f);
@@ -1151,9 +1183,10 @@
                                                                           const float* __restrict__ scale,
                                                                           const float* __restrict__ shift, int relu,
                                                                           float* __restrict__ out, const V3dActScale as,
-                                                                          unsigned short* __restrict__ out_s, const RbScanJob rider) {
+                                                                          unsigned short* __restrict__ out_s, const RbScanJob rider,
+                                                                          const int* __restrict__ order, const RbOrderJob oj) {
   constexpr int RB0 = OG * (CIN / 32) * (COUT / 16) * 2 * 1024;
-  static_assert(RB0 >= RB_SCAN_LDS, "a rider's scratch fits round buffer 0");
+  static_assert(RB0 >= RB_SCAN_LDS && RB0 >= RB_ORDER_LDS, "a rider's scratch fits round buffer 0");
   __shared__ __attribute__((aligned(16))) unsigned char wb0[RB0];
   constexpr bool HOST = !(CIN == 64 && COUT == 64);
   int bid = (int)blockIdx.x, nblk = (int)gridDim.x;
@@ -1164,6 +1197,12 @@
     }
     bid -= rider.blocks;
     nblk -= rider.blocks;
+    if (oj.blocks && bid < oj.blocks) {
+      if (threadIdx.x < V3D_BLOCK) rb_row_order_body(oj.nbr, oj.n_ptr, oj.cap, oj.K, oj.order, bid, wb0);
+      return;
+    }
+    bid -= oj.blocks;
+    nblk -= oj.blocks;
   }
   const int n = min(*n_ptr, cap);
   const int nwg = (n + 16 * TILES - 1) / (16 * TILES);
@@ -1172,7 +1211,7 @@
   float vmax = 0.f;
   for (int g = bid; g < nwg; g += nblk) {
     spconv_ring_body<CIN, COUT, OG, NBUF, NMV, ALOOK, STAGE, TILES, PREC, INS>(in, wimg, nbr, n, cap, scale, shift, relu, out, g, ss, vmax,
-                                                                              out_s, s_next, wb0);
+                                                                              out_s, s_next, wb0, order);
     __syncthreads();
   }
   if constexpr (PREC == 1) sp_range_check(as, vmax, ss.limit);
@@ -1185,6 +1224,9 @@
   unsigned short* out_split;
   const RbScanJob* rider;
   bool* rider_taken;
+  const int* order;
+  const RbOrderJob* order_job;
+  bool* order_job_taken;
 };
 
 static RbScanJob sp_ring_rider(const SpLaunch& sl, int max_blocks) {
@@ -1206,11 +1248,14 @@
     *slots = std::max(8, per_cu * n_cu / 8 * 8);
   }
   const RbScanJob r = sp_ring_rider(sl, CIN == 64 && COUT == 64 ? 0 : 512);
-  const int grid = std::min(v3d_ceil_div(cap, 16 * TILES), std::max(*slots - r.blocks, 8));
-  hipLaunchKernelGGL((spconv_fwd_rows_ring<CIN, COUT, OG, NBUF, NMV, ALOOK, STAGE, TILES, PREC, INS>), dim3(grid + r.blocks),
+  RbOrderJob oj{};
+  if (!(CIN == 64 && COUT == 64) && sl.order_job && sl.order_job->blocks > 0 && sl.order_job->blocks <= 512) oj = *sl.order_job;
+  const int grid = std::min(v3d_ceil_div(cap, 16 * TILES), std::max(*slots - r.blocks - oj.blocks, 8));
+  hipLaunchKernelGGL((spconv_fwd_rows_ring<CIN, COUT, OG, NBUF, NMV, ALOOK, STAGE, TILES, PREC, INS>), dim3(grid + r.blocks + oj.blocks),
                      dim3((TILES * OG + NMV) * 64), 0, st, INS ? (const float*)sl.in_split : in, (const unsigned short*)wimg, nbr, n_ptr, cap,
-                     scale, shift, relu, out, sl.as, sl.out_split, r);
+                     scale, shift, relu, out, sl.as, sl.out_split, r, CIN == 64 && COUT == 64 ? sl.order : nullptr, oj);
   if (sl.rider_taken) *sl.rider_taken = r.blocks > 0;
+  if (sl.order_job_taken) *sl.order_job_taken = oj.blocks > 0;
   V3D_CHECK_LAUNCH();
   return V3D_OK;
 }
@@ -1299,6 +1344,19 @@
                                       relu, out, rows_hint, (hipStream_t)stream, nullptr, 2, prec, &as, in_split, out_split);
 }
 
+extern "C" int v3d_sparse_conv_fwd_ordered(const float* in, const void* weight_image, const int32_t* nbr, const int32_t* n_out, int cap_out,
+                                            int K, int Cin, int Cout, const float* scale, const float* shift, int relu, float* out,
+                                            int rows_hint, int prec, const float* act_in, const float* act_next, int32_t* range_flag,
+                                            const void* in_split, void* out_split, const int32_t* order, v3d_stream_t stream) {
+  const V3dActScale as{act_in, act_next, range_flag, nullptr};
+  return v3d_i_sparse_conv_fwd_packed(in ? in : (const float*)in_split, weight_image, nbr, n_out, cap_out, K, Cin, Cout, scale, shift,
+                                      relu, out, rows_hint, (hipStream_t)stream, nullptr, 2, prec, &as, in_split, out_split, nullptr, nullptr,
+                                      order);
+}
+extern "C" int v3d_sparse_row_order(const int32_t* nbr, const int32_t* n_out, int cap_out, int K, int32_t* order, v3d_stream_t stream) {
+  return v3d_i_row_order(nbr, n_out, cap_out, K, order, (hipStream_t)stream);
+}
+
 template <int PREC>
 __global__ __launch_bounds__(256) void rows_split_kernel(const float* __restrict__ rows, const int* __restrict__ n_ptr, int cap, int C,
                                                          const float* __restrict__ entry, unsigned short* __restrict__ out) {
@@ -1334,12 +1392,19 @@
   return false;
 }
 
+bool v3d_i_sparse_conv_takes_order(int Cin, int Cout, int K, int rows_hint) {
+  if (Cin != 64 || Cout != 64 || K != 27) return false;
+  const int force = rows_hint < 0 ? -rows_hint : 0;
+  return force == 10 || force == 16 || (force >= 12 && force <= 14) || (force == 0 && rows_hint <= V3D_RING_ROWS);
+}
+
 int v3d_i_sparse_conv_fwd_packed(const float* in, const void* weight_image, const int32_t* nbr, const int32_t* n_out,
                                  int cap_out, int K, int Cin, int Cout, const float* scale, const float* shift, int relu,
                                  float* out, int rows_hint, hipStream_t st, const V3dDensifyOut* densify, int ring_tiles_min,
                                  int prec, const V3dActScale* act, const void* in_split, void* out_split, const RbScanJob* rider,
-                                 bool* rider_taken) {
+                                 bool* rider_taken, const int32_t* order, const RbOrderJob* order_job, bool* order_job_taken) {
   if (rider_taken) *rider_taken = false;
+  if (order_job_taken) *order_job_taken = false;
   if (!in || !weight_image || !nbr || !n_out || (!out && !out_split) || cap_out < 1 || K < 1) return V3D_EINVAL;
   if ((scale == nullptr) != (shift == nullptr)) return V3D_EINVAL;
   if (!out && densify) return V3D_EINVAL;
@@ -1353,6 +1418,9 @@
   sl.out_split = (unsigned short*)out_split;
   sl.rider = rider;
   sl.rider_taken = rider_taken;
+  sl.order = order;
+  sl.order_job = order_job;
+  sl.order_job_taken = order_job_taken;
 #define V3D_GO(ci, co, P, I) \
   return launch_rows<ci, co, P, I>(in, weight_image, nbr, n_out, cap_out, K, scale, shift, relu, out, rows_hint, st, densify, ring_tiles_min, sl)
 #define V3D_TRY(ci, co)                                    \
diff --git a/vision3d_amd/csrc/v3d_internal.h b/vision3d_amd/csrc/v3d_internal.h
--- a/vision3d_amd/csrc/v3d_internal.h
+++ b/vision3d_amd/csrc/v3d_internal.h
@@ -9,6 +9,7 @@
 #endif
 
 struct RbScanJob;
+struct RbOrderJob;
 struct RbStep;
 struct V3dRbHash {
   v3d_key_t* keys;
@@ -90,7 +91,13 @@
                                  const void* in_split = nullptr ,
                                  void* out_split = nullptr ,
                                  const RbScanJob* rider = nullptr ,
-                                 bool* rider_taken = nullptr );
+                                 bool* rider_taken = nullptr ,
+                                 const int32_t* order = nullptr ,
+                                 const RbOrderJob* order_job = nullptr ,
+                                 bool* order_job_taken = nullptr);
+
+#define V3D_ORDER_CHUNK 1024
+int v3d_i_row_order(const int32_t* nbr, const int32_t* n, int cap, int K, int32_t* order, hipStream_t st);
 
 struct V3dBrickTables {
   uint16_t* lidx;
@@ -105,6 +112,7 @@
                                 float* out, int prec, const V3dActScale* act, void* out_split, hipStream_t st);
 
 bool v3d_i_sparse_conv_packed_supported(int Cin, int Cout);
+bool v3d_i_sparse_conv_takes_order(int Cin, int Cout, int K, int rows_hint);
 
 int v3d_i_sparse_conv_fwd_exact(const float* in, const float* weight, const int32_t* nbr, const int32_t* n_out, int cap_out, int K,
                                 int Cin, int Cout, const float* scale, const float* shift, int relu, float* out, int algo,
diff --git a/vision3d_amd/runtime.py b/vision3d_amd/runtime.py
--- a/vision3d_amd/runtime.py
+++ b/vision3d_amd/runtime.py
@@ -100,6 +100,8 @@
         self.set_precision(precision)
         if os.environ.get("V3D_PRESPLIT", "1") == "0":
             self.set_presplit(False)
+        if os.environ.get("V3D_ROW_GROUPING", "1") == "0":
+            self.set_row_grouping(False)
         self.out_channels = self.layers[-1][0].out_channels
         shape = list(self.grid_shape)
         for conv, _, _ in self.layers:
@@ -134,6 +136,15 @@
 
     def set_presplit(self, on=True):
         L.check(L.lib().v3d_backbone_set_presplit(self._handle, int(bool(on))), "backbone_set_presplit")
+
+    def set_row_grouping(self, on=True):
+        L.check(L.lib().v3d_backbone_set_row_grouping(self._handle, int(bool(on))), "backbone_set_row_grouping")
+
+    def row_order(self, layer):
+        order, nbr, cap, k = C.c_void_p(), C.c_void_p(), C.c_int(), C.c_int()
+        L.check(L.lib().v3d_backbone_row_order(self._handle, int(layer), C.byref(order), C.byref(nbr), C.byref(cap), C.byref(k)), "backbone_row_order")
+        return (_view(order.value, (cap.value,), torch.int32, self.device) if order.value else None,
+                _view(nbr.value, (k.value, cap.value), torch.int32, self.device))
 
     def act_scales(self):
         ptr = L.lib().v3d_backbone_act_scales(self._handle)
```

Result: slower. 4499 (-6.5%).
